# terminusdb-labs/parallel-hnsw

Measured on AMD Instinct MI355X. Metric: queries/sec at recall@10≥0.95 on 1M×768 f32, higher is better.
Workload: dtype f32

## Files before the change

### parallel_hnsw_amd/csrc/api.hip

```cpp
#include <hip/hip_runtime.h>

#include <algorithm>
#include <atomic>
#include <cmath>
#include <cstdarg>
#include <cstdio>
#include <cstring>
#include <new>
#include <stdexcept>
#include <vector>

#include "exact_slices.h"
#include "phnsw_internal.h"

static thread_local std::string g_err;

void ph_set_error(const char *fmt, ...) {
  char buf[1024];
  va_list ap;
  va_start(ap, fmt);
  vsnprintf(buf, sizeof(buf), fmt, ap);
  va_end(ap);
  g_err = buf;
}
// ... 359 lines not shown
    int rc = ph_order_by_keys_device(L.pos + first, count, L.ord, 0);
    if (rc) return rc;
    L.ord_first = first;
    L.ord_count = count;
  }
  *out = L.ord;
  return 0;
}

int ph_layer_upload(phnsw_index *ix, const uint32_t *nodes, const uint32_t *neighbors, uint32_t n, uint32_t W,
                    PhLayerHost *out) {
  if (ix) ix->nodes_epoch++;
  PhLayerHost l;
  l.n_nodes = n;
  l.W = W;
  hipError_t e = hipMalloc(&l.nodes, (size_t)n * 4);
  if (e == hipSuccess) e = hipMalloc(&l.neighbors, (size_t)n * W * 4);
  if (e == hipSuccess) e = hipMemcpy(l.nodes, nodes, (size_t)n * 4, hipMemcpyHostToDevice);
  if (e == hipSuccess && neighbors)
    e = hipMemcpy(l.neighbors, neighbors, (size_t)n * W * 4, hipMemcpyHostToDevice);
  if (e != hipSuccess) {
    ph_layer_free(l);
    return ph_hip_fail(e, "layer upload", __FILE__, __LINE__);
  }
  if (!neighbors) {
    int rc = ph_fill_u32(l.neighbors, PH_EMPTY32, (uint64_t)n * W, 0);
    if (rc) {
      ph_layer_free(l);
      return rc;
    }
  }
  bool identity = true;
  for (uint32_t i = 0; i < n; i++)
    if (nodes[i] != i) {
      identity = false;
      break;
    }
  l.identity = identity;
  if (!identity) {
    e = hipMalloc(&l.vec2node, (size_t)ix->store->n * 4);
    if (e != hipSuccess) {
      ph_layer_free(l);
      return ph_hip_fail(e, "vec2node alloc", __FILE__, __LINE__);
    }
    int rc = ph_fill_u32(l.vec2node, PH_EMPTY32, ix->store->n, 0);
    if (!rc) rc = ph_scatter_vec2node(l.nodes, n, l.vec2node, 0);
    if (!rc) {
      e = hipDeviceSynchronize();
      if (e != hipSuccess) rc = ph_hip_fail(e, "vec2node sync", __FILE__, __LINE__);
    }
    if (rc) {
      ph_layer_free(l);
      return rc;
    }
  }
  *out = l;
  return 0;
}

static std::atomic<uint64_t> g_import_dups{0};
extern "C" uint64_t phnsw_debug_import_duplicates(void) { return g_import_dups.load(); }

static int validate_layer(const phnsw_store *s, const uint64_t *nodes, const uint64_t *neighbors, uint64_t n,
                          uint64_t W, std::vector<uint32_t> &nodes32, std::vector<uint32_t> &nb32) {
  if (n == 0 || W == 0 || W > 64 || n >= 0x7FFFFFFFull) {
    ph_set_error("layer shape unsupported: node_count=%llu neighborhood_size=%llu (1..64)", (unsigned long long)n,
                 (unsigned long long)W);
    return PHNSW_E_UNSUPPORTED;
  }
  const bool strict = getenv("PHNSW_STRICT_IMPORT") != nullptr;
  nodes32.resize(n);
  nb32.resize(n * W);
  for (uint64_t i = 0; i < n; i++) {
    if (nodes[i] >= s->n || (i > 0 && nodes[i] <= nodes[i - 1])) {
      ph_set_error("layer nodes must be strictly increasing VectorIds below the store size (search.rs:150-157)");
      return PHNSW_E_INVALID;
    }
    nodes32[i] = (uint32_t)nodes[i];
  }
  for (uint64_t i = 0; i < n; i++) {
    bool ended = false;
    uint64_t o = 0;
    for (uint64_t k = 0; k < W; k++) {
      uint64_t v = neighbors[i * W + k];
      if (v == PHNSW_EMPTY) {
        ended = true;
        continue;
      }
      if (ended || v >= n) {
        ph_set_error("neighbor row %llu: ids must be < node_count and sentinels trailing only (lib.rs:108-125)",
                     (unsigned long long)i);
        return PHNSW_E_INVALID;
      }
      bool dup = false;
      for (uint64_t j = 0; j < o; j++)
        if (nb32[i * W + j] == (uint32_t)v) dup = true;
      if (dup) {
        if (strict) {
          ph_set_error("neighbor row %llu holds node %llu twice (PHNSW_STRICT_IMPORT)", (unsigned long long)i,
                       (unsigned long long)v);
          return PHNSW_E_INVALID;
        }
        g_import_dups++;
        continue;
      }
      nb32[i * W + o++] = (uint32_t)v;
    }
    for (; o < W; o++) nb32[i * W + o] = PH_EMPTY32;
  }
  return 0;
}

extern "C" int phnsw_index_from_layers(phnsw_store *s, uint32_t layer_count, const uint64_t *node_counts,
                                       const uint64_t *neighborhood_sizes, const uint64_t *const *nodes,
                                       const uint64_t *const *neighbors, phnsw_index **out) try {
  if (!s || !out || layer_count == 0 || layer_count > PH_MAX_LAYERS || !node_counts || !neighborhood_sizes ||
      !nodes || !neighbors) {
    ph_set_error("phnsw_index_from_layers: invalid argument");
    return PHNSW_E_INVALID;
  }
  PH_HIP(hipSetDevice(s->device));
  phnsw_index *ix = new phnsw_index();
  ix->store = s;
  s->refcount++;
  phnsw_default_build_params(&ix->bp);
  for (uint32_t l = 0; l < layer_count; l++) {
    std::vector<uint32_t> n32, nb32;
    int rc = validate_layer(s, nodes[l], neighbors[l], node_counts[l], neighborhood_sizes[l], n32, nb32);
    PhLayerHost lh;
    if (!rc) rc = ph_layer_upload(ix, n32.data(), nb32.data(), (uint32_t)node_counts[l], (uint32_t)neighborhood_sizes[l], &lh);
    if (rc) {
      phnsw_index_destroy(ix);
      return rc;
    }
    ix->layers.push_back(lh);
  }
  *out = ix;
  return 0;
} catch (...) { return ph_caught(); }

extern "C" void phnsw_index_destroy(phnsw_index *ix) {
  if (!ix) return;
  hipSetDevice(ix->store->device);
  for (auto &l : ix->layers) ph_layer_free(l);
  ph_pending_free(ix);
  ph_workspace_free(ix->ws[0]);
  ph_workspace_free(ix->ws[1]);
  ph_host_stages_free(ix);
  ph_exact_free(ix);
  ph_auto_free(ix);
  ph_build_table_free(ix);
  if (ix->totals) hipFree(ix->totals);
  phnsw_store_destroy(ix->store);
  delete ix;
  ph_pool_trim();
}

extern "C" uint32_t phnsw_index_layer_count(const phnsw_index *ix) { return ix ? (uint32_t)ix->layers.size() : 0; }

extern "C" int phnsw_index_layer_info(const phnsw_index *ix, uint32_t lft, uint64_t *node_count, uint64_t *W) try {
  if (!ix || lft >= ix->layers.size()) {
    ph_set_error("layer %u out of range", lft);
    return PHNSW_E_INVALID;
  }
  if (node_count) *node_count = ix->layers[lft].n_nodes;
  if (W) *W = ix->layers[lft].W;
  return 0;
} catch (...) { return ph_caught(); }

extern "C" int phnsw_index_layer_read(const phnsw_index *ix, uint32_t lft, uint64_t *nodes, uint64_t *neighbors) try {
  if (!ix || lft >= ix->layers.size()) {
    ph_set_error("layer %u out of range", lft);
    return PHNSW_E_INVALID;
  }
  PH_HIP(hipSetDevice(ix->store->device));
  const PhLayerHost &l = ix->layers[lft];
  if (nodes) {
    std::vector<uint32_t> t(l.n_nodes);
    PH_HIP(hipMemcpy(t.data(), l.nodes, (size_t)l.n_nodes * 4, hipMemcpyDeviceToHost));
    for (uint32_t i = 0; i < l.n_nodes; i++) nodes[i] = t[i];
  }
  if (neighbors) {
    std::vector<uint32_t> t((size_t)l.n_nodes * l.W);
    PH_HIP(hipMemcpy(t.data(), l.neighbors, t.size() * 4, hipMemcpyDeviceToHost));
    for (size_t i = 0; i < t.size(); i++) neighbors[i] = t[i] == PH_EMPTY32 ? PHNSW_EMPTY : t[i];
  }
  return 0;
} catch (...) { return ph_caught(); }


int ph_check_sp(const phnsw_index *ix, const phnsw_search_params *sp) {
  if (!ix || !sp || ix->layers.empty()) {
    ph_set_error("search: null index/params or index without layers");
    return PHNSW_E_INVALID;
  }
  if (sp->number_of_candidates == 0 || sp->number_of_candidates > 1024 || sp->probe_depth == 0 ||
      sp->probe_depth > 0xFFFFFFFFull) {
    ph_set_error("search: number_of_candidates must be 1..1024 and probe_depth >= 1 (got %llu, %llu)",
                 (unsigned long long)sp->number_of_candidates, (unsigned long long)sp->probe_depth);
    return PHNSW_E_INVALID;
  }
  return 0;
}

static void fill_args(const phnsw_index *ix, const PhSearchCall &c, PhSearchArgs &a) {
  memset(&a, 0, sizeof(a));
  const phnsw_store *s = ix->store;
  a.dist = ph_dist_args(s);
  uint32_t nl = (c.upto == 0 || c.upto > ix->layers.size()) ? (uint32_t)ix->layers.size() : c.upto;
  a.n_layers = nl;
  for (uint32_t l = 0; l < nl; l++) {
    const PhLayerHost &h = ix->layers[l];
    a.layers[l].n_nodes = h.n_nodes;
    a.layers[l].W = h.W;
    a.layers[l].nodes = h.nodes;
    a.layers[l].neighbors = h.neighbors;
    a.layers[l].vec2node = h.identity ? nullptr : h.vec2node;
  }
  a.ef = (uint32_t)c.sp->number_of_candidates;
  a.upper = (uint32_t)std::min<uint64_t>(c.sp->upper_layer_candidate_count, 0xFFFFFFFFull);
  a.probe_depth = (uint32_t)c.sp->probe_depth;
  a.queries = c.queries;
  a.ldq = c.ldq;
  a.qids = c.qids;
  a.exclude = c.exclude;
  if (c.filter.words) {
    a.filter = c.filter.words;
    a.filter_stride = c.filter.stride;
    a.filter_flags = c.filter.flags;
  }
  a.nq = (uint32_t)c.nq;
  a.out_ids = c.out_ids;
  a.out_d = c.out_d;
  a.out_len = c.out_len;
  a.out_stats = c.out_stats;
  a.status = c.status;
  a.knn_mode = c.knn_mode;
  a.out_stride = c.out_stride;
  a.out_hit = c.out_hit;
  a.threshold = c.threshold;
  a.first_node = c.first_node;
  a.hit_eps = c.hit_eps;
  a.cap_max = c.knn_mode == 2 ? c.out_stride : 0;
  a.out_index = c.out_index;
  a.order = c.order;
}

uint32_t ph_default_ovf_cap(uint32_t ef) {
  if (const char *e = getenv("PHNSW_OVF_CAP"))
    if (atoi(e) > 0) return (uint32_t)atoi(e);
  return std::max<uint32_t>(8192u, ef * 64u);
}
static uint32_t default_ovf_cap(uint32_t ef) { return ph_default_ovf_cap(ef); }

static uint64_t two_launch_min() {
  const char *e = getenv("PHNSW_TWO_LAUNCH_MIN");
  return (e && atoll(e) > 0) ? (uint64_t)atoll(e) : (uint64_t)PH_TWO_LAUNCH_MIN;
}
static std::atomic<uint64_t> g_two_launch_count{0};
extern "C" uint64_t phnsw_debug_two_launch_count(void) { return g_two_launch_count.load(); }
extern "C" uint32_t phnsw_debug_last_search_chunks(const phnsw_index *ix) { return ix ? ix->ws[ix->ws_last].n_chunks : 0; }

extern "C" int phnsw_stream_create_beside(int device, void *other_stream, void **out_stream) try {
  if (!out_stream) {
    ph_set_error("phnsw_stream_create_beside: out_stream is NULL");
    return PHNSW_E_INVALID;
  }
  PH_HIP(hipSetDevice(device));
  hipStream_t st = nullptr;
  int rc = ph_stream_beside((hipStream_t)other_stream, &st);
  if (rc) return rc;
  *out_stream = (void *)st;
  return 0;
} catch (...) { return ph_caught(); }

static int attach_probes(phnsw_index *mix, const PhSearchCall &c, PhSearchArgs &a) {
  (void)mix, (void)c, (void)a;
#ifdef PH_CELL_PROBE
  {
    static unsigned long long *probe_dev = nullptr;
    if (!probe_dev) {
      PH_HIP(hipMalloc(&probe_dev, 12 * sizeof(unsigned long long)));
      PH_HIP(hipMemset(probe_dev, 0, 12 * sizeof(unsigned long long)));
    } else {
      unsigned long long h[12];
      PH_HIP(hipDeviceSynchronize());
      PH_HIP(hipMemcpy(h, probe_dev, sizeof(h), hipMemcpyDeviceToHost));
      if (h[11]) {
        fprintf(stderr, "[cell probe] %llu queries, %llu bottom-layer evaluations; within r chain ranks of the landing cell:", h[11], h[10]);
        for (int k = 0; k < 10; k++) fprintf(stderr, " r<=%u: %.3f", k ? (1u << (k - 1)) : 0u, (double)h[k] / (double)h[10]);
        fprintf(stderr, "\n");
      }
      PH_HIP(hipMemset(probe_dev, 0, 12 * sizeof(unsigned long long)));
    }
    a.probe_out = probe_dev;
    a.probe_pos = nullptr;
    if (!c.knn_mode && ph_store_f32(mix->store) && c.nq >= 1000) {
      int rc = ph_layer_anchor_pos(mix->store, mix->layers[a.n_layers - 1]);
      if (rc) return rc;
      a.probe_pos = mix->layers[a.n_layers - 1].pos;
    }
  }
#endif
#ifdef PH_VISITED_PROBE
  {
    static unsigned long long *vprobe_dev = nullptr;
    if (!vprobe_dev) {
      PH_HIP(hipMalloc(&vprobe_dev, 130 * sizeof(unsigned long long)));
      PH_HIP(hipMemset(vprobe_dev, 0, 130 * sizeof(unsigned long long)));
    } else {
      unsigned long long h[130];
      PH_HIP(hipDeviceSynchronize());
      PH_HIP(hipMemcpy(h, vprobe_dev, sizeof(h), hipMemcpyDeviceToHost));
      for (int k = 0; k < 2; k++) {
        unsigned long long n = 0, sum = 0, run = 0;
        for (int b = 0; b < 64; b++) n += h[64 * k + b], sum += h[64 * k + b] * (64ull * b + 32ull);
        if (!n) continue;
        fprintf(stderr, "[visited probe] %s: %llu walks, mean ~%.0f ids, past the LDS load limit: %.4f; ids < 64*(b+1) for",
                k ? "bottom layer" : "upper gathered layers", n, (double)sum / (double)n, (double)h[128 + k] / (double)n);
        for (int b = 0; b < 64; b++) {
          run += h[64 * k + b];
          if (h[64 * k + b]) fprintf(stderr, " b%d:%.4f", b, (double)run / (double)n);
        }
        fprintf(stderr, "\n");
      }
      PH_HIP(hipMemset(vprobe_dev, 0, 130 * sizeof(unsigned long long)));
    }
    a.vprobe_out = vprobe_dev;
  }
#endif
  return 0;
}

int ph_search_device(const phnsw_index *ix, const PhSearchCall &c) {
  phnsw_index *mix = const_cast<phnsw_index *>(ix);
  const uint64_t nq = c.nq;
  const uint32_t knn_mode = c.knn_mode, out_stride = c.out_stride;
  uint32_t *const out_index = c.out_index;
  const hipStream_t stream = c.stream;
  if (ph_store_converted(ix->store) && (knn_mode || out_index || c.hint || c.out_hit)) {
    return ph_search_only_unsupported(ix->store, knn_mode ? "knn / threshold_nn" : (out_index ? "search_instrumented" : "build search"));
  }
  PhSearchArgs a;
  fill_args(ix, c, a);
  if (ix->dbg_order && ix->dbg_order_n == nq) a.order = ix->dbg_order;
  std::lock_guard<std::mutex> g(mix->ws_mutex);
  if (!mix->totals) {
    PH_HIP(hipMalloc(&mix->totals, 16));
    PH_HIP(hipMemset(mix->totals, 0, 16));
  }
  a.totals = mix->totals;
  PhWorkspace &ws = mix->ws[mix->ws_next & 1];
  mix->ws_last = mix->ws_next & 1;
  mix->ws_next++;
  int rc = ph_workspace_ensure(ix, ws, std::max(a.ef, a.cap_max), c.ovf_cap ? c.ovf_cap : default_ovf_cap(a.ef));
  if (rc) return rc;
  const uint32_t T = (knn_mode || out_index) ? 0u : ph_tiny_layer_count(ix, a.n_layers, a.ef);
  uint32_t first_big = a.n_layers;
  for (uint32_t l = std::max(1u, T); l < a.n_layers; l++)
    if (ph_layer_own_launch(ix->layers[l].n_nodes, ph_row_bytes(ix->store))) {
      first_big = l;
      break;
    }
  if (!a.order && knn_mode && nq >= PH_ORDER_MIN) {
    PhLayerHost &B = mix->layers[a.n_layers - 1];
    rc = ph_layer_anchor_pos(ix->store, B);
    if (!rc && c.first_node + nq <= B.n_nodes) rc = ph_layer_range_order(B, c.first_node, (uint32_t)nq, &a.order);
    if (rc) return rc;
  }
  const bool split = (ph_store_f32(ix->store) || ph_store_converted(ix->store)) && !a.order && !knn_mode && !out_stride && !out_index && first_big < a.n_layers &&
                     nq >= two_launch_min() &&
                     !getenv("PHNSW_NO_LOCALITY");
  if (split) {
    g_two_launch_count++;
    rc = ph_workspace_order_ensure(ws, a.nq);
    for (uint32_t l = first_big; l < a.n_layers && !rc; l++)
      rc = ph_layer_anchor_pos(ix->store, mix->layers[l - 1]);
    if (rc) return rc;
  }
  rc = attach_probes(mix, c, a);
  if (rc) return rc;
  rc = ph_search_begin(ws, stream);
  if (rc) return rc;
  bool kept_table = false;
  if (c.hint && T && !split) {
    rc = ph_build_table_prepare(mix, ws, a, *c.hint, T, stream, &kept_table);
    if (rc) return rc;
  }
  const uint64_t tmax = (T && !kept_table) ? ph_tiny_max_positions(ix, a.n_layers, a.ef) : 0;
  const uint64_t chunk = (tmax && nq > tmax) ? tmax : nq;
  for (uint64_t c0 = 0; c0 < nq; c0 += chunk) {
    PhSearchArgs b = a;
    const uint64_t cnt = std::min<uint64_t>(chunk, nq - c0);
    const bool last_chunk = c0 + cnt == nq;
    b.nq = (uint32_t)cnt;
    if (b.order) {
      b.order += c0;
    } else if (c0) {
      const uint32_t ostride = out_stride ? out_stride : b.ef;
      if (b.queries) b.queries += c0 * c.ldq;
      if (b.qids) b.qids += c0;
      if (b.exclude) b.exclude += c0;
      if (b.filter) b.filter += c0 * b.filter_stride;
      b.out_ids += c0 * ostride;
      b.out_d += c0 * ostride;
      b.out_len += c0;
      if (b.out_stats) b.out_stats += 2 * c0;
      b.status += c0;
      if (b.out_hit) b.out_hit += c0;
      b.first_node += (uint32_t)c0;
    }
    ws.n_chunks = (uint32_t)(c0 / chunk) + 1;
    PH_HIP(hipEventRecord(ws.evc, stream));
    if (c0) PH_HIP(hipMemsetAsync(ws.dtotals, 0, sizeof(unsigned long long) * 3 * PH_MAX_DISPATCH, stream));
    if (!kept_table) {
      rc = ph_tiny_prepare(ix, ws, b, T, stream);
      if (rc) return rc;
    }
    ws.d_tiny = b.tiny_layers != 0;
    PH_HIP(hipEventRecord(ws.evd[0], stream));
    if (!split) {
      b.launch_totals = ws.dtotals;
      b.launch_tab = ws.dtotals + 2 * PH_MAX_DISPATCH;
      rc = ph_search_launch(ix, ws, b, stream, last_chunk);
      if (rc) return rc;
      PH_HIP(hipEventRecord(ws.evd[1], stream));
      ws.n_dispatch = 1;
      ws.d_lo[0] = knn_mode ? b.n_layers - 1 : 0;
      ws.d_hi[0] = b.n_layers;
      continue;
    }
    const uint32_t Td = b.tiny_layers;
    const bool dense_first = Td && Td < b.n_layers && b.nq >= PH_DENSE_SPLIT_MIN && !getenv("PHNSW_NO_DENSE_SPLIT");
    if (dense_first) b.dense_flag = ws.tiny_member + b.tiny_n;
    uint32_t di = 0;
    uint32_t *const out_hit_final = b.out_hit;
    const uint32_t first_hi = dense_first ? Td : first_big;
    for (uint32_t lo = 0, hi = first_hi; lo < b.n_layers; lo = hi, hi = (lo == Td && dense_first && first_big > Td) ? first_big : hi + 1) {
      PhSearchArgs p = b;
      const bool last = hi == b.n_layers;
      p.layer_lo = lo;
      p.layer_hi = hi;
      if (lo) p.tiny_layers = 0;
      if (dense_first) {
        p.dense_only = lo == 0 ? 1u : 0u;
        p.after_dense = lo == Td ? Td : 0u;
      }
      p.order = lo ? ws.oorder : nullptr;
      p.out_hit = last ? out_hit_final : nullptr;
      p.out_key = last ? nullptr : ws.okey;
      p.key_pos = last ? nullptr : ix->layers[hi - 1].pos;
      p.launch_totals = ws.dtotals + 2 * di;
      p.launch_tab = ws.dtotals + 2 * PH_MAX_DISPATCH + di;
      rc = ph_search_launch(ix, ws, p, stream, last && last_chunk);
      if (!rc && !last) rc = ph_workspace_order_sort(ws, b.nq, stream);
      if (rc) return rc;
      PH_HIP(hipEventRecord(ws.evd[1 + di], stream));
      ws.d_lo[di] = lo;
      ws.d_hi[di] = hi;
      ws.n_dispatch = ++di;
    }
  }
  return 0;
}

static int check_device_call(const char *call, const phnsw_index *ix, const PhSearchCall &c) {
  int rc = ph_check_sp(ix, c.sp);
  if (rc) return rc;
  if ((!c.queries && !c.qids) || !c.out_ids || !c.out_d || !c.out_len || !c.status || c.nq > 0xFFFFFFFFull ||
      (c.queries && (c.ldq < ix->store->ld || (c.ldq % 4) || ((uintptr_t)c.queries % 16)))) {
    ph_set_error("%s: invalid argument (queries need ldq >= store ld, multiple of 4, 16-byte base)", call);
    return PHNSW_E_INVALID;
  }
  return 0;
}

static PhSearchCall device_call(const float *queries_dev, uint32_t ldq, const uint32_t *qids_dev, uint64_t nq,
                                const phnsw_search_params *sp, uint32_t upto_layers, const uint32_t *exclude_dev,
                                uint32_t *out_ids_dev, float *out_d_dev, uint32_t *out_len_dev, uint32_t *out_stats_dev,
                                uint32_t *status_dev, void *stream) {
  PhSearchCall c = {};
  c.queries = queries_dev, c.ldq = ldq, c.qids = qids_dev, c.exclude = exclude_dev, c.nq = nq;
  c.sp = sp, c.upto = upto_layers;
  c.out_ids = out_ids_dev, c.out_d = out_d_dev, c.out_len = out_len_dev, c.status = status_dev;
  c.out_stats = out_stats_dev;
  c.stream = (hipStream_t)stream;
  return c;
}

extern "C" int phnsw_search_batch_device(const phnsw_index *ix, const float *queries_dev, uint32_t ldq,
                                         const uint32_t *qids_dev, uint64_t nq, const phnsw_search_params *sp,
                                         uint32_t upto_layers, const uint32_t *exclude_dev, uint32_t *out_ids_dev,
                                         float *out_d_dev, uint32_t *out_len_dev, uint32_t *out_stats_dev,
                                         uint32_t *status_dev, void *stream) try {
  const PhSearchCall c = device_call(queries_dev, ldq, qids_dev, nq, sp, upto_layers, exclude_dev, out_ids_dev, out_d_dev,
                                     out_len_dev, out_stats_dev, status_dev, stream);
  int rc = check_device_call("phnsw_search_batch_device", ix, c);
  if (rc) return rc;
  if (nq == 0) return 0;
  PH_HIP(hipSetDevice(ix->store->device));
  return ph_search_device(ix, c);
} catch (...) { return ph_caught(); }


int ph_filter_check(const phnsw_index *ix, const uint32_t *filter, uint32_t stride, uint32_t flags, const char *call,
                    PhFilter *f) {
  const uint64_t words = (ix->store->n + 31u) / 32u;
  if (flags & ~(uint32_t)PHNSW_FILTER_STRICT) {
    ph_set_error("%s: unknown flag bits 0x%x", call, flags);
    return PHNSW_E_INVALID;
  }
  if (stride && stride < words) {
    ph_set_error("%s: filter_stride_words %u is below the %llu words of one bitmap (0 = one shared bitmap)", call, stride,
                 (unsigned long long)words);
    return PHNSW_E_INVALID;
  }
  f->words = filter;
  f->stride = filter ? stride : 0u;
  f->flags = flags;
  return 0;
}

extern "C" int phnsw_search_batch_filtered_device(const phnsw_index *ix, const float *queries_dev, uint32_t ldq,
                                                  const uint32_t *qids_dev, uint64_t nq, const phnsw_search_params *sp,
                                                  uint32_t upto_layers, const uint32_t *exclude_dev,
                                                  const uint32_t *filter_dev, uint32_t filter_stride_words, uint32_t flags,
                                                  uint32_t *out_ids_dev, float *out_d_dev, uint32_t *out_len_dev,
                                                  uint32_t *out_stats_dev, uint32_t *status_dev, void *stream) try {
  PhSearchCall c = device_call(queries_dev, ldq, qids_dev, nq, sp, upto_layers, exclude_dev, out_ids_dev, out_d_dev,
                               out_len_dev, out_stats_dev, status_dev, stream);
  int rc = check_device_call("phnsw_search_batch_filtered_device", ix, c);
  if (rc) return rc;
  rc = ph_filter_check(ix, filter_dev, filter_stride_words, flags, "phnsw_search_batch_filtered_device", &c.filter);
  if (rc) return rc;
  if (!c.filter.words) c.filter.words = ix->default_filter;
  if (nq == 0) return 0;
  PH_HIP(hipSetDevice(ix->store->device));
  return ph_search_device(ix, c);
} catch (...) { return ph_caught(); }

extern "C" int phnsw_index_set_filter_device(phnsw_index *ix, const uint32_t *filter_dev) try {
  if (!ix) {
    ph_set_error("phnsw_index_set_filter_device: null index");
    return PHNSW_E_INVALID;
  }
  ix->default_filter = filter_dev;
  return 0;
} catch (...) { return ph_caught(); }


int ph_exact_check(const phnsw_index *ix, uint64_t k, const char *call) {
  if (!ix || ix->layers.empty()) {
    ph_set_error("%s: null index or index without layers", call);
    return PHNSW_E_INVALID;
  }
  if (!ph_exact_k_valid(k)) {
    ph_set_error("%s: k must be 1..1024 (got %llu)", call, (unsigned long long)k);
    return PHNSW_E_INVALID;
  }
  if (ph_store_pq_shared(ix->store)) {
    ph_set_error("%s: not supported over a shared-codebook PQ store; use its reconstruction store", call);
    return PHNSW_E_UNSUPPORTED;
  }
  return 0;
}

extern "C" int phnsw_search_exact_filtered_device(const phnsw_index *ix, const float *queries_dev, uint32_t ldq,
                                                  const uint32_t *qids_dev, uint64_t nq, const uint32_t *exclude_dev,
                                                  const uint32_t *filter_dev, uint32_t filter_stride_words, uint64_t k,
                                                  uint32_t *out_ids_dev, float *out_d_dev, uint32_t *out_len_dev,
                                                  uint32_t *status_dev, void *stream) try {
  const char *const call = "phnsw_search_exact_filtered_device";
  int rc = ph_exact_check(ix, k, call);
  if (rc) return rc;
  if (nq == 0) return 0;
  if (((!queries_dev) == (!qids_dev)) || !out_ids_dev || !out_d_dev || !out_len_dev || !status_dev || nq > 0xFFFFFFFFull ||
      (queries_dev && (ldq < ix->store->ld || (ldq % 4) || ((uintptr_t)queries_dev % 16)))) {
    ph_set_error("%s: invalid argument (queries or qids, exactly one; outputs; queries need ldq >= store ld, multiple of 4, "
                 "16-byte base)", call);
    return PHNSW_E_INVALID;
  }
  PhExactCall c = {};
  rc = ph_filter_check(ix, filter_dev, filter_stride_words, 0u, call, &c.filter);
  if (rc) return rc;
  if (!c.filter.words) c.filter.words = ix->default_filter;
  c.queries = queries_dev, c.ldq = ldq, c.qids = qids_dev, c.exclude = exclude_dev, c.nq = nq, c.k = (uint32_t)k;
  c.out_ids = out_ids_dev, c.out_d = out_d_dev, c.out_len = out_len_dev, c.status = status_dev;
  c.stream = (hipStream_t)stream;
  PH_HIP(hipSetDevice(ix->store->device));
  return ph_exact_device(ix, c);
} catch (...) { return ph_caught(); }

extern "C" int phnsw_filter_count_device(const phnsw_index *ix, const uint32_t *filter_dev, uint32_t filter_stride_words,
                                         uint64_t nbitmaps, uint32_t *out_count_dev, void *stream) try {
  const char *const call = "phnsw_filter_count_device";
  if (!ix || ix->layers.empty() || (!out_count_dev && nbitmaps)) {
    ph_set_error("%s: null index, index without layers or null output", call);
    return PHNSW_E_INVALID;
  }
  PhFilter f;
  int rc = ph_filter_check(ix, filter_dev, filter_stride_words, 0u, call, &f);
  if (rc) return rc;
  if (!f.words) f.words = ix->default_filter;
  PH_HIP(hipSetDevice(ix->store->device));
  return ph_filter_count(ix, f, nbitmaps, out_count_dev, (hipStream_t)stream);
} catch (...) { return ph_caught(); }

extern "C" int phnsw_debug_last_tiny_table(const phnsw_index *ix, float *out_host, uint64_t cap_floats, uint32_t *npos,
                                           uint32_t *tn, uint32_t *stride, int *g) try {
  if (!ix) return PHNSW_E_INVALID;
  phnsw_index *mix = const_cast<phnsw_index *>(ix);
  std::lock_guard<std::mutex> lock(mix->ws_mutex);
  PhWorkspace &ws = mix->ws[mix->ws_last];
  if (!ws.timed || !ws.d_tiny || !ws.tiny_d) {
    ph_set_error("the last search on this index made no dense table");
    return PHNSW_E_INVALID;
  }
  const uint64_t need = (uint64_t)ws.tiny_last_npos * ws.tiny_last_stride;
  if (npos) *npos = ws.tiny_last_npos;
  if (tn) *tn = ws.tiny_last_tn;
  if (stride) *stride = ws.tiny_last_stride;
  if (g) *g = ws.tiny_table_g;
  if (out_host) {
    if (cap_floats < need) {
      ph_set_error("phnsw_debug_last_tiny_table: %llu floats needed", (unsigned long long)need);
      return PHNSW_E_INVALID;
    }
    PH_HIP(hipSetDevice(ix->store->device));
    PH_HIP(hipEventSynchronize(ws.ev1));
    PH_HIP(hipMemcpy(out_host, ws.tiny_d, need * 4u, hipMemcpyDeviceToHost));
  }
  return 0;
} catch (...) { return ph_caught(); }

extern "C" int phnsw_debug_layer_pos(phnsw_index *ix, uint32_t lft, uint32_t *out_host) try {
  if (lft >= ix->layers.size() || !ix->layers[lft].pos) return PHNSW_E_INVALID;
  PH_HIP(hipMemcpy(out_host, ix->layers[lft].pos, (size_t)ix->layers[lft].n_nodes * 4, hipMemcpyDeviceToHost));
  return 0;
} catch (...) { return ph_caught(); }

extern "C" int phnsw_debug_set_order(phnsw_index *ix, const uint32_t *order_dev, uint64_t n) try {
  ix->dbg_order = order_dev;
  ix->dbg_order_n = n;
  return 0;
} catch (...) { return ph_caught(); }

extern "C" int phnsw_index_counters(const phnsw_index *ix, uint64_t *n_dist, uint64_t *n_hops) try {
  if (!ix) return PHNSW_E_INVALID;
  unsigned long long h[2] = {0, 0};
  if (ix->totals) {
    PH_HIP(hipSetDevice(ix->store->device));
    PH_HIP(hipDeviceSynchronize());
    PH_HIP(hipMemcpy(h, ix->totals, 16, hipMemcpyDeviceToHost));
  }
  if (n_dist) *n_dist = h[0];
  if (n_hops) *n_hops = h[1];
  return 0;
} catch (...) { return ph_caught(); }

extern "C" int phnsw_last_search_kernel_ms(const phnsw_index *ix, float *ms) try {
  if (!ix || !ms) return PHNSW_E_INVALID;
  phnsw_index *mix = const_cast<phnsw_index *>(ix);
  std::lock_guard<std::mutex> g(mix->ws_mutex);
  PhWorkspace &ws = mix->ws[mix->ws_last];
  if (!ws.timed) {
    ph_set_error("no search has been launched on this index");
    return PHNSW_E_INVALID;
  }
  PH_HIP(hipEventSynchronize(ws.ev1));
  PH_HIP(hipEventElapsedTime(ms, ws.ev0, ws.ev1));
  return 0;
} catch (...) { return ph_caught(); }

extern "C" int phnsw_last_search_dispatches(const phnsw_index *ix, uint32_t cap, uint32_t *count, float *ms,
                                            uint64_t *n_dist, uint64_t *n_hops, uint32_t *layer_lo,
                                            uint32_t *layer_hi) try {
  if (!ix || !count) return PHNSW_E_INVALID;
  phnsw_index *mix = const_cast<phnsw_index *>(ix);
  std::lock_guard<std::mutex> g(mix->ws_mutex);
  PhWorkspace &ws = mix->ws[mix->ws_last];
  if (!ws.timed) {
    ph_set_error("no search has been launched on this index");
    return PHNSW_E_INVALID;
  }
  PH_HIP(hipSetDevice(ix->store->device));
  PH_HIP(hipEventSynchronize(ws.ev1));
  unsigned long long h[2 * PH_MAX_DISPATCH];
  PH_HIP(hipMemcpy(h, ws.dtotals, sizeof(h), hipMemcpyDeviceToHost));
  const uint32_t n = ws.n_dispatch + 1;
  *count = n;
  for (uint32_t i = 0; i < n && i < cap; i++) {
    float t = 0.f;
    PH_HIP(hipEventElapsedTime(&t, i == 0 ? ws.evc : ws.evd[i - 1], ws.evd[i]));
    if (ms) ms[i] = t;
    if (n_dist) n_dist[i] = i ? h[2 * (i - 1)] : 0;
    if (n_hops) n_hops[i] = i ? h[2 * (i - 1) + 1] : 0;
    if (layer_lo) layer_lo[i] = i ? ws.d_lo[i - 1] : 0;
    if (layer_hi) layer_hi[i] = i ? ws.d_hi[i - 1] : 0;
  }
  return 0;
} catch (...) { return ph_caught(); }

extern "C" int phnsw_last_search_table_evals(const phnsw_index *ix, uint32_t cap, uint32_t *count, uint64_t *n_table) try {
  if (!ix || !count) return PHNSW_E_INVALID;
  phnsw_index *mix = const_cast<phnsw_index *>(ix);
  std::lock_guard<std::mutex> g(mix->ws_mutex);
  PhWorkspace &ws = mix->ws[mix->ws_last];
  if (!ws.timed) {
    ph_set_error("no search has been launched on this index");
    return PHNSW_E_INVALID;
  }
  PH_HIP(hipSetDevice(ix->store->device));
  PH_HIP(hipEventSynchronize(ws.ev1));
  unsigned long long h[PH_MAX_DISPATCH];
  PH_HIP(hipMemcpy(h, ws.dtotals + 2 * PH_MAX_DISPATCH, sizeof(h), hipMemcpyDeviceToHost));
  const uint32_t n = ws.n_dispatch + 1;
  *count = n;
  for (uint32_t i = 0; i < n && i < cap; i++)
    if (n_table) n_table[i] = i ? h[i - 1] : 0;
  return 0;
} catch (...) { return ph_caught(); }

extern "C" int phnsw_dense_top_layers(const phnsw_index *ix, uint64_t number_of_candidates, uint32_t *layers, uint64_t *nodes,
                                      uint32_t *matrix_cores) try {
  if (!ix || !ix->store) {
    ph_set_error("phnsw_dense_top_layers: null index");
    return PHNSW_E_INVALID;
  }
  const uint32_t ef = (uint32_t)std::min<uint64_t>(number_of_candidates, 0xFFFFFFFFull);
  const uint32_t T = ph_tiny_layer_count(ix, (uint32_t)ix->layers.size(), ef);
  if (layers) *layers = T;
  if (nodes) *nodes = T ? ix->layers[T - 1].n_nodes : 0;
  if (matrix_cores) *matrix_cores = (T && ph_tiny_matrix_cores(ix)) ? 1u : 0u;
  return 0;
} catch (...) { return ph_caught(); }

extern "C" int phnsw_knn(const phnsw_index *ix, uint64_t k, uint64_t probe_depth, uint64_t *out_ids, float *out_d,
                         uint64_t *out_len) try {
  if (ix)
    if (int rc = ph_search_only_unsupported(ix->store, "phnsw_knn")) return rc;
  if (!ix || ix->layers.empty() || k == 0 || k * 3 > 1024) {
    ph_set_error("phnsw_knn: k must be 1..341");
    return PHNSW_E_INVALID;
  }
  const PhLayerHost &L = ix->layers.back();
  phnsw_search_params sp = {k * 3, k * 3, probe_depth};
  uint64_t n = L.n_nodes, cap = k * 3;
  std::vector<uint64_t> ids(n * cap), len(n);
  std::vector<float> d(n * cap);
  PhHostSearch h = {};
  h.nq = n, h.sp = &sp, h.knn_mode = 1;
  h.out_ids = ids.data(), h.out_d = d.data(), h.out_len = len.data();
  int rc = ph_search_host(ix, h);
  if (rc) return rc;
  std::vector<uint64_t> nodes(n);
  rc = phnsw_index_layer_read(ix, (uint32_t)ix->layers.size() - 1, nodes.data(), nullptr);
  if (rc) return rc;
  for (uint64_t i = 0; i < n; i++) {
    uint64_t o = 0;
    for (uint64_t j = 0; j < len[i] && o < k; j++) {
      if (ids[i * cap + j] == nodes[i]) continue;
      out_ids[i * k + o] = ids[i * cap + j];
      out_d[i * k + o] = d[i * cap + j];
      o++;
    }
    out_len[i] = o;
    for (; o < k; o++) {
      out_ids[i * k + o] = PHNSW_EMPTY;
      out_d[i * k + o] = PH_FMAX;
    }
  }
  return 0;
} catch (...) { return ph_caught(); }

namespace {
template <class T>
struct GrowBuf {
  T *p = nullptr;
  size_t have = 0;
  int alloc(size_t count) {
    count = std::max<size_t>(count, 1);
    if (have >= count) return 0;
    if (p) hipFree(p);
    p = nullptr;
    have = 0;
    hipError_t e = hipMalloc((void **)&p, count * sizeof(T));
    if (e != hipSuccess) return ph_hip_fail(e, "hipMalloc (threshold_nn)", __FILE__, __LINE__);
    have = count;
    return 0;
  }
  ~GrowBuf() {
    if (p) hipFree(p);
  }
  GrowBuf() = default;
  GrowBuf(const GrowBuf &) = delete;
  GrowBuf &operator=(const GrowBuf &) = delete;
};
}
#define PH_TRY_(x)         \
  do {                     \
    int rc__ = (x);        \
    if (rc__) return rc__; \
  } while (0)

static int threshold_nn_big(const phnsw_index *ix, const phnsw_search_params *sp, float threshold,
                            const std::vector<uint32_t> &all_nodes, const std::vector<uint32_t> &h_nodes, uint64_t max_out,
                            uint64_t *out_ids, float *out_d, uint64_t *out_len, uint32_t lds_cap) {
  const PhLayerHost &L = ix->layers.back();
  const uint32_t n = L.n_nodes;
  const uint64_t isd = sp->number_of_candidates;
  const uint32_t os = (uint32_t)std::min<uint64_t>(max_out + 2, (uint64_t)n + 1);
  const uint64_t words = ((uint64_t)n + 31) / 32 + 1;
  uint64_t cap0 = isd * 2;
  while (cap0 <= lds_cap) cap0 *= 2;
  GrowBuf<uint32_t> d_nodes, d_vis, d_q, d_oid, d_len, d_status, d_counter;
  GrowBuf<float> d_od;
  GrowBuf<uint2> d_ovf;
  std::vector<uint32_t> h_ids, h_len, h_status;
  std::vector<float> h_d;
  size_t piece = std::max<size_t>(1, std::min<size_t>(16384, (1ull << 30) / ((size_t)os * 8)));
  if (const char *e = getenv("PHNSW_THRESHOLD_BIG_PIECE"))
    if (atoll(e) > 0) piece = (size_t)atoll(e);
  for (size_t c0 = 0; c0 < all_nodes.size(); c0 += piece) {
  std::vector<uint32_t> nodes(all_nodes.begin() + c0, all_nodes.begin() + std::min(all_nodes.size(), c0 + piece));
  uint64_t cap = cap0;
  while (!nodes.empty()) {
    if (cap > 0x7FFFFFFFull) {
      ph_set_error("threshold_nn: queue capacity beyond 2^31");
      return PHNSW_E_UNSUPPORTED;
    }
    const bool final_cap = cap >= 2ull * n;
    const uint64_t per_slot = cap * 8 + (uint64_t)n * 8 + words * 4;
    uint64_t budget = 4ull << 30;
    if (const char *e = getenv("PHNSW_THRESHOLD_BIG_BYTES")) budget = strtoull(e, nullptr, 10);
    const uint32_t grid = (uint32_t)std::min<uint64_t>(std::min<uint64_t>(nodes.size(), 1024), std::max<uint64_t>(1, budget / per_slot));
    const size_t cnt = nodes.size();
    PH_TRY_(d_nodes.alloc(cnt));
    PH_TRY_(d_oid.alloc(cnt * os));
    PH_TRY_(d_od.alloc(cnt * os));
    PH_TRY_(d_len.alloc(cnt));
    PH_TRY_(d_status.alloc(cnt));
    PH_TRY_(d_counter.alloc(128));
    PH_TRY_(d_vis.alloc((size_t)grid * words));
    PH_TRY_(d_ovf.alloc((size_t)grid * n));
    PH_TRY_(d_q.alloc((size_t)grid * 2 * cap));
    PH_HIP(hipMemset(d_vis.p, 0, (size_t)grid * words * 4));
    PH_HIP(hipMemcpy(d_nodes.p, nodes.data(), cnt * 4, hipMemcpyHostToDevice));
    PhSearchCall c = {};
    c.nq = cnt, c.sp = sp;
    c.out_ids = d_oid.p, c.out_d = d_od.p, c.out_len = d_len.p, c.status = d_status.p;
    c.knn_mode = 2, c.threshold = threshold, c.out_stride = os;
    PhSearchArgs a;
    fill_args(ix, c, a);
    a.cap_max = (uint32_t)cap;
    a.knn_nodes = d_nodes.p;
    a.big_q = d_q.p;
    a.visited = d_vis.p;
    a.visited_words = words;
    a.ovf = d_ovf.p;
    a.ovf_cap = n;
    a.counter = d_counter.p;
    PH_TRY_(ph_search_launch_big(ix, a, grid, 0));
    PH_HIP(hipDeviceSynchronize());
    h_ids.resize(cnt * os);
    h_d.resize(cnt * os);
    h_len.resize(cnt);
    h_status.resize(cnt);
    PH_HIP(hipMemcpy(h_ids.data(), d_oid.p, cnt * os * 4, hipMemcpyDeviceToHost));
    PH_HIP(hipMemcpy(h_d.data(), d_od.p, cnt * os * 4, hipMemcpyDeviceToHost));
    PH_HIP(hipMemcpy(h_len.data(), d_len.p, cnt * 4, hipMemcpyDeviceToHost));
    PH_HIP(hipMemcpy(h_status.data(), d_status.p, cnt * 4, hipMemcpyDeviceToHost));
    std::vector<uint32_t> again;
    for (size_t x = 0; x < cnt; x++) {
      const uint64_t i = nodes[x];
      if (h_status[x] == 6 && !final_cap) {
        again.push_back(nodes[x]);
        continue;
      }
      if (h_status[x]) {
        ph_set_error("threshold_nn: node %llu failed with status %u at a queue capacity of %llu", (unsigned long long)i,
                     h_status[x], (unsigned long long)cap);
        return PHNSW_E_OVERFLOW;
      }
      uint64_t o = 0;
      for (uint32_t j = 0; j < h_len[x]; j++) {
        const uint32_t v = h_ids[x * os + j];
        const float d = h_d[x * os + j];
        if (v == h_nodes[i]) continue;
        if (!(d < threshold)) break;
        if (o == max_out) {
          ph_set_error("threshold_nn: node %llu has more than max_out=%llu results", (unsigned long long)i,
                       (unsigned long long)max_out);
          return PHNSW_E_OVERFLOW;
        }
        out_ids[i * max_out + o] = v;
        out_d[i * max_out + o] = d;
        o++;
      }
      out_len[i] = o;
      for (; o < max_out; o++) {
        out_ids[i * max_out + o] = PHNSW_EMPTY;
        out_d[i * max_out + o] = PH_FMAX;
      }
    }
    nodes.swap(again);
    cap *= 2;
  }
  }
  return 0;
}

extern "C" int phnsw_threshold_nn(const phnsw_index *ix, float threshold, uint64_t probe_depth,
                                  uint64_t initial_search_depth, uint64_t max_out, uint64_t *out_ids, float *out_d,
                                  uint64_t *out_len) try {
  if (ix)
    if (int rc = ph_search_only_unsupported(ix->store, "phnsw_threshold_nn")) return rc;
  if (!ix || ix->layers.empty() || !out_ids || !out_d || !out_len || initial_search_depth == 0 ||
      initial_search_depth > 0x40000000ull || probe_depth == 0 || max_out == 0) {
    ph_set_error("phnsw_threshold_nn: initial_search_depth and probe_depth must be >= 1");
    return PHNSW_E_INVALID;
  }
  const phnsw_store *s = ix->store;
  PH_HIP(hipSetDevice(s->device));
  const PhLayerHost &L = ix->layers.back();
  const uint32_t n = L.n_nodes, CAPMAX = 1024, CHUNK = 16384;
  phnsw_search_params sp = {initial_search_depth, initial_search_depth, probe_depth};
  std::vector<uint32_t> h_nodes(n);
  PH_HIP(hipMemcpy(h_nodes.data(), L.nodes, (size_t)n * 4, hipMemcpyDeviceToHost));
  std::vector<uint32_t> big;
  if (initial_search_depth > CAPMAX || getenv("PHNSW_THRESHOLD_ALL_BIG")) {
    big.resize(n);
    for (uint32_t i = 0; i < n; i++) big[i] = i;
    return threshold_nn_big(ix, &sp, threshold, big, h_nodes, max_out, out_ids, out_d, out_len, 0);
// ... 70 lines not shown
```

### parallel_hnsw_amd/csrc/phnsw_internal.h

```cpp
#pragma once
#include <hip/hip_runtime.h>
#include <stdint.h>
#include <stdlib.h>

#include <mutex>
#include <string>
#include <vector>

#include "../../include/phnsw.h"

#define PH_EMPTY32 0xFFFFFFFFu
#define PH_FMAX 3.4028234663852886e38f
#define PH_MAX_LAYERS 24
#define PH_WAVE 64
#define PH_MAX_DISPATCH 24
#define PH_DENSE_SPLIT_MIN 2048u
#define PH_TINY_MAX_NODES 8192u
#define PH_TINY_LDS_NODES 1024u
#define PH_TINY_MAX_LAYERS 8

void ph_set_error(const char *fmt, ...);
int ph_caught() noexcept;
int ph_hip_fail(hipError_t e, const char *what, const char *file, int line);
#define PH_HIP(x)                                                       \
  do {                                                                  \
    hipError_t e__ = (x);                                               \
    if (e__ != hipSuccess) return ph_hip_fail(e__, #x, __FILE__, __LINE__); \
  } while (0)

struct PhLayerDev {
  uint32_t n_nodes;
  uint32_t W;
  const uint32_t *nodes;
  const uint32_t *neighbors;
  const uint32_t *vec2node;
};

struct PhLayerHost {
  uint32_t n_nodes = 0, W = 0;
  uint32_t *nodes = nullptr;
  uint32_t *neighbors = nullptr;
  float *nbr_dist = nullptr;
  uint64_t links_epoch = 0;
  uint32_t *vec2node = nullptr;
  bool identity = false;
  uint32_t *recall_q = nullptr;
  uint32_t recall_n = 0;
  uint32_t *pos = nullptr;
  uint32_t *ord = nullptr;
  uint32_t ord_first = 0, ord_count = 0;
};

enum PhRowKind : int {
  PH_ROWS_F32 = 0,
  PH_ROWS_F16,
  PH_ROWS_I8,
  PH_ROWS_PQ,
  PH_ROWS_PQ_SHARED,
  PH_ROWS_I8Q,
};
static inline bool ph_rows_converted(int kind) { return kind == PH_ROWS_F16 || kind == PH_ROWS_I8 || kind == PH_ROWS_I8Q; }
static inline bool ph_rows_i8_layout(int kind) { return kind == PH_ROWS_I8 || kind == PH_ROWS_I8Q; }
static inline const char *ph_rows_name(int kind) {
  static const char *const names[] = {"f32", "f16", "i8", "product-quantised", "shared-codebook product-quantised", "i8q"};
  return names[kind];
}
static inline int ph_chunk_count(uint32_t nv4) { return nv4 <= 64 ? 1 : (nv4 <= 192 ? 3 : (nv4 <= 384 ? 6 : 0)); }
int ph_dim_unsupported(uint32_t dim);
struct PhRows {
  const void *base;
  uint32_t stride;
  int kind;
};

struct PhDistArgs {
  PhRows rows;
  uint32_t ld, nv4;
  int metric;
  const uint8_t *codes;
  const uint16_t *codes16;
  const float *codebook;
  uint32_t m, ksub, dsub;
  uint32_t table_f16;
};

struct phnsw_store {
  int device = 0;
  int kind = PH_ROWS_F32;
  float *rows = nullptr;
  uint8_t *codes = nullptr;
  uint16_t *codes16 = nullptr;
  phnsw_store *centroid_store = nullptr;
  phnsw_index *centroid_index = nullptr;
  phnsw_search_params quantized_search = {0, 0, 0};
  float *codebook = nullptr;
  uint32_t pq_m = 0, pq_ksub = 0, pq_dsub = 0;
  uint32_t pq_table_f16 = 0;
  void *packed = nullptr;
  uint32_t packed_stride = 0;
  float *anchors = nullptr;
  uint32_t *anchor_rank = nullptr;
  uint32_t n_anchors = 0;
  bool owns_rows = true;
  uint64_t n = 0;
  uint32_t dim = 0, ld = 0;
  int metric = 0;
  int refcount = 1;
};

struct PhTinyPrepKey {
  bool valid = false;
  uint64_t nodes_epoch = 0;
  uint32_t T = 0, tn = 0;
  const void *nodes[PH_TINY_MAX_LAYERS] = {}, *nbrs[PH_TINY_MAX_LAYERS] = {}, *vec2node = nullptr;
  uint32_t n[PH_TINY_MAX_LAYERS] = {}, W[PH_TINY_MAX_LAYERS] = {};
  uint64_t links[PH_TINY_MAX_LAYERS] = {};
};
struct PhTinyPackKey {
  bool valid = false;
  uint64_t nodes_epoch = 0;
  const void *vecs = nullptr, *tnodes = nullptr;
  uint32_t ld = 0, tn = 0, nv = 0;
};

struct PhWorkspace {
  uint32_t *visited = nullptr;
  uint64_t visited_words = 0;
  uint2 *ovf = nullptr;
  uint32_t ovf_cap = 0;
  uint32_t n_slots = 0;
  uint32_t *counter = nullptr;
  hipEvent_t ev0 = nullptr, ev1 = nullptr;
  hipEvent_t evc = nullptr;
  bool timed = false;
  void *pq_tables = nullptr;
  size_t pq_tables_bytes = 0;
  uint32_t *okey = nullptr, *okey_sorted = nullptr, *oiota = nullptr, *oorder = nullptr;
  void *sort_tmp = nullptr;
  size_t sort_tmp_bytes = 0;
  uint32_t order_cap = 0;
  float *tiny_d = nullptr;
  size_t tiny_d_bytes = 0;
  uint32_t *tiny_nbr = nullptr;
  size_t tiny_nbr_bytes = 0;
  uint32_t *tiny_member = nullptr;
  size_t tiny_member_bytes = 0;
  float4 *tiny_pq = nullptr, *tiny_pn = nullptr;
  size_t tiny_pq_bytes = 0, tiny_pn_bytes = 0;
  PhTinyPrepKey tiny_prep_key;
  PhTinyPackKey tiny_pack_key;
  int tiny_table_g = 0;
  uint32_t tiny_last_npos = 0, tiny_last_tn = 0, tiny_last_stride = 0;
  uint2 *dense_ovf = nullptr;
  size_t dense_ovf_bytes = 0;
  uint32_t *ovf_s = nullptr;
  size_t ovf_s_cap = 0;
  hipEvent_t evd[PH_MAX_DISPATCH + 1] = {};
  unsigned long long *dtotals = nullptr;
  uint32_t n_dispatch = 0;
  uint32_t n_chunks = 0;
  int cus = 0;
  uint32_t d_lo[PH_MAX_DISPATCH] = {}, d_hi[PH_MAX_DISPATCH] = {};
  bool d_tiny = false;
};

struct PhBuildTable {
  float *D = nullptr;
  size_t bytes = 0;
  size_t cap = 0;
  const uint32_t *qnodes = nullptr, *tnodes = nullptr;
  uint32_t qn = 0, tn = 0, T = 0, stride = 0;
  uint32_t lo_alloc = 0, hi_alloc = 0, lo = 0, hi = 0;
  uint64_t epoch = 0;
};
struct PhRowHint {
  const uint32_t *qnodes;
  uint32_t qn;
  const uint32_t *vec2node;
  uint32_t first, count;
  bool contiguous;
};

struct PhFilter {
  const uint32_t *words;
  uint32_t stride, flags;
};

struct PhExactScratch {
  uint64_t *keys = nullptr;
  size_t bytes = 0;
  hipEvent_t done = nullptr;
};

struct PhAutoSet;
struct PhPendingLayer;
struct PhHostStage;
struct phnsw_index {
  std::vector<PhHostStage *> stages;
  std::mutex stage_mutex;
  std::vector<PhBuildTable> bt;
  std::vector<std::pair<float *, size_t>> bt_spare;
  bool bt_enabled = false;
  uint64_t nodes_epoch = 0;
  PhPendingLayer *pending = nullptr;
  phnsw_store *store = nullptr;
  std::vector<PhLayerHost> layers;
  phnsw_build_params bp;
  std::mutex ws_mutex;
  PhWorkspace ws[2];
  uint32_t ws_next = 0, ws_last = 0;
  float last_kernel_ms = 0.f;
  unsigned long long *totals = nullptr;
  const uint32_t *dbg_order = nullptr;
  const uint32_t *default_filter = nullptr;
  uint64_t dbg_order_n = 0;
  std::mutex exact_mutex;
  PhExactScratch exact[2];
  uint32_t exact_next = 0;
  std::vector<PhAutoSet *> autos;
  std::mutex auto_mutex;
};

struct PhSearchArgs {
  PhDistArgs dist;
  const float *queries;
  uint32_t ldq;
  const uint32_t *qids;
  const uint32_t *exclude;
  const uint32_t *filter;
  uint32_t filter_stride, filter_flags;
  uint32_t nq;
  uint32_t n_layers;
  PhLayerDev layers[PH_MAX_LAYERS];
  uint32_t ef, upper, probe_depth;
  uint32_t *out_ids;
  float *out_d;
  uint32_t *out_len;
  uint32_t *out_stats;
  uint32_t *status;
  uint32_t *visited;
  uint64_t visited_words;
  uint2 *ovf;
  uint32_t ovf_cap;
  uint32_t *counter;
  uint32_t knn_mode;
  float threshold;
  uint32_t first_node;
  uint32_t cap_max;
  const uint32_t *knn_nodes;
  uint32_t *big_q;
  uint32_t tiny_lds_nodes;
  float hit_eps;
  uint32_t out_stride;
  unsigned long long *totals;
  unsigned long long *launch_totals;
  unsigned long long *launch_tab;
  void *pq_tables;
  uint32_t pq_table_bytes;
  uint32_t layer_lo, layer_hi;
  uint32_t *out_key;
  const uint32_t *key_pos;
  uint32_t dense_only, after_dense;
  const uint32_t *dense_flag;
  uint2 *dense_ovf;
  uint32_t dense_ovf_cap;
#ifdef PH_CELL_PROBE
  const uint32_t *probe_pos;
  unsigned long long *probe_out;
#endif
#ifdef PH_VISITED_PROBE
  unsigned long long *vprobe_out;
#endif
  uint32_t vis_slots, vis_limit, vis_off;
  const uint32_t *order;
  uint32_t seg;
  uint32_t *out_hit;
  uint32_t *out_index;
  uint32_t *ovf_s;
  uint32_t tiny_layers, tiny_n, tiny_stride;
  const float *tiny_d;
  const uint32_t *tiny_nbr;
  const uint32_t *tiny_member;
  uint32_t tiny_rows, tiny_row_first;
  const uint32_t *tiny_row_map;
  uint32_t tiny_off[PH_TINY_MAX_LAYERS];
};

uint32_t ph_default_ovf_cap(uint32_t ef);
hipError_t ph_timed_malloc(void **p, size_t bytes);
hipError_t ph_timed_free(void *p);
#ifndef PH_RAW_ALLOC
#define hipMalloc(p, n) ph_timed_malloc((void **)(p), (n))
#define hipFree(p) ph_timed_free((void *)(p))
#endif
int ph_stream_beside(hipStream_t other, hipStream_t *io);
hipError_t ph_pool_alloc(void **p, size_t bytes);
void ph_pool_free(void *p);
void ph_pool_trim(void);
void ph_layer_free(PhLayerHost &l);
void ph_pending_free(phnsw_index *ix);
void ph_host_stages_free(phnsw_index *ix);
int ph_layer_upload(phnsw_index *ix, const uint32_t *nodes, const uint32_t *neighbors, uint32_t n, uint32_t W,
                    PhLayerHost *out);
struct PhSearchCall {
  const float *queries;
  uint32_t ldq;
  const uint32_t *qids, *exclude;
  uint64_t nq;
  const phnsw_search_params *sp;
  uint32_t upto;
  PhFilter filter;
  uint32_t *out_ids;
  float *out_d;
  uint32_t *out_len, *status;
  uint32_t *out_stats;
  uint32_t ovf_cap;
  hipStream_t stream;
  uint32_t knn_mode, first_node, out_stride;
  float threshold, hit_eps;
  uint32_t *out_hit, *out_index;
  const uint32_t *order;
  const PhRowHint *hint;
};
int ph_search_device(const phnsw_index *ix, const PhSearchCall &c);
int ph_check_sp(const phnsw_index *ix, const phnsw_search_params *sp);
int ph_filter_check(const phnsw_index *ix, const uint32_t *filter, uint32_t stride, uint32_t flags, const char *call,
                    PhFilter *f);
struct PhHostSearch {
  const float *queries;
  const uint64_t *qids, *exclude;
  uint64_t nq;
  const phnsw_search_params *sp;
  uint32_t upto, knn_mode;
  uint64_t out_k;
  uint64_t *out_ids;
  float *out_d;
  uint64_t *out_len;
  uint64_t *out_stats, *out_index;
  PhFilter filter;
  bool filter_on_device;
  bool exact;
};
int ph_search_host(const phnsw_index *ix, const PhHostSearch &h);
struct PhExactCall {
  const float *queries;
  uint32_t ldq;
  const uint32_t *qids, *exclude;
  uint64_t nq;
  PhFilter filter;
  uint32_t k;
  uint32_t *out_ids;
  float *out_d;
  uint32_t *out_len, *status;
  hipStream_t stream;
  const uint32_t *list;
};
int ph_exact_device(const phnsw_index *ix, const PhExactCall &c);
int ph_exact_supported(const phnsw_index *ix, uint32_t k);
void ph_exact_bottom_layer(const phnsw_index *ix, uint32_t *n_nodes, const uint32_t **nodes, const uint32_t **vec2node);
int ph_filter_count(const phnsw_index *ix, const PhFilter &f, uint64_t nbitmaps, uint32_t *out_count_dev, hipStream_t stream);
void ph_exact_free(phnsw_index *ix);
struct PhAutoCall {
  const float *queries;
  uint32_t ldq;
  const uint32_t *qids, *exclude;
  uint64_t nq;
  const phnsw_search_params *sp;
  PhFilter filter;
  uint32_t k;
  uint64_t scan_below;
  uint32_t *out_ids;
  float *out_d;
  uint32_t *out_len, *status;
  uint32_t *out_route;
  hipStream_t stream;
};
int ph_auto_device(const phnsw_index *ix, const PhAutoCall &c);
void ph_auto_free(phnsw_index *ix);
int ph_exact_check(const phnsw_index *ix, uint64_t k, const char *call);
#define PH_ORDER_MIN 16384u
#define PH_POS_MIN 256u
#define PH_SPLIT_BYTES (4ull << 20)
static inline bool ph_layer_own_launch(uint64_t n_nodes, uint32_t row_bytes) {
  const char *e = getenv("PHNSW_SPLIT_BYTES");
  const uint64_t limit = (e && atoll(e) > 0) ? (uint64_t)atoll(e) : (uint64_t)PH_SPLIT_BYTES;
  return n_nodes * (uint64_t)row_bytes > limit;
}
int ph_layer_anchor_pos(const phnsw_store *s, PhLayerHost &L);
bool ph_layer_wants_cells(const phnsw_store *s, uint32_t n_nodes);
int ph_layer_cells_range(const phnsw_store *s, const PhLayerHost &L, uint32_t first, uint32_t count, uint32_t *out_pos);
void ph_store_anchors_free(phnsw_store *s);
int ph_order_by_keys_device(const uint32_t *keys, uint32_t n, uint32_t *order_out, hipStream_t st);
int ph_layer_range_order(PhLayerHost &L, uint32_t first, uint32_t count, const uint32_t **out);

static inline bool ph_store_converted(const phnsw_store *s) { return ph_rows_converted(s->kind); }
static inline bool ph_store_f32(const phnsw_store *s) { return s->kind == PH_ROWS_F32; }
static inline bool ph_store_pq(const phnsw_store *s) { return s->kind == PH_ROWS_PQ; }
static inline bool ph_store_pq_shared(const phnsw_store *s) { return s->kind == PH_ROWS_PQ_SHARED; }
int ph_converted_gather_rows(const phnsw_store *s, const uint32_t *ids_dev, uint32_t first, uint32_t cnt, float *out_dev);
int ph_converted_store_read(const phnsw_store *s, uint64_t first, uint64_t count, float *out);

int ph_tiny_prepare(const phnsw_index *ix, PhWorkspace &ws, PhSearchArgs &a, uint32_t max_layers, hipStream_t stream);
int ph_build_table_prepare(phnsw_index *ix, PhWorkspace &ws, PhSearchArgs &a, const PhRowHint &h, uint32_t T,
                           hipStream_t stream, bool *used);
void ph_build_table_free(phnsw_index *ix);
size_t ph_tiny_lds_bytes(const PhSearchArgs &a);
bool ph_tiny_matrix_cores(const phnsw_index *ix);
uint32_t ph_tiny_layer_count(const phnsw_index *ix, uint32_t n_layers, uint32_t ef);
uint64_t ph_tiny_max_positions(const phnsw_index *ix, uint32_t n_layers, uint32_t ef);
void ph_tiny_free(PhWorkspace &ws);

int ph_search_begin(PhWorkspace &ws, hipStream_t stream);
int ph_search_launch(const phnsw_index *ix, PhWorkspace &ws, PhSearchArgs &a, hipStream_t stream, bool mark_end = true);
int ph_search_launch_big(const phnsw_index *ix, PhSearchArgs &a, uint32_t grid, hipStream_t stream);
int ph_workspace_order_ensure(PhWorkspace &ws, uint32_t nq);
int ph_workspace_order_sort(PhWorkspace &ws, uint32_t nq, hipStream_t stream);
void ph_workspace_order_free(PhWorkspace &ws);
#define PH_TWO_LAUNCH_MIN 32768u
int ph_workspace_ensure(const phnsw_index *ix, PhWorkspace &ws, uint32_t ef, uint32_t ovf_cap);
void ph_workspace_free(PhWorkspace &ws);
size_t ph_tiny_beside_lds(const phnsw_index *ix, const PhSearchArgs &a);
static inline PhRows ph_store_rows(const phnsw_store *s) {
  PhRows r;
  r.base = ph_store_converted(s) ? (const void *)s->packed : (const void *)s->rows;
  r.stride = ph_store_converted(s) ? s->packed_stride : s->ld * 4u;
  r.kind = s->kind;
  return r;
}
static inline PhDistArgs ph_dist_args(const phnsw_store *s) {
  PhDistArgs d;
  d.rows = ph_store_rows(s);
  d.ld = s->ld;
  d.nv4 = s->ld / 4;
  d.metric = s->metric;
  d.codes = s->codes;
  d.codes16 = s->codes16;
  d.codebook = s->codebook;
  d.m = s->pq_m;
  d.ksub = s->pq_ksub;
  d.dsub = s->pq_dsub;
  d.table_f16 = s->pq_table_f16;
  return d;
}
static inline uint32_t ph_row_bytes(const phnsw_store *s) { return ph_store_rows(s).stride; }
static inline int ph_search_only_unsupported(const phnsw_store *s, const char *call) {
  if (!s || !ph_store_converted(s)) return 0;
  ph_set_error("%s: not supported on an %s store or an index over one (search-only; use the f32 store)", call,
               ph_rows_name(s->kind));
  return PHNSW_E_UNSUPPORTED;
}
static inline bool ph_pq_global_tables() {
  const char *e = getenv("PHNSW_PQ_TABLE");
  return !(e && e[0] == 'l');
}
static inline size_t ph_pq_lds_bytes(const phnsw_store *s) {
  return ph_store_pq(s) ? (size_t)s->pq_m * s->pq_ksub * (s->pq_table_f16 == 2 ? 1 : (s->pq_table_f16 ? 2 : 4)) : 0;
}

void ph_comm_range(const phnsw_comm *comm, uint32_t r, uint64_t n, uint64_t *chunk, uint64_t *first, uint64_t *count);
int ph_comm_all_gather_device(const phnsw_comm *comm, const void *send_dev, void *recv_dev, uint64_t bytes);

int ph_synth_rows(float *rows_dev, uint64_t first, uint64_t count, uint32_t dim, uint32_t ld,
                  uint64_t seed, int normalize, hipStream_t s);
int ph_synth_clustered_rows(float *rows_dev, uint64_t first, uint64_t count, uint32_t dim, uint32_t ld, uint64_t seed,
                            uint32_t n_clusters, float noise, hipStream_t s);
int ph_distance_batch(const phnsw_store *st, const float *q_dev, uint32_t query_id, const uint32_t *ids_dev,
                      uint32_t k, float *out_dev, hipStream_t s);
int ph_fill_u32(uint32_t *p, uint32_t v, uint64_t n, hipStream_t s);
int ph_take_launch(const uint32_t *ids, const float *d, uint32_t ef, uint32_t k, uint64_t n, uint64_t *ids64, float *dk,
                   hipStream_t s);
int ph_scatter_vec2node(const uint32_t *nodes, uint32_t n, uint32_t *vec2node, hipStream_t s);
int ph_count_nan(const float *rows, uint64_t n_floats, uint32_t *out_count_dev, hipStream_t s);

__host__ __device__ inline uint64_t ph_mix64(uint64_t x) {
  x ^= x >> 30;
  x *= 0xBF58476D1CE4E5B9ULL;
  x ^= x >> 27;
  x *= 0x94D049BB133111EBULL;
  x ^= x >> 31;
  return x;
}
__host__ __device__ inline uint64_t ph_mulhi64(uint64_t a, uint64_t b) {
#if defined(__HIP_DEVICE_COMPILE__)
  return __umul64hi(a, b);
#else
  return (uint64_t)(((__uint128_t)a * b) >> 64);
#endif
}
__host__ __device__ inline uint64_t ph_feistel_perm(uint64_t i, uint64_t domain, uint64_t key) {
  if (domain <= 1) return 0;
  uint32_t bits = 0;
  while (((uint64_t)1 << bits) < domain) bits++;
  uint32_t h = (bits + 1) / 2;
  if (h == 0) h = 1;
  uint64_t mask = ((uint64_t)1 << h) - 1;
  uint64_t x = i;
  do {
    uint64_t L = x >> h, R = x & mask;
    for (uint32_t r = 0; r < 4; r++) {
      uint64_t f = ph_mix64(R + key * 0x9E3779B97F4A7C15ULL + r * 0xC2B2AE3D27D4EB4FULL) & mask;
      uint64_t nl = R;
      R = L ^ f;
      L = nl;
    }
    x = (L << h) | R;
  } while (x >= domain);
  return x;
}
void ph_shuffle_u64(uint64_t *v, uint64_t n, uint64_t seed);
```

### parallel_hnsw_amd/csrc/search.hip

```cpp
#include "search_kernels.h"


static int pick_capc(uint32_t ef) { return ef <= 128 ? 2 : (ef <= 512 ? 8 : (ef <= 1024 ? 16 : 0)); }

static bool vis_lds_on() {
  const char *e = getenv("PHNSW_VISITED");
  return !(e && !strcmp(e, "global"));
}
static int pick_capc_f32(uint32_t ef, bool grows, int nv) {
  return (!grows && ef > 128 && ef <= 256 && vis_lds_on() && vis_lds_shape(4, nv)) ? 4 : pick_capc(ef);
}
static int pick_capc_dense(uint32_t ef) { return ef <= 128 ? 2 : (ef <= 256 ? 4 : (ef <= 512 ? 8 : (ef <= 1024 ? 16 : 0))); }

static int pick_pqr(const phnsw_store *s, int capc) {
  if (!ph_store_pq(s) || s->pq_table_f16 != 2 || (capc != 2 && capc != 8) || getenv("PHNSW_PQ_TABLE")) return 0;
  const uint32_t m = s->pq_m;
  return (s->pq_ksub == 256 && (m == 32 || m == 64 || m == 96 || m == 128)) ? (int)m : 0;
}
static ph_search_fn pick_kernel_instr(int capc, int nv) {
#define PH_KI(C, N) \
  if (capc == C && nv == N) return (ph_search_fn)ph_search_kernel_instr<C, N>;
  PH_KI(8, 1) PH_KI(8, 3) PH_KI(8, 6) PH_KI(16, 1) PH_KI(16, 3) PH_KI(16, 6)
#undef PH_KI
  return nullptr;
}

#define PH_LATENCY_MAX 1024u
static size_t lds_bytes(int capc, size_t pq_lds) { return (size_t)(5 * capc * 64 + 64) * 4 + pq_lds; }

#define PH_VIS_SLOTS_MIN 1024u
#define PH_VIS_SLOTS_MAX 4096u
#define PH_LDS_GRANULE 1280u

static uint32_t vis_table_slots(ph_search_fn fn, size_t lds, int per_cu, size_t lds_cu, uint32_t ef, size_t hole) {
  if (!vis_lds_on() || per_cu <= 0) return 0;
  if (const char *e = getenv("PHNSW_VISITED_LDS_SLOTS")) {
    const long n = atol(e);
    if (n > 0) return lds + (size_t)n * 4u <= 64u * 1024u ? (uint32_t)n : 0u;
  }
  const uint32_t least = std::max<uint32_t>(PH_VIS_SLOTS_MIN, 4u * ef);
  size_t share = lds_cu / (size_t)per_cu;
  if (hole) {
    const size_t G = PH_LDS_GRANULE, hole_blocks = (hole + G - 1u) / G;
    const size_t with_hole = lds_cu / G > hole_blocks ? (lds_cu / G - hole_blocks) / (size_t)per_cu * G : 0u;
    if (with_hole >= lds + (size_t)least * 4u) share = with_hole;
  }
  const size_t room = std::min<size_t>(share, 64u * 1024u);
  if (room <= lds) return 0;
  for (uint32_t n = std::min<uint32_t>(PH_VIS_SLOTS_MAX, (uint32_t)((room - lds) / 4u) & ~63u); n >= least; n -= 64u) {
    int got = 0;
    if (hipOccupancyMaxActiveBlocksPerMultiprocessor(&got, (const void *)fn, 64, lds + (size_t)n * 4u) == hipSuccess &&
        got >= per_cu)
      return n;
  }
  return 0;
}

struct PhKernelChoice {
  ph_search_fn fn = nullptr;
  PhKernelFamily family = PH_KF_ROWS_F32;
  int capc = 0;
  int nv = 0;
  int pqr_m = 0;
  size_t pq_lds = 0;
  bool lat_shape = false;
};
static bool kf_rows(PhKernelFamily f) {
  return f == PH_KF_ROWS_F32 || f == PH_KF_ROWS_F16 || f == PH_KF_ROWS_I8 || f == PH_KF_ROWS_I8Q;
}

static PhKernelChoice pick_unfiltered_kernel(const phnsw_store *s, uint32_t ef_max, uint32_t nv4, bool grows, uint64_t nq,
                                             bool instr) {
  PhKernelChoice k;
  const int capc = pick_capc(ef_max);
  k.capc = capc;
  if (!capc) return k;
  switch (s->kind) {
    case PH_ROWS_PQ:
      k.pqr_m = pick_pqr(s, capc);
      k.family = k.pqr_m ? PH_KF_PQ_REG : PH_KF_PQ_TABLE;
      if (k.pqr_m) {
        k.fn = pick_kernel_pqr<false>(capc, k.pqr_m);
      } else {
        k.fn = pick_kernel_pqt<false>(capc, ph_pq_global_tables());
        k.pq_lds = ph_pq_global_tables() ? 0 : ph_pq_lds_bytes(s);
      }
      return k;
    case PH_ROWS_PQ_SHARED:
      k.family = PH_KF_PQ_SHARED;
      k.nv = ph_chunk_count(nv4);
      k.fn = pick_kernel_pqs<false>(capc, k.nv);
      return k;
    default: break;
  }
  k.nv = ph_chunk_count(nv4);
  if (s->kind == PH_ROWS_F32 && !instr && nq <= PH_LATENCY_MAX && !getenv("PHNSW_NO_LAT") && pick_kernel_lat<false>(capc, k.nv)) {
    k.family = PH_KF_LATENCY;
    k.fn = pick_kernel_lat<false>(capc, k.nv);
    k.lat_shape = true;
    return k;
  }
  if (instr) {
    k.family = PH_KF_INSTR;
    k.capc = std::max(capc, 8);
    k.fn = pick_kernel_instr(k.capc, k.nv);
    k.lat_shape = nq <= PH_LATENCY_MAX && !getenv("PHNSW_NO_LAT") && pick_kernel_lat<false>(capc, k.nv);
    return k;
  }
  k.capc = pick_capc_f32(ef_max, grows, k.nv);
  switch (s->kind) {
    case PH_ROWS_F16: k.family = PH_KF_ROWS_F16; k.fn = pick_kernel_rows<DistF16, false>(k.capc, k.nv); break;
    case PH_ROWS_I8: k.family = PH_KF_ROWS_I8; k.fn = pick_kernel_rows<DistI8, false>(k.capc, k.nv); break;
    case PH_ROWS_I8Q: k.family = PH_KF_ROWS_I8Q; k.fn = pick_kernel_rows<DistI8Q, false>(k.capc, k.nv); break;
    default: k.family = PH_KF_ROWS_F32; k.fn = pick_kernel_rows<DistF32, false>(k.capc, k.nv); break;
  }
  return k;
}

static PhKernelChoice pick_search_kernel(const phnsw_store *s, uint32_t ef_max, uint32_t nv4, bool grows, uint64_t nq,
                                         bool instr, bool filt = false) {
  PhKernelChoice k = pick_unfiltered_kernel(s, ef_max, nv4, grows, nq, instr);
  if (filt && k.fn) k.fn = ph_pick_filtered_kernel(k.family, k.capc, k.nv, k.pqr_m, ph_pq_global_tables());
  return k;
}

static uint32_t ph_search_slots(const PhKernelChoice &k, uint32_t ef, uint32_t *vis_slots = nullptr, size_t hole = 0) {
  if (vis_slots) *vis_slots = 0;
  if (!k.fn) return 0;
  int dev = 0;
  hipGetDevice(&dev);
  hipDeviceProp_t prop;
  if (hipGetDeviceProperties(&prop, dev) != hipSuccess) return 0;
  size_t lds = lds_bytes(k.capc, k.pq_lds);
  if (lds > 64 * 1024) {
    if (lds > 160 * 1024) return 0;
    if (hipFuncSetAttribute((const void *)k.fn, hipFuncAttributeMaxDynamicSharedMemorySize, (int)lds) != hipSuccess) return 0;
  }
  int per_cu = 0;
  if (hipOccupancyMaxActiveBlocksPerMultiprocessor(&per_cu, (const void *)k.fn, 64, lds) != hipSuccess || per_cu <= 0)
    per_cu = 1;
  int cap = 16;
  per_cu = std::min(per_cu, cap);
  if (const char *e = getenv("PHNSW_WAVES_PER_CU")) {
    if (atoi(e) > 0) per_cu = atoi(e);
    if (getenv("PHNSW_VERBOSE")) fprintf(stderr, "[phnsw] search grid: %d waves per CU (forced), lds %zu\n", per_cu, lds);
  }
  if (vis_slots && kf_rows(k.family) && vis_lds_shape(k.capc, k.nv))
    *vis_slots = vis_table_slots(k.fn, lds, per_cu, prop.maxSharedMemoryPerMultiProcessor, ef, hole);
  if (vis_slots && getenv("PHNSW_VERBOSE"))
    fprintf(stderr, "[phnsw] search grid: %d waves per CU, lds %zu + visited table %u slots (of %zu per CU, %zu left to a table block)\n",
            per_cu, lds, *vis_slots, (size_t)prop.maxSharedMemoryPerMultiProcessor, hole);
  return (uint32_t)(per_cu * prop.multiProcessorCount);
}

void ph_workspace_free(PhWorkspace &ws) {
  if (ws.visited) hipFree(ws.visited);
  if (ws.ovf) hipFree(ws.ovf);
  if (ws.counter) hipFree(ws.counter);
  if (ws.pq_tables) hipFree(ws.pq_tables);
  if (ws.ev0) hipEventDestroy(ws.ev0);
  if (ws.ev1) hipEventDestroy(ws.ev1);
  if (ws.evc) hipEventDestroy(ws.evc);
  for (auto &e : ws.evd)
    if (e) hipEventDestroy(e);
  if (ws.dtotals) hipFree(ws.dtotals);
  if (ws.dense_ovf) hipFree(ws.dense_ovf);
  if (ws.ovf_s) hipFree(ws.ovf_s);
  ph_workspace_order_free(ws);
  ph_tiny_free(ws);
  ws = PhWorkspace();
}

int ph_workspace_ensure(const phnsw_index *ix, PhWorkspace &ws, uint32_t ef, uint32_t ovf_cap) {
  uint64_t max_nodes = 0;
  for (auto &l : ix->layers) max_nodes = std::max<uint64_t>(max_nodes, l.n_nodes);
  uint64_t words = (max_nodes + 31) / 32 + 1;
  const phnsw_store *st = ix->store;
  uint32_t slots = 0;
  PhKernelFamily family = PH_KF_ROWS_F32;
  for (bool grows : {false, true}) {
    const PhKernelChoice k = pick_search_kernel(st, ef, st->ld / 4, grows, UINT64_MAX, false);
    slots = std::max(slots, ph_search_slots(k, ef));
    family = k.family;
  }
  const bool pqg = family == PH_KF_PQ_REG || (family == PH_KF_PQ_TABLE && ph_pq_global_tables());
  if (slots == 0) {
    ph_set_error("unsupported search shape: ef=%u dim=%u (ef <= 1024, dim <= 1536; PQ table + queue <= 160 KB LDS)", ef,
                 ix->store->dim);
    return PHNSW_E_UNSUPPORTED;
  }
  if (!ws.counter) {
    PH_HIP(hipMalloc(&ws.counter, 512));
    PH_HIP(hipEventCreate(&ws.ev0));
    PH_HIP(hipEventCreate(&ws.ev1));
    PH_HIP(hipEventCreate(&ws.evc));
    for (auto &e : ws.evd) PH_HIP(hipEventCreate(&e));
    PH_HIP(hipMalloc(&ws.dtotals, sizeof(unsigned long long) * 3 * PH_MAX_DISPATCH));
  }
  if (ws.n_slots < slots || ws.visited_words < words) {
    if (ws.visited) PH_HIP(hipFree(ws.visited));
    ws.visited = nullptr;
    uint32_t ns = std::max(ws.n_slots, slots);
    uint64_t nw = std::max(ws.visited_words, words);
    PH_HIP(hipMalloc(&ws.visited, (size_t)ns * nw * 4));
    PH_HIP(hipMemset(ws.visited, 0, (size_t)ns * nw * 4));
    if (ws.ovf && ws.n_slots < ns) {
      PH_HIP(hipFree(ws.ovf));
      ws.ovf = nullptr;
    }
    ws.n_slots = ns;
    ws.visited_words = nw;
  }
  if (pqg && ws.pq_tables_bytes < (size_t)ws.n_slots * ph_pq_lds_bytes(ix->store)) {
    if (ws.pq_tables) PH_HIP(hipFree(ws.pq_tables));
    ws.pq_tables = nullptr;
    ws.pq_tables_bytes = (size_t)ws.n_slots * ph_pq_lds_bytes(ix->store);
    PH_HIP(hipMalloc(&ws.pq_tables, ws.pq_tables_bytes));
  }
  if (!ws.ovf || ws.ovf_cap < ovf_cap) {
    if (ws.ovf) PH_HIP(hipFree(ws.ovf));
    ws.ovf = nullptr;
    ws.ovf_cap = std::max(ws.ovf_cap, ovf_cap);
    PH_HIP(hipMalloc(&ws.ovf, (size_t)ws.n_slots * ws.ovf_cap * sizeof(uint2)));
  }
  return 0;
}

int ph_search_begin(PhWorkspace &ws, hipStream_t stream) {
  if (ws.timed) PH_HIP(hipStreamWaitEvent(stream, ws.ev1, 0));
  PH_HIP(hipEventRecord(ws.ev0, stream));
  PH_HIP(hipMemsetAsync(ws.dtotals, 0, sizeof(unsigned long long) * 3 * PH_MAX_DISPATCH, stream));
  ws.n_dispatch = 0;
  ws.d_tiny = false;
  return 0;
}

template <class T>
static hipError_t grow_buf(T **p, size_t *have, size_t need) {
  if (*have >= need) return hipSuccess;
  if (*p) hipFree(*p);
  *p = nullptr;
  *have = 0;
  hipError_t e = hipMalloc((void **)p, need);
  if (e == hipSuccess) *have = need;
  return e;
}

static int search_launch_dense(PhWorkspace &ws, PhSearchArgs &a, hipStream_t stream) {
  const int capc = pick_capc_dense(a.ef);
  ph_search_fn fn = a.filter ? ph_pick_filtered_dense(capc) : pick_kernel_dense<false>(capc);
  if (!fn) {
    ph_set_error("unsupported search shape: ef=%u", a.ef);
    return PHNSW_E_UNSUPPORTED;
  }
  const size_t lds = lds_bytes(capc, ph_tiny_lds_bytes(a));
  if (!ws.cus) {
    int dev = 0;
    PH_HIP(hipGetDevice(&dev));
    PH_HIP(hipDeviceGetAttribute(&ws.cus, hipDeviceAttributeMultiprocessorCount, dev));
  }
  const int cus = ws.cus;
  int per_cu = 0;
  if (hipOccupancyMaxActiveBlocksPerMultiprocessor(&per_cu, (const void *)fn, 64, lds) != hipSuccess || per_cu <= 0) per_cu = 8;
  per_cu = std::min(per_cu, 32);
  if (const char *e = getenv("PHNSW_DENSE_WAVES_PER_CU"))
    if (atoi(e) > 0) per_cu = atoi(e);
  const uint32_t grid = (uint32_t)std::min<uint64_t>((uint64_t)per_cu * cus, a.nq);
  if (grid == 0) return 0;
  a.dense_ovf_cap = a.tiny_stride;
  PH_HIP(grow_buf(&ws.dense_ovf, &ws.dense_ovf_bytes, (size_t)grid * a.dense_ovf_cap * sizeof(uint2)));
  a.dense_ovf = ws.dense_ovf;
  a.visited = ws.visited;
  a.visited_words = 0;
  a.vis_slots = a.vis_limit = a.vis_off = 0;
  a.ovf = ws.ovf;
  a.ovf_cap = ws.ovf_cap;
  a.counter = ws.counter;
  PH_HIP(hipMemsetAsync(ws.counter, 0, 512, stream));
  a.seg = a.order ? (a.nq + 7u) / 8u : 0u;
  hipLaunchKernelGGL(fn, dim3(grid), dim3(64), lds, stream, a);
  PH_HIP(hipGetLastError());
  return 0;
}

int ph_search_launch_big(const phnsw_index *ix, PhSearchArgs &a, uint32_t grid, hipStream_t stream) {
  const phnsw_store *s = ix->store;
  const int nv = s->kind == PH_ROWS_PQ ? 0 : ph_chunk_count(a.dist.nv4);
  ph_search_fn fn = nullptr;
  size_t pq_lds = 0;
  if (s->kind == PH_ROWS_PQ_SHARED) {
    fn = nv == 1 ? (ph_search_fn)ph_search_kernel_big<DistPQS<1>>
                 : (nv == 3 ? (ph_search_fn)ph_search_kernel_big<DistPQS<3>> : (nv == 6 ? (ph_search_fn)ph_search_kernel_big<DistPQS<6>> : nullptr));
  } else if (s->kind == PH_ROWS_PQ) {
    fn = (ph_search_fn)ph_search_kernel_big<DistPQ>;
    pq_lds = ph_pq_lds_bytes(s);
  } else if (s->kind == PH_ROWS_F32) {
    fn = nv == 1 ? (ph_search_fn)ph_search_kernel_big<DistF32<1>>
                 : (nv == 3 ? (ph_search_fn)ph_search_kernel_big<DistF32<3>> : (nv == 6 ? (ph_search_fn)ph_search_kernel_big<DistF32<6>> : nullptr));
  }
  const size_t lds = lds_bytes(2, pq_lds);
  if (!fn || lds > 160 * 1024 || a.knn_mode != 2 || !a.big_q || a.cap_max < 2 * a.ef || grid == 0) {
    ph_set_error("unsupported search shape: threshold_nn with a queue of %u entries, dim %u", a.cap_max, s->dim);
    return PHNSW_E_UNSUPPORTED;
  }
  if (lds > 64 * 1024)
    PH_HIP(hipFuncSetAttribute((const void *)fn, hipFuncAttributeMaxDynamicSharedMemorySize, (int)lds));
  a.pq_tables = nullptr;
  a.pq_table_bytes = 0;
  a.seg = 0;
  a.order = nullptr;
  a.vis_slots = a.vis_limit = a.vis_off = 0;
  PH_HIP(hipMemsetAsync(a.counter, 0, 512, stream));
  hipLaunchKernelGGL(fn, dim3(grid), dim3(64), lds, stream, a);
  PH_HIP(hipGetLastError());
  return 0;
}

int ph_search_launch(const phnsw_index *ix, PhWorkspace &ws, PhSearchArgs &a, hipStream_t stream, bool mark_end) {
  if (a.dense_only) return search_launch_dense(ws, a, stream);
  const phnsw_store *st = ix->store;
  const uint32_t ef_max = std::max(a.ef, a.cap_max);
  if (ph_store_converted(st) && (a.knn_mode || a.out_index))
    return ph_search_only_unsupported(st, "knn / threshold_nn / search_instrumented");
  if (a.out_index && st->kind != PH_ROWS_F32) {
    ph_set_error("search_instrumented: f32 stores only");
    return PHNSW_E_UNSUPPORTED;
  }
  if (a.filter && (a.knn_mode || a.out_index)) {
    ph_set_error("knn / threshold_nn / search_instrumented take no filter");
    return PHNSW_E_UNSUPPORTED;
  }
  PhKernelChoice k = pick_search_kernel(st, ef_max, a.dist.nv4, a.knn_mode == 2, a.nq, a.out_index != nullptr, a.filter != nullptr);
  a.pq_tables = ws.pq_tables;
  a.pq_table_bytes = (uint32_t)ph_pq_lds_bytes(st);
  if (k.lat_shape && a.tiny_layers && a.tiny_n > a.tiny_lds_nodes && !getenv("PHNSW_NO_LAT_LDS_ROW") &&
      lds_bytes(pick_capc(ef_max), (size_t)a.tiny_stride * 4u + (size_t)((a.tiny_n + 31u) / 32u + 1u) * 4u) <= (160u * 1024u) / 3u)
    a.tiny_lds_nodes = a.tiny_n;
  if (st->kind != PH_ROWS_PQ) k.pq_lds = ph_tiny_lds_bytes(a);
  if (k.family == PH_KF_INSTR && k.fn) {
    if (ws.ovf_s_cap < (size_t)ws.n_slots * ws.ovf_cap) {
      if (ws.ovf_s) PH_HIP(hipFree(ws.ovf_s));
      ws.ovf_s = nullptr;
      ws.ovf_s_cap = 0;
      PH_HIP(hipMalloc(&ws.ovf_s, (size_t)ws.n_slots * ws.ovf_cap * 4));
      ws.ovf_s_cap = (size_t)ws.n_slots * ws.ovf_cap;
    }
    a.ovf_s = ws.ovf_s;
  }
  const ph_search_fn fn = k.fn;
  if (!fn) {
    ph_set_error("unsupported search shape: ef=%u nv4=%u", a.ef, a.dist.nv4);
    return PHNSW_E_UNSUPPORTED;
  }
  a.visited = ws.visited;
  a.visited_words = ws.visited_words;
  a.ovf = ws.ovf;
  a.ovf_cap = ws.ovf_cap;
  a.counter = ws.counter;
  uint32_t vis_slots = 0;
  const bool lat = k.family == PH_KF_LATENCY || k.family == PH_KF_INSTR;
  uint32_t slots = std::min<uint32_t>(ph_search_slots(k, ef_max, &vis_slots, lat ? 0 : ph_tiny_beside_lds(ix, a)), ws.n_slots);
  uint32_t grid = (uint32_t)std::min<uint64_t>(slots, a.nq);
  if (grid == 0) return 0;
  a.vis_slots = vis_slots;
  a.vis_limit = vis_slots - vis_slots / 4u;
  a.vis_off = (uint32_t)(lds_bytes(k.capc, k.pq_lds) / 4u);
  PH_HIP(hipMemsetAsync(ws.counter, 0, 512, stream));
  a.seg = a.order ? (a.nq + 7u) / 8u : 0u;
  hipLaunchKernelGGL(fn, dim3(grid), dim3(64), lds_bytes(k.capc, k.pq_lds) + (size_t)vis_slots * 4u, stream, a);
  PH_HIP(hipGetLastError());
  if (mark_end) {
    PH_HIP(hipEventRecord(ws.ev1, stream));
    ws.timed = true;
  }
  return 0;
}
```

### parallel_hnsw_amd/csrc/search_kernels.h

```cpp
#pragma once
#include <hip/hip_runtime.h>

#include <algorithm>
#include <cstdio>
#include <cstdlib>
#include <cstring>

#include "phnsw_internal.h"

#include "phnsw_device.h"

#ifdef PH_HOP_PROFILE
#define PH_TICK(k)                                   \
  {                                                  \
    asm volatile("s_waitcnt vmcnt(0) lgkmcnt(0)");   \
    const uint64_t t_now = wall_clock64();           \
    tprof[k] += t_now - t_last;                      \
    t_last = t_now;                                  \
  }
#else
#define PH_TICK(k)
#endif

template <bool BIG>
__device__ __forceinline__ void queue_sync() {
  if constexpr (BIG) __threadfence();
  __syncthreads();
}

__host__ __device__ constexpr bool vis_lds_shape(int capc, int nv) {
  return capc == 2 || (capc == 4 && nv != 1) || (capc == 8 && nv == 6);
}
template <int CAPC, class D, class = void>
struct vis_lds_policy : std::false_type {};
template <int CAPC, class D>
struct vis_lds_policy<CAPC, D, std::enable_if_t<D::ROW_STORE>>
    : std::integral_constant<bool, D::ROWS_IN_FLIGHT != 0 && vis_lds_shape(CAPC, D::CHUNKS)> {};

__device__ __forceinline__ uint32_t vis_slot(uint32_t id, uint32_t slots) {
  return (uint32_t)(((uint64_t)(id * 0x9E3779B1u) * slots) >> 32);
}

__device__ __forceinline__ bool vis_insert(uint32_t *H, uint32_t slots, uint32_t id, bool valid) {
  bool fresh = false, pending = valid;
  uint32_t s = valid ? vis_slot(id, slots) : 0u;
  while (__ballot(pending)) {
    if (pending) {
      const uint32_t old = atomicCAS(&H[s], PH_EMPTY32, id);
      if (old == PH_EMPTY32 || old == id) {
        fresh = old == PH_EMPTY32;
        pending = false;
      } else {
        s = s + 1u == slots ? 0u : s + 1u;
      }
    }
  }
  return fresh;
}

template <int CAPC, class Dist, bool INSTR = false, bool BIG = false, bool FILT = false>
__device__ __forceinline__ void ph_search_body(const PhSearchArgs &a) {
  extern __shared__ uint32_t smem[];
  constexpr int CAP = CAPC * 64;
  uint32_t *Cid = smem;
  float *Cd = (float *)(smem + CAP);
  uint32_t *Qid = smem + 2 * CAP;
  float *Qd = (float *)(smem + 3 * CAP);
  if constexpr (BIG) {
    Qid = a.big_q + (uint64_t)blockIdx.x * 2u * a.cap_max;
    Qd = (float *)(Qid + a.cap_max);
  }
  uint32_t *S = smem + 4 * CAP;
  float *dist_lds = (float *)(smem + 5 * CAP + 64);
  if (Dist::GLOBAL_TABLE) dist_lds = (float *)((char *)a.pq_tables + (size_t)blockIdx.x * a.pq_table_bytes);
  const uint32_t T = (a.tiny_layers && a.tiny_member[a.tiny_n] == 0u) ? a.tiny_layers : 0u;
  const bool tiny_lds_row = a.tiny_n <= a.tiny_lds_nodes;
  float *Dl = (float *)(smem + 5 * CAP + 64);
  uint32_t *Vl = smem + 5 * CAP + 64 + (tiny_lds_row ? a.tiny_stride : 0u);
  const uint32_t tiny_words = (a.tiny_n + 31u) / 32u;

  const uint32_t lane = threadIdx.x;
  const uint64_t lt = lanemask_lt(lane);
  constexpr bool DENSE_ONLY = dist_is_none<Dist>::value;
  const bool table_ok = (a.dense_only || a.after_dense) ? a.dense_flag[0] == 0u : true;
  if (DENSE_ONLY && !table_ok) return;
  const uint32_t layer_lo = a.after_dense ? (table_ok ? a.after_dense : 0u) : a.layer_lo;
  uint32_t *vis = a.visited + (uint64_t)blockIdx.x * a.visited_words;
  uint2 *ovf = DENSE_ONLY ? a.dense_ovf + (uint64_t)blockIdx.x * a.dense_ovf_cap : a.ovf + (uint64_t)blockIdx.x * a.ovf_cap;
  const uint32_t ovf_cap = DENSE_ONLY ? a.dense_ovf_cap : a.ovf_cap;
  uint32_t *const Qs = S;
  uint32_t *const ovf_s = INSTR ? a.ovf_s + (uint64_t)blockIdx.x * a.ovf_cap : nullptr;
  uint32_t *const H = smem + a.vis_off;
  const uint32_t hslots = (BIG || INSTR || !vis_lds_policy<CAPC, Dist>::value) ? 0u : a.vis_slots;
  for (uint32_t i = lane; i < hslots; i += 64) H[i] = PH_EMPTY32;

  uint32_t seg_cur = 0, seg_done = 0;
  if (a.order) {
    uint32_t xcc;
    asm volatile("s_getreg_b32 %0, hwreg(HW_REG_XCC_ID)" : "=s"(xcc));
    seg_cur = (xcc & 15u) & 7u;
  }

  for (;;) {
    uint32_t q = 0, qpos = 0;
    if (!a.order) {
      if (lane == 0) q = atomicAdd(a.counter, 1u);
      q = rfl32(q);
      if (q >= a.nq) break;
      qpos = q;
    } else {
      for (;;) {
        uint32_t p = 0;
        if (lane == 0) p = atomicAdd(a.counter + seg_cur * 16u, 1u);
        p = rfl32(p);
        const uint32_t base = seg_cur * a.seg;
        const uint32_t len = base >= a.nq ? 0u : min(a.seg, a.nq - base);
        if (p < len) {
          qpos = base + p;
          q = a.order[qpos];
          break;
        }
        seg_cur = (seg_cur + 1u) & 7u;
        if (++seg_done == 8u) {
          q = PH_EMPTY32;
          break;
        }
      }
      if (q == PH_EMPTY32) break;
    }

    const uint32_t last_layer = a.n_layers - 1;
    const uint32_t layer_hi = a.layer_hi ? a.layer_hi : a.n_layers;
    if (layer_lo && a.status[q] != ST_OK) continue;
    const uint32_t qnode = (BIG && a.knn_nodes) ? a.knn_nodes[q] : a.first_node + q;
    uint32_t qvec = a.knn_mode ? a.layers[last_layer].nodes[qnode] : (a.qids ? a.qids[q] : 0u);
    uint64_t trow = qpos;
    if (a.tiny_rows) trow = (uint64_t)((a.tiny_row_map ? a.tiny_row_map[qvec] : qvec) - a.tiny_row_first);
    Dist dist;
    if (a.queries && !a.knn_mode)
      dist.prepare_raw(a.dist, a.queries + (uint64_t)q * a.ldq, dist_lds, lane);
    else
      dist.prepare_stored(a.dist, qvec, dist_lds, lane);
    const uint32_t excl = a.exclude ? a.exclude[q] : PH_EMPTY32;
    const uint32_t *const allow = FILT ? a.filter + (uint64_t)q * a.filter_stride : nullptr;
    uint32_t n_dist = 0, n_hops = 0, err = ST_OK;
    uint32_t index_distance = 0xFFFFFFFFu;
    uint32_t n_tab = 0;
    uint32_t n_dist0 = 0, n_hops0 = 0;
    uint32_t clen = 0;
    uint32_t ef = a.ef;
    bool big_written = false;

    if (layer_lo) {
      clen = a.out_len[q];
#pragma unroll
      for (int c = 0; c < CAPC; c++) {
        uint32_t i = lane + 64u * c;
        if (i < clen) {
          Cid[i] = a.out_ids[(uint64_t)q * a.ef + i];
          Cd[i] = a.out_d[(uint64_t)q * a.ef + i];
        }
      }
      if (a.out_stats) {
        n_dist = a.out_stats[2 * (uint64_t)q];
        n_hops = a.out_stats[2 * (uint64_t)q + 1];
      }
      n_dist0 = n_dist;
      n_hops0 = n_hops;
    } else if (!a.knn_mode) {
      uint32_t entry = a.layers[0].nodes[0];
      float d0;
      if constexpr (DENSE_ONLY) {
        const PhLayerDev TLy = a.layers[a.tiny_layers - 1];
        const uint32_t tid = TLy.vec2node ? TLy.vec2node[entry] : entry;
        d0 = (a.tiny_d + trow * a.tiny_stride)[tid < a.tiny_n ? tid : 0u];
      } else {
        d0 = dist.batch(a.dist, 1ull, entry, lane);
      }
      d0 = __uint_as_float(rl32(__float_as_uint(d0), 0));
      n_dist = 1;
      if (lane == 0) {
        Cid[0] = entry;
        Cd[0] = d0;
      }
      clen = 1;
    }
    const float *Dg = a.tiny_d + trow * a.tiny_stride;
    if (T) {
      if (tiny_lds_row)
        for (uint32_t i = lane; i < a.tiny_n; i += 64) Dl[i] = Dg[i];
      for (uint32_t i = lane; i < tiny_words; i += 64) Vl[i] = 0u;
    }
    queue_sync<BIG>();

    for (uint32_t li = a.knn_mode ? last_layer : layer_lo; li < layer_hi && err == ST_OK; li++) {
      PhLayerDev L = a.layers[li];
      const bool tl = li < T;
      if (tl) {
        const PhLayerDev TLy = a.layers[T - 1];
        L.n_nodes = a.tiny_n;
        L.nodes = TLy.nodes;
        L.vec2node = TLy.vec2node;
        L.neighbors = a.tiny_nbr + a.tiny_off[li];
      }
      const bool identity = L.vec2node == nullptr;
      bool hv = hslots && !tl;
      uint32_t hn = 0;
      auto visit = [&](uint32_t id, bool valid) -> bool {
        if (hv && hn + (uint32_t)__popcll(__ballot(valid)) > a.vis_limit) {
          for (uint32_t i = lane; i < hslots; i += 64) {
            const uint32_t o = H[i];
            if (o != PH_EMPTY32) {
              atomicOr(&vis[o >> 5], 1u << (o & 31));
              H[i] = PH_EMPTY32;
            }
          }
          wait_vm0();
          hv = false;
        }
        if (hv) {
          const bool f = vis_insert(H, hslots, id, valid);
          hn += (uint32_t)__popcll(__ballot(f));
          return f;
        }
        if (!valid) return false;
        const uint32_t bit = 1u << (id & 31);
        return !(atomicOr(&vis[id >> 5], bit) & bit);
      };
      uint32_t qlen;
      if (a.knn_mode) {
        if (lane == 0) {
          Qid[0] = qnode;
          Qd[0] = 0.0f;
        }
        visit(qnode, lane == 0);
        qlen = 1;
      } else {
        bool miss = false;
#pragma unroll
        for (int c = 0; c < CAPC; c++) {
          uint32_t i = lane + 64u * c;
          if (i < clen) {
            uint32_t vid = Cid[i];
            uint32_t nid = identity ? vid : L.vec2node[vid];
            if (nid >= L.n_nodes || (tl && !((a.tiny_member[nid] >> li) & 1u))) {
              miss = true;
              nid = 0;
            }
            Qid[i] = nid;
            Qd[i] = Cd[i];
          }
        }
        if (__ballot(miss)) {
          err = ST_MISSING;
          break;
        }
#pragma unroll
        for (int c = 0; c < CAPC; c++) {
          uint32_t i = lane + 64u * c;
          if (tl) {
            if (i < clen) atomicOr(&Vl[Qid[i] >> 5], 1u << (Qid[i] & 31));
          } else if (64u * c < clen) {
            visit(i < clen ? Qid[i] : 0u, i < clen);
          }
        }
        qlen = clen;
      }
      queue_sync<BIG>();

      float thr_last = 0.0f;
      uint32_t thr_last_size = 0;
      for (;;) {
      if (a.knn_mode == 2) {
        if (!(thr_last < a.threshold && qlen > thr_last_size)) break;
        thr_last_size = qlen;
        if (thr_last_size > 1 || n_hops > 0) {
#pragma unroll
          for (int c = 0; c < (BIG ? (int)((qlen + 63u) >> 6) : CAPC); c++) {
            uint32_t i = lane + 64u * c;
            uint32_t nid = 0;
            if (i < qlen) {
              nid = Qid[i] & IDM;
              Qid[i] = nid;
            }
            if (64u * c < qlen) visit(nid, i < qlen);
          }
          queue_sync<BIG>();
        }
      }
      uint32_t ovf_n = 0;
      uint32_t pd = a.probe_depth;
      uint32_t highest = 0;
      if constexpr (INSTR) {
#pragma unroll
        for (int c = 0; c < CAPC; c++)
          if (lane + 64u * c < qlen) Qs[lane + 64u * c] = 0u;
        queue_sync<BIG>();
      }
      uint32_t scan_from = 0;
#ifdef PH_CELL_PROBE
      const bool probing = a.probe_pos && li == last_layer && !tl;
      uint32_t probe_p0 = 0, probe_cnt[11] = {0, 0, 0, 0, 0, 0, 0, 0, 0, 0, 0};
      if (probing) probe_p0 = a.probe_pos[Qid[0] & IDM];
#endif
#ifdef PH_HOP_PROFILE
      uint64_t tprof[8] = {0, 0, 0, 0, 0, 0, 0, 0};
      uint64_t t_last = wall_clock64();
      const uint32_t hops_before = n_hops, dist_before = n_dist;
#endif
      for (;;) {
        int pop = -1;
        uint32_t cur = 0;
        for (uint32_t c = scan_from >> 6; 64u * c < qlen; c++) {
          const uint32_t i = lane + 64u * c;
          const uint32_t e = i < qlen ? Qid[i] : EXPF;
          const uint64_t b = __ballot(!(e & EXPF));
          if (b) {
            const int pl = __builtin_ctzll(b);
            pop = (int)(64u * c) + pl;
            cur = rl32(e, pl);
            break;
          }
        }
        if (pop >= 0) {
          if (lane == 0) Qid[pop] = cur | EXPF;
          if constexpr (BIG) __threadfence();
        } else {
          if (ovf_n == 0) break;
          wait_vm0();
          uint64_t best = KEY_NONE;
          uint32_t bi = 0;
          for (uint32_t i = lane; i < ovf_n; i += 64) {
            uint32_t id = __hip_atomic_load(&ovf[i].x, __ATOMIC_RELAXED, __HIP_MEMORY_SCOPE_AGENT);
            if (!(id & EXPF)) {
              uint32_t db = __hip_atomic_load(&ovf[i].y, __ATOMIC_RELAXED, __HIP_MEMORY_SCOPE_AGENT);
              uint64_t k = mkkey(__uint_as_float(db), id);
              if (k < best) {
                best = k;
                bi = i;
              }
            }
          }
#pragma unroll
          for (int s = 32; s >= 1; s >>= 1) {
            uint64_t o = ((uint64_t)__shfl_xor((uint32_t)(best >> 32), s) << 32) | __shfl_xor((uint32_t)best, s);
            uint32_t oi = __shfl_xor(bi, s);
            if (o < best) {
              best = o;
              bi = oi;
            }
          }
          if (best == KEY_NONE) break;
          cur = (uint32_t)best & IDM;
          if (lane == 0)
            __hip_atomic_store(&ovf[bi].x, cur | EXPF, __ATOMIC_RELAXED, __HIP_MEMORY_SCOPE_AGENT);
          pop = -1 - (int)bi;
        }
        uint32_t cur_s = 0;
        if constexpr (INSTR) cur_s = pop >= 0 ? Qs[pop] : ovf_s[(uint32_t)(-1 - pop)];
        cur &= IDM;
        n_hops++;
        PH_TICK(0)

        uint32_t nb = PH_EMPTY32;
        if (lane < L.W) nb = L.neighbors[(uint64_t)cur * L.W + lane];
        if constexpr (Dist::EARLY) {
          const bool valid = nb < L.n_nodes;
          uint32_t v = 0;
          if (valid) v = identity ? nb : L.nodes[nb];
          dist.prefetch(a.dist, valid, v, lane);
        }
        PH_TICK(1)
        bool fresh = false;
        if (tl) {
          if (nb < L.n_nodes) {
            uint32_t bit = 1u << (nb & 31);
            fresh = !(atomicOr(&Vl[nb >> 5], bit) & bit);
          }
        } else {
          fresh = visit(nb, nb < L.n_nodes);
        }
        const uint64_t fm = __ballot(fresh);
        const uint32_t m = __popcll(fm);
        n_dist += m;
        if (tl) n_tab += m;
#ifdef PH_CELL_PROBE
        if (probing) {
          uint32_t dd = 0xFFFFFFFFu;
          if (fresh) {
            const int d0 = (int)a.probe_pos[nb] - (int)probe_p0;
            dd = (uint32_t)(d0 < 0 ? -d0 : d0);
          }
#pragma unroll
          for (int k = 0; k < 10; k++) probe_cnt[k] += __popcll(__ballot(fresh && dd <= (k ? (1u << (k - 1)) : 0u)));
          probe_cnt[10] += m;
        }
#endif
        PH_TICK(2)

        float myd;
        if (tl) {
          myd = 0.f;
          if (fresh) myd = tiny_lds_row ? Dl[nb] : Dg[nb];
        } else if constexpr (Dist::EARLY) {
          myd = dist.finish(a.dist, fm, lane);
        } else {
          uint32_t vid = 0;
          if (fresh) vid = identity ? nb : L.nodes[nb];
          myd = dist.batch(a.dist, fm, vid, lane);
        }

        PH_TICK(3)
        const uint64_t key = fresh ? mkkey(myd, nb) : KEY_NONE;
        uint32_t my_s = 0;
        if constexpr (INSTR) {
          uint32_t rank_all = 0;
          uint64_t remf = fm;
          while (remf) {
            const int j = __builtin_ctzll(remf);
            remf &= remf - 1;
            rank_all += (rl64(key, j) < key) ? 1u : 0u;
          }
          my_s = cur_s + rank_all + 1u;
        }
        const bool full = qlen == ef;
        const float dtail = full ? Qd[ef - 1] : PH_FMAX;
        const uint64_t tailkey = full ? mkkey(dtail, Qid[ef - 1]) : KEY_NONE;
        const bool ins = fresh && key < tailkey && myd <= PH_FMAX;
        const uint64_t im = __ballot(ins);
        uint32_t pos = 0, pos_min = 0xFFFFFFFFu, newpos = 0xFFFFFFFFu;
        bool did = im != 0;
        if (!im && m >= 2) did = __ballot(fresh && myd == dtail) != 0;
        if (im) {
          uint32_t rank = 0, greater = 0;
          bool first_pass = true;
          const int c_top = (int)((qlen - 1u) >> 6);
          int c = c_top, c_low;
          for (;;) {
            const bool two = c > 0;
            const uint32_t i1 = lane + 64u * (uint32_t)c, i0 = i1 - 64u;
            const bool has1 = i1 < qlen;
            const uint32_t qi1 = has1 ? Qid[i1] : PH_EMPTY32;
            const float qd1 = has1 ? Qd[i1] : PH_FMAX;
            const uint64_t qk1 = has1 ? mkkey(qd1, qi1) : KEY_NONE;
            uint32_t qi0 = PH_EMPTY32;
            float qd0 = PH_FMAX;
            if (two) {
              qi0 = Qid[i0];
              qd0 = Qd[i0];
            }
            const uint64_t qk0 = two ? mkkey(qd0, qi0) : KEY_NONE;
            uint32_t qs1 = 0, qs0 = 0;
            if constexpr (INSTR) {
              qs1 = has1 ? Qs[i1] : 0u;
              qs0 = two ? Qs[i0] : 0u;
            }
            uint32_t sh1 = 0, sh0 = 0;
            uint64_t rem = im;
            if (first_pass) {
              while (rem) {
                const int j = __builtin_ctzll(rem);
                rem &= rem - 1;
                const uint64_t kj = rl64(key, j);
                rank += (kj < key) ? 1u : 0u;
                const bool g1 = kj < qk1, g0 = two && kj < qk0;
                sh1 += g1 ? 1u : 0u;
                sh0 += g0 ? 1u : 0u;
                const uint32_t g = (uint32_t)__popcll(__ballot(g1)) + (uint32_t)__popcll(__ballot(g0));
                greater += lane == (uint32_t)j ? g : 0u;
              }
              first_pass = false;
            } else {
              while (rem) {
                const int j = __builtin_ctzll(rem);
                rem &= rem - 1;
                const uint64_t kj = rl64(key, j);
                const bool g1 = kj < qk1, g0 = two && kj < qk0;
                sh1 += g1 ? 1u : 0u;
                sh0 += g0 ? 1u : 0u;
                const uint32_t g = (uint32_t)__popcll(__ballot(g1)) + (uint32_t)__popcll(__ballot(g0));
                greater += lane == (uint32_t)j ? g : 0u;
              }
            }
            __builtin_amdgcn_fence(__ATOMIC_ACQ_REL, "wavefront");
            if constexpr (BIG) wait_vm0();
            const uint32_t np1 = i1 + sh1, np0 = i0 + sh0;
            if (has1 && np1 < ef) {
              Qid[np1] = qi1;
              Qd[np1] = qd1;
              if constexpr (INSTR) Qs[np1] = qs1;
            }
            if (two && np0 < ef) {
              Qid[np0] = qi0;
              Qd[np0] = qd0;
              if constexpr (INSTR) Qs[np0] = qs0;
            }
            if (qlen + 64u > ef) {
              const bool spill1 = has1 && np1 >= ef;
              const uint64_t sm1 = __ballot(spill1);
              if (sm1) {
                const uint32_t at = ovf_n + __popcll(sm1 & lt);
                if (spill1 && at < ovf_cap) ovf[at] = make_uint2(qi1, __float_as_uint(qd1));
                if constexpr (INSTR)
                  if (spill1 && at < ovf_cap) ovf_s[at] = qs1;
                ovf_n += __popcll(sm1);
              }
              const bool spill0 = two && np0 >= ef;
              const uint64_t sm0 = __ballot(spill0);
              if (sm0) {
                const uint32_t at = ovf_n + __popcll(sm0 & lt);
                if (spill0 && at < ovf_cap) ovf[at] = make_uint2(qi0, __float_as_uint(qd0));
                if constexpr (INSTR)
                  if (spill0 && at < ovf_cap) ovf_s[at] = qs0;
                ovf_n += __popcll(sm0);
              }
            }
            c_low = two ? c - 1 : c;
            if (c_low == 0 || rl32(two ? sh0 : sh1, 0) == 0u) break;
            c -= 2;
          }
          pos = 64u * (uint32_t)(c_top + 1) - greater;
          if (ins) newpos = pos + rank;
          pos_min = rl32(pos, __builtin_ctzll(__ballot(ins && rank == 0u)));
          PH_TICK(5)
          queue_sync<BIG>();
          PH_TICK(6)
        }
        {
          if (fresh && newpos < ef) {
            Qid[newpos] = nb;
            Qd[newpos] = myd;
            if constexpr (INSTR) Qs[newpos] = my_s;
          }
          bool spill = fresh && newpos >= ef;
          uint64_t sm = __ballot(spill);
          if (sm) {
            uint32_t at = ovf_n + __popcll(sm & lt);
            if (spill && at < ovf_cap) ovf[at] = make_uint2(nb, __float_as_uint(myd));
            if constexpr (INSTR)
              if (spill && at < ovf_cap) ovf_s[at] = my_s;
            ovf_n += __popcll(sm);
          }
          if constexpr (INSTR)
            if (__ballot(fresh && newpos == 0u)) highest = cur_s;
        }
        qlen = min(ef, qlen + (uint32_t)__popcll(im));
        scan_from = min(pop >= 0 ? (uint32_t)pop + 1u : scan_from, pos_min);
        queue_sync<BIG>();
        PH_TICK(4)
        if (ovf_n > ovf_cap) {
          err = ST_OVERFLOW;
          break;
        }
        if (!did) {
          pd -= 1;
          if (pd == 0) break;
        }
      }
      if (err != ST_OK) break;
      if constexpr (INSTR) index_distance = highest;
#ifdef PH_CELL_PROBE
      if (probing && lane == 0) {
        for (int k = 0; k < 11; k++) atomicAdd(&a.probe_out[k], (unsigned long long)probe_cnt[k]);
        atomicAdd(&a.probe_out[11], 1ull);
      }
#endif
#ifdef PH_HOP_PROFILE
      if (lane == 0 && q == 0)
        printf("hop profile q0 layer %u%s: hops %u evals %u | us: pop %.1f nbr %.1f visited %.1f dist %.1f merge %.1f (+ search/rank %.1f, shift %.1f)\n", li,
               tl ? " (dense)" : "", n_hops - hops_before, n_dist - dist_before, tprof[0] * 0.01, tprof[1] * 0.01, tprof[2] * 0.01,
               tprof[3] * 0.01, tprof[4] * 0.01, tprof[5] * 0.01, tprof[6] * 0.01);
#endif

#ifdef PH_VISITED_PROBE
      if (!tl && lane == 0) {
        const uint32_t k = li == last_layer ? 1u : 0u;
        atomicAdd(&a.vprobe_out[k * 64u + min((qlen + ovf_n) >> 6, 63u)], 1ull);
        if (!hv && hslots) atomicAdd(&a.vprobe_out[128u + k], 1ull);
      }
#endif
      if (tl) {
        for (uint32_t i = lane; i < tiny_words; i += 64) Vl[i] = 0u;
      } else if (hv) {
        for (uint32_t i = lane; i < hslots; i += 64) H[i] = PH_EMPTY32;
      } else {
#pragma unroll
        for (int c = 0; c < (BIG ? (int)((qlen + 63u) >> 6) : CAPC); c++) {
          uint32_t i = lane + 64u * c;
          if (i < qlen) vis[(Qid[i] & IDM) >> 5] = 0u;
        }
        if (ovf_n) {
          wait_vm0();
          for (uint32_t i = lane; i < ovf_n; i += 64) {
            uint32_t id = __hip_atomic_load(&ovf[i].x, __ATOMIC_RELAXED, __HIP_MEMORY_SCOPE_AGENT) & IDM;
            vis[id >> 5] = 0u;
          }
        }
      }
      wait_vm0();
      hv = hslots && !tl;
      hn = 0;
      if (a.knn_mode != 2) break;
      thr_last = Qd[qlen - 1];
      if (thr_last < a.threshold && qlen == ef) {
        if (ef * 2 > (BIG ? a.cap_max : (uint32_t)CAP)) {
          err = ST_CAPACITY;
          break;
        }
        ef *= 2;
      }
      }
      if (err != ST_OK) break;

      if constexpr (BIG) {
        const uint32_t os = a.out_stride ? a.out_stride : a.ef;
        uint32_t kept = 0;
        for (uint32_t base = 0; base < qlen && kept < os; base += 64) {
          const uint32_t i = base + lane;
          const bool has = i < qlen;
          const uint32_t nid = has ? (Qid[i] & IDM) : 0u;
          const uint32_t v = has ? (identity ? nid : L.nodes[nid]) : PH_EMPTY32;
          const bool keep = has && v != excl;
          const uint64_t km = __ballot(keep);
          const uint32_t at = kept + __popcll(km & lt);
          if (keep && at < os) {
            a.out_ids[(uint64_t)q * os + at] = v;
            a.out_d[(uint64_t)q * os + at] = Qd[i];
          }
          kept += __popcll(km);
        }
        clen = min(kept, os);
        for (uint32_t i = clen + lane; i < os; i += 64) {
          a.out_ids[(uint64_t)q * os + i] = PH_EMPTY32;
          a.out_d[(uint64_t)q * os + i] = PH_FMAX;
        }
        big_written = true;
        continue;
      }
      const uint32_t candidate_count = (a.n_layers == 1 || li == last_layer) ? ef : a.upper;
      uint32_t bv[CAPC];
      float bd[CAPC];
      uint32_t bpos[CAPC];
      uint32_t kept = 0;
#pragma unroll
      for (int c = 0; c < CAPC; c++) {
        uint32_t i = lane + 64u * c;
        bool has = i < qlen;
        uint32_t nid = has ? (Qid[i] & IDM) : 0u;
        bd[c] = has ? Qd[i] : PH_FMAX;
        bv[c] = has ? (identity ? nid : L.nodes[nid]) : PH_EMPTY32;
        bool keep = has && bv[c] != excl;
        if constexpr (FILT)
          if (keep) keep = (allow[bv[c] >> 5] >> (bv[c] & 31)) & 1u;
        uint64_t km = __ballot(keep);
        uint32_t at = kept + __popcll(km & lt);
        bpos[c] = (keep && at < candidate_count) ? at : PH_EMPTY32;
        kept += __popcll(km);
      }
      const uint32_t blen = min(kept, candidate_count);
      queue_sync<BIG>();
#pragma unroll
      for (int c = 0; c < CAPC; c++) {
        if (bpos[c] != PH_EMPTY32) {
          Qid[bpos[c]] = bv[c];
          Qd[bpos[c]] = bd[c];
        }
      }
      queue_sync<BIG>();

      uint32_t ci[CAPC];
      float cd[CAPC];
      uint32_t cpos[CAPC];
      uint32_t dups = 0;
#pragma unroll
      for (int c = 0; c < CAPC; c++) {
        uint32_t i = lane + 64u * c;
        bool has = i < clen;
        ci[c] = has ? Cid[i] : PH_EMPTY32;
        cd[c] = has ? Cd[i] : PH_FMAX;
        bool dup = false;
        uint32_t lb = 0;
        if (has) {
          uint64_t k = mkkey(cd[c], ci[c]);
          lb = lds_lower_bound(Qid, Qd, blen, k);
          dup = lb < blen && mkkey(Qd[lb], Qid[lb]) == k;
        }
        uint64_t dm = __ballot(dup);
        uint32_t pre = dups + __popcll(dm & lt);
        S[i] = pre;
        cpos[c] = (has && !dup) ? (i - pre) + lb : PH_EMPTY32;
        dups += __popcll(dm);
      }
      if (lane == 0) S[CAP] = dups;
      queue_sync<BIG>();
#pragma unroll
      for (int c = 0; c < CAPC; c++) {
        uint32_t j = lane + 64u * c;
        bool has = j < blen;
        bv[c] = has ? Qid[j] : PH_EMPTY32;
        bd[c] = has ? Qd[j] : PH_FMAX;
        bpos[c] = PH_EMPTY32;
        if (has) {
          uint32_t la = lds_lower_bound(Cid, Cd, clen, mkkey(bd[c], bv[c]));
          uint32_t dupb = la < clen ? S[la] : S[CAP];
          if (la == clen) dupb = dups;
          bpos[c] = j + (la - dupb);
        }
      }
      queue_sync<BIG>();
#pragma unroll
      for (int c = 0; c < CAPC; c++) {
        if (cpos[c] < ef) {
          Cid[cpos[c]] = ci[c];
          Cd[cpos[c]] = cd[c];
        }
        if (bpos[c] < ef) {
          Cid[bpos[c]] = bv[c];
          Cd[bpos[c]] = bd[c];
        }
      }
      clen = min(ef, clen - dups + blen);
      queue_sync<BIG>();
    }

    if (err != ST_OK) {
      if (!DENSE_ONLY)
        for (uint64_t w = lane; w < a.visited_words; w += 64) vis[w] = 0u;
      for (uint32_t i = lane; i < hslots; i += 64) H[i] = PH_EMPTY32;
      wait_vm0();
      clen = 0;
    }
    if (FILT && (a.filter_flags & PHNSW_FILTER_STRICT) && layer_hi == a.n_layers && !big_written) {
      uint32_t sv[CAPC];
      float sd[CAPC];
      uint32_t spos[CAPC];
      uint32_t kept = 0;
#pragma unroll
      for (int c = 0; c < CAPC; c++) {
        const uint32_t i = lane + 64u * c;
        const bool has = i < clen;
        sv[c] = has ? Cid[i] : 0u;
        sd[c] = has ? Cd[i] : PH_FMAX;
        bool keep = false;
        if (has) keep = (allow[sv[c] >> 5] >> (sv[c] & 31)) & 1u;
        const uint64_t km = __ballot(keep);
        spos[c] = keep ? kept + __popcll(km & lt) : PH_EMPTY32;
        kept += __popcll(km);
      }
      queue_sync<BIG>();
#pragma unroll
      for (int c = 0; c < CAPC; c++) {
        if (spos[c] != PH_EMPTY32) {
          Cid[spos[c]] = sv[c];
          Cd[spos[c]] = sd[c];
        }
      }
      clen = kept;
      queue_sync<BIG>();
    }
    const uint32_t ostride = a.out_stride ? a.out_stride : a.ef;
    for (uint32_t i = lane; i < ostride && !big_written; i += 64) {
      a.out_ids[(uint64_t)q * ostride + i] = i < clen ? Cid[i] : PH_EMPTY32;
      a.out_d[(uint64_t)q * ostride + i] = i < clen ? Cd[i] : PH_FMAX;
    }
    if (a.out_hit) {
      uint32_t cut = clen;
      if (a.hit_eps > 0.f) {
#pragma unroll
        for (int c = 0; c < CAPC; c++) {
          uint32_t i = lane + 64u * c;
          bool far = i < clen && !(fabsf(Cd[i]) < a.hit_eps);
          uint64_t fmk = __ballot(far);
          if (fmk && cut == clen) cut = 64u * c + __builtin_ctzll(fmk);
        }
      }
      bool hit = false;
#pragma unroll
      for (int c = 0; c < CAPC; c++) {
        uint32_t i = lane + 64u * c;
        hit |= (i < cut && Cid[i] == qvec);
      }
      uint64_t hm = __ballot(hit);
      if (lane == 0) a.out_hit[q] = hm ? 1u : 0u;
    }
    if (a.out_key && lane == 0) {
      uint32_t key = PH_EMPTY32;
      if (clen) {
        const PhLayerDev KL = a.layers[layer_hi - 1];
        uint32_t nid = KL.vec2node ? KL.vec2node[Cid[0]] : Cid[0];
        if (nid < KL.n_nodes) key = a.key_pos ? a.key_pos[nid] : nid;
      }
      a.out_key[q] = key;
    }
    if (lane == 0 && a.totals) {
      atomicAdd(&a.totals[0], (unsigned long long)(n_dist - n_dist0));
      atomicAdd(&a.totals[1], (unsigned long long)(n_hops - n_hops0));
    }
    if (lane == 0 && a.launch_totals) {
      atomicAdd(&a.launch_totals[0], (unsigned long long)(n_dist - n_dist0));
      atomicAdd(&a.launch_totals[1], (unsigned long long)(n_hops - n_hops0));
      if (a.launch_tab && n_tab) atomicAdd(a.launch_tab, (unsigned long long)n_tab);
    }
    if constexpr (INSTR)
      if (lane == 0) a.out_index[q] = index_distance;
    if (lane == 0) {
      a.out_len[q] = clen;
      a.status[q] = err;
      if (a.out_stats) {
        a.out_stats[2 * (uint64_t)q] = n_dist;
        a.out_stats[2 * (uint64_t)q + 1] = n_hops;
      }
    }
    queue_sync<BIG>();
  }
}

template <int CAPC, class Dist, bool FILT = false>
__global__ __launch_bounds__(64) void ph_search_kernel(PhSearchArgs a) {
  ph_search_body<CAPC, Dist, false, false, FILT>(a);
}

template <int CAPC, bool FILT = false>
__global__ __launch_bounds__(64) void ph_search_kernel_dense(PhSearchArgs a) {
  ph_search_body<CAPC, DistNone, false, false, FILT>(a);
}

template <int CAPC, int NV, bool FILT = false>
__global__ __launch_bounds__(64, 1) void ph_search_kernel_lat(PhSearchArgs a) {
  ph_search_body<CAPC, DistF32<NV, 0>, false, false, FILT>(a);
}

template <int CAPC, int NV>
__global__ __launch_bounds__(64) void ph_search_kernel_instr(PhSearchArgs a) {
  ph_search_body<CAPC, DistF32<NV>, true>(a);
}

template <class Dist>
__global__ __launch_bounds__(64) void ph_search_kernel_big(PhSearchArgs a) {
  ph_search_body<2, Dist, false, true>(a);
}

template <int CAPC, int M, bool FILT = false>
__global__ __launch_bounds__(64, 2) void ph_search_kernel_pqr(PhSearchArgs a) {
  ph_search_body<CAPC, DistPQR<M>, false, false, FILT>(a);
}


typedef void (*ph_search_fn)(PhSearchArgs);

enum PhKernelFamily {
  PH_KF_ROWS_F32,
  PH_KF_ROWS_F16,
  PH_KF_ROWS_I8,
  PH_KF_ROWS_I8Q,
  PH_KF_PQ_TABLE,
  PH_KF_PQ_REG,
  PH_KF_PQ_SHARED,
  PH_KF_LATENCY,
  PH_KF_INSTR,
};

template <bool FILT>
static ph_search_fn pick_kernel_pqr(int capc, int m) {
#define PH_KR(C, M) \
  if (capc == C && m == M) return (ph_search_fn)ph_search_kernel_pqr<C, M, FILT>;
  PH_KR(2, 32) PH_KR(2, 64) PH_KR(2, 96) PH_KR(2, 128)
  PH_KR(8, 32) PH_KR(8, 64) PH_KR(8, 96) PH_KR(8, 128)
#undef PH_KR
  return nullptr;
}

template <bool FILT>
static ph_search_fn pick_kernel_pqs(int capc, int nv) {
#define PH_KS(C, N) \
  if (capc == C && nv == N) return (ph_search_fn)ph_search_kernel<C, DistPQS<N>, FILT>;
  PH_KS(2, 1) PH_KS(2, 3) PH_KS(2, 6) PH_KS(8, 1) PH_KS(8, 3) PH_KS(8, 6) PH_KS(16, 1) PH_KS(16, 3) PH_KS(16, 6)
#undef PH_KS
  return nullptr;
}

template <bool FILT>
static ph_search_fn pick_kernel_dense(int capc) {
  switch (capc) {
    case 2: return (ph_search_fn)ph_search_kernel_dense<2, FILT>;
    case 4: return (ph_search_fn)ph_search_kernel_dense<4, FILT>;
    case 8: return (ph_search_fn)ph_search_kernel_dense<8, FILT>;
    case 16: return (ph_search_fn)ph_search_kernel_dense<16, FILT>;
  }
  return nullptr;
}

template <bool FILT>
static ph_search_fn pick_kernel_lat(int capc, int nv) {
#define PH_KL(C, N) \
  if (capc == C && nv == N) return (ph_search_fn)ph_search_kernel_lat<C, N, FILT>;
  PH_KL(2, 1) PH_KL(2, 3) PH_KL(8, 1) PH_KL(8, 3)
#undef PH_KL
  return nullptr;
}

template <template <int, int> class D, bool FILT>
static ph_search_fn pick_kernel_rows(int capc, int nv) {
#define PH_K(C, N) \
  if (capc == C && nv == N) return (ph_search_fn)ph_search_kernel<C, D<N, 4>, FILT>;
  PH_K(2, 1) PH_K(2, 3) PH_K(2, 6)
  if (capc == 4 && nv == 3) return (ph_search_fn)ph_search_kernel<4, D<3, 8>, FILT>;
  PH_K(4, 6)
  PH_K(8, 1) PH_K(8, 3) PH_K(8, 6)
  PH_K(16, 1) PH_K(16, 3) PH_K(16, 6)
#undef PH_K
  return nullptr;
}

template <bool FILT>
static ph_search_fn pick_kernel_pqt(int capc, bool global) {
#define PH_KQ(C) \
  if (capc == C) return global ? (ph_search_fn)ph_search_kernel<C, DistPQG, FILT> : (ph_search_fn)ph_search_kernel<C, DistPQ, FILT>;
  PH_KQ(2) PH_KQ(8) PH_KQ(16)
#undef PH_KQ
  return nullptr;
}

template <bool FILT>
static ph_search_fn pick_kernel_family(int family, int capc, int nv, int pqr_m, bool pq_global) {
  switch (family) {
    case PH_KF_ROWS_F32: return pick_kernel_rows<DistF32, FILT>(capc, nv);
    case PH_KF_ROWS_F16: return pick_kernel_rows<DistF16, FILT>(capc, nv);
    case PH_KF_ROWS_I8: return pick_kernel_rows<DistI8, FILT>(capc, nv);
    case PH_KF_ROWS_I8Q: return pick_kernel_rows<DistI8Q, FILT>(capc, nv);
    case PH_KF_PQ_TABLE: return pick_kernel_pqt<FILT>(capc, pq_global);
    case PH_KF_PQ_REG: return pick_kernel_pqr<FILT>(capc, pqr_m);
    case PH_KF_PQ_SHARED: return pick_kernel_pqs<FILT>(capc, nv);
    case PH_KF_LATENCY: return pick_kernel_lat<FILT>(capc, nv);
    default: return nullptr;
  }
}

ph_search_fn ph_pick_filtered_kernel(int family, int capc, int nv, int pqr_m, bool pq_global);
ph_search_fn ph_pick_filtered_dense(int capc);
```

### parallel_hnsw_amd/csrc/tiny.hip

```cpp
#include <hip/hip_runtime.h>

#include <algorithm>
#include <cstdlib>
#include <cstring>

#include "phnsw_device.h"

struct PhTinyPrepArgs {
  PhLayerDev layers[PH_TINY_MAX_LAYERS];
  uint32_t T, tiny_n;
  uint32_t off[PH_TINY_MAX_LAYERS];
  uint32_t *nbr;
  uint32_t *member;
};

__global__ void ph_tiny_prep_kernel(PhTinyPrepArgs p) {
  const uint32_t l = blockIdx.y;
  const PhLayerDev L = p.layers[l], TL = p.layers[p.T - 1];
  for (uint32_t i = blockIdx.x * blockDim.x + threadIdx.x; i < L.n_nodes; i += gridDim.x * blockDim.x) {
    const uint32_t vid = L.nodes[i];
    const uint32_t t = TL.vec2node ? TL.vec2node[vid] : vid;
    if (t >= p.tiny_n) {
      p.member[p.tiny_n] = 1u;
      continue;
    }
    atomicOr(&p.member[t], 1u << l);
    for (uint32_t k = 0; k < L.W; k++) {
      const uint32_t nb = L.neighbors[(uint64_t)i * L.W + k];
      uint32_t tn = PH_EMPTY32;
      if (nb < L.n_nodes) {
        const uint32_t v2 = L.nodes[nb];
        tn = TL.vec2node ? TL.vec2node[v2] : v2;
        if (tn >= p.tiny_n) {
          p.member[p.tiny_n] = 1u;
          tn = PH_EMPTY32;
        }
      }
      p.nbr[p.off[l] + (uint64_t)t * L.W + k] = tn;
    }
  }
}

struct PhTinyTableArgs {
  PhDistArgs dist;
  const float *queries;
  uint32_t ldq;
  const uint32_t *qids;
  const uint32_t *order;
  uint32_t npos;
  const uint32_t *tnodes;
  uint32_t tiny_n, stride;
  float *D;
  uint32_t rows_per_slice;
  uint32_t dbg;
};

template <int M>
__device__ __forceinline__ float fold2(float A, float B, uint32_t lane) {
#ifdef PH_FOLD_GENERIC
  const bool hi = (lane & M) != 0;
  const float own = hi ? B : A, other = hi ? A : B;
  return own + __shfl_xor(other, M);
#else
  if constexpr (M == 32) {
    auto r = __builtin_amdgcn_permlane32_swap(__float_as_uint(A), __float_as_uint(B), false, false);
    return __uint_as_float(r[0]) + __uint_as_float(r[1]);
  } else if constexpr (M == 16) {
    auto r = __builtin_amdgcn_permlane16_swap(__float_as_uint(A), __float_as_uint(B), false, false);
    return __uint_as_float(r[0]) + __uint_as_float(r[1]);
  } else {
    const bool hi = (lane & M) != 0;
    const float own = hi ? B : A, other = hi ? A : B;
    const int o = (int)__float_as_uint(other);
    int t;
    if constexpr (M == 8) {
      t = __builtin_amdgcn_update_dpp(0, o, 0x128, 0xF, 0xF, true);
    } else if constexpr (M == 4) {
      t = __builtin_amdgcn_update_dpp(o, o, 0x114, 0xF, 0xA, false);
      t = __builtin_amdgcn_update_dpp(t, o, 0x104, 0xF, 0x5, false);
    } else if constexpr (M == 2) {
      t = __builtin_amdgcn_update_dpp(0, o, 0x4E, 0xF, 0xF, true);
    } else {
      t = __builtin_amdgcn_update_dpp(0, o, 0xB1, 0xF, 0xF, true);
    }
    return own + __uint_as_float((uint32_t)t);
  }
#endif
}

template <int NV, int QT, bool EXACT, bool L2>
__device__ __forceinline__ void tiny_tile(const float4 *lds, const ph_f2 (&qv)[QT / 2][NV][4], uint32_t nv4, uint32_t lane,
                                          float &V) {
  float R[8];
#pragma unroll
  for (int i = 0; i < 8; i++) {
    float4 x[NV];
#pragma unroll
    for (int k = 0; k < NV; k++) x[k] = lds[(i * NV + k) * 64 + lane];
    float p[QT];
    ph_f2 pp[QT / 2];
    chain_partial2<NV, QT / 2, EXACT, L2>(x, qv, nv4, lane, pp);
#pragma unroll
    for (int j = 0; j < QT / 2; j++) {
      p[2 * j] = pp[j].x;
      p[2 * j + 1] = pp[j].y;
    }
    if constexpr (QT == 8) {
      float f0 = fold2<32>(p[0], p[1], lane), f1 = fold2<32>(p[2], p[3], lane);
      float f2 = fold2<32>(p[4], p[5], lane), f3 = fold2<32>(p[6], p[7], lane);
      float g0 = fold2<16>(f0, f1, lane), g1 = fold2<16>(f2, f3, lane);
      R[i] = fold2<8>(g0, g1, lane);
    } else {
      float f0 = fold2<32>(p[0], p[1], lane), f1 = fold2<32>(p[2], p[3], lane);
      R[i] = fold2<16>(f0, f1, lane);
    }
  }
  constexpr int M0 = QT == 8 ? 4 : 8;
  float h0 = fold2<M0>(R[0], R[1], lane), h1 = fold2<M0>(R[2], R[3], lane);
  float h2 = fold2<M0>(R[4], R[5], lane), h3 = fold2<M0>(R[6], R[7], lane);
  float e0 = fold2<M0 / 2>(h0, h1, lane), e1 = fold2<M0 / 2>(h2, h3, lane);
  V = fold2<M0 / 4>(e0, e1, lane);
  if constexpr (QT == 4) V += __shfl_xor(V, 1);
}

template <int NV, int QT, class R = RowF32>
__global__ __launch_bounds__(256) void ph_tiny_table_kernel(PhTinyTableArgs a) {
  __shared__ float4 rows_lds[8 * NV * 64];
  const uint32_t lane = threadIdx.x & 63u, w = threadIdx.x >> 6;
  const uint32_t nv4 = a.dist.nv4;
  const uint32_t p0 = (blockIdx.x * 4u + w) * QT;
  ph_f2 qv[QT / 2][NV][4];
#pragma unroll
  for (int j = 0; j < QT; j++) {
    const uint32_t p = p0 + j;
    const bool valid = p < a.npos;
    const uint32_t q = valid ? (a.order ? a.order[p] : p) : 0u;
    const float4 *src = nullptr;
    const typename R::chunk *srcs = nullptr;
    typename R::aux sax = typename R::aux();
    if (valid) {
      if (a.queries)
        src = (const float4 *)(a.queries + (uint64_t)q * a.ldq);
      else {
        srcs = R::row(a.dist.rows, a.qids[q]);
        sax = R::row_aux(srcs);
      }
    }
#pragma unroll
    for (int k = 0; k < NV; k++) {
      const uint32_t c = lane + 64u * k;
      const float4 v = (valid && c < nv4) ? (src ? src[c] : R::widen(R::load(srcs, c), sax)) : make_float4(0.f, 0.f, 0.f, 0.f);
      qv[j / 2][k][0][j & 1] = v.x;
      qv[j / 2][k][1][j & 1] = v.y;
      qv[j / 2][k][2][j & 1] = v.z;
      qv[j / 2][k][3][j & 1] = v.w;
    }
  }
  const bool exact = nv4 == 64u * NV, l2 = a.dist.metric == PHNSW_METRIC_L2;
  const uint32_t r_begin = blockIdx.y * a.rows_per_slice;
  const uint32_t r_end = min(a.tiny_n, r_begin + a.rows_per_slice);
  for (uint32_t r0 = r_begin; r0 < r_end; r0 += 8) {
    __syncthreads();
    if (!(a.dbg & 2u) || r0 == r_begin)
#pragma unroll
    for (int u = 0; u < 2; u++) {
      const uint32_t slot = 2u * w + u;
      const uint32_t rr = min(r0 + slot, a.tiny_n - 1u);
      const typename R::chunk *src = R::row(a.dist.rows, a.tnodes[rr]);
      const typename R::aux ax = R::row_aux(src);
#pragma unroll
      for (int k = 0; k < NV; k++) {
        uint32_t c = lane + 64u * k;
        c = c < nv4 ? c : nv4 - 1u;
        rows_lds[(slot * NV + k) * 64 + lane] = R::widen(R::load(src, c), ax);
      }
    }
    __syncthreads();
    float V;
    if (exact) {
      if (l2)
        tiny_tile<NV, QT, true, true>(rows_lds, qv, nv4, lane, V);
      else
        tiny_tile<NV, QT, true, false>(rows_lds, qv, nv4, lane, V);
    } else {
      if (l2)
        tiny_tile<NV, QT, false, true>(rows_lds, qv, nv4, lane, V);
      else
        tiny_tile<NV, QT, false, false>(rows_lds, qv, nv4, lane, V);
    }
    uint32_t j, i;
    bool writer = true;
    if (QT == 8) {
      j = ((lane >> 5) & 1u) | (((lane >> 4) & 1u) << 1) | (((lane >> 3) & 1u) << 2);
      i = ((lane >> 2) & 1u) | (((lane >> 1) & 1u) << 1) | ((lane & 1u) << 2);
    } else {
      j = ((lane >> 5) & 1u) | (((lane >> 4) & 1u) << 1);
      i = ((lane >> 3) & 1u) | (((lane >> 2) & 1u) << 1) | (((lane >> 1) & 1u) << 2);
      writer = (lane & 1u) == 0u;
    }
    const uint32_t p = p0 + j, r = r0 + i;
    if (writer && p < a.npos && r < r_end && !(a.dbg & 1u)) a.D[(uint64_t)p * a.stride + r] = finalize_metric(V, a.dist.metric);
  }
}

typedef float ph_f32x32 __attribute__((ext_vector_type(32)));

__host__ __device__ constexpr uint32_t ph_rev5(uint32_t t) {
  return ((t & 1u) << 4) | ((t & 2u) << 2) | (t & 4u) | ((t & 8u) >> 2) | ((t & 16u) >> 4);
}

struct PhTinyPackArgs {
  PhRows rows;
  const float *queries;
  uint32_t ldq;
  const uint32_t *ids;
  const uint32_t *order;
  uint32_t n, n_pad;
  uint32_t nv;
  float4 *out;
};

template <class R>
__device__ __forceinline__ float4 tiny_pack_stored(const PhRows &rows, uint32_t vid, uint32_t c) {
  const typename R::chunk *src = R::row(rows, vid);
  return R::widen(R::load(src, c), R::row_aux(src));
}
__global__ void ph_tiny_pack_kernel(PhTinyPackArgs p) {
  const uint32_t r = blockIdx.x * 32u + threadIdx.x;
  const uint32_t c = blockIdx.y * 8u + threadIdx.y;
  float4 v = make_float4(0.f, 0.f, 0.f, 0.f);
  if (r < p.n) {
    const uint32_t e = p.order ? p.order[r] : r;
    if (p.queries) {
      v = ((const float4 *)(p.queries + (uint64_t)e * p.ldq))[c];
    } else {
      switch (p.rows.kind) {
        case PH_ROWS_F16: v = tiny_pack_stored<RowF16>(p.rows, p.ids[e], c); break;
        case PH_ROWS_I8: v = tiny_pack_stored<RowI8>(p.rows, p.ids[e], c); break;
        default: v = tiny_pack_stored<RowF32>(p.rows, p.ids[e], c); break;
      }
    }
  }
  const uint32_t t = ph_rev5(c & 31u), b = (c >> 5) & 1u, k = c >> 6;
  p.out[(((((uint64_t)(r >> 5) * 32u + t) * p.nv + k) * 2u + b) << 5) + (r & 31u)] = v;
}

struct PhTinyMfmaArgs {
  const float4 *pq, *pn;
  uint32_t npos, tiny_n, stride;
  uint32_t qtiles, ntiles;
  int metric;
  float *D;
};

template <int NV, int G>
struct PhMfmaTile {
  static constexpr int TILE4 = G * NV * 64;
  static constexpr int BUF4 = 4 * TILE4;
  static constexpr int NG = 32 / G;
  float4 *sm4;
  const float4 *mysrc;
  const float4 *A0, *B0;
  float4 *mydst;
  float4 stage[G * NV];

  __device__ __forceinline__ void fetch(int g) {
#pragma unroll
    for (int i = 0; i < G * NV; i++) stage[i] = mysrc[g * TILE4 + i * 64];
  }
  __device__ __forceinline__ void park(int buf) {
#pragma unroll
    for (int i = 0; i < G * NV; i++) mydst[buf * BUF4 + i * 64] = stage[i];
  }
  template <int T>
  __device__ __forceinline__ void leaf(float (&out)[16]) {
    constexpr int g = T / G, tt = T % G;
    if (tt == 0 && g + 1 < NG) fetch(g + 1);
    ph_f32x32 acc;
#pragma unroll
    for (int v = 0; v < 32; v++) acc[v] = 0.f;
#pragma unroll
    for (int k = 0; k < NV; k++) {
      const float4 qa = A0[(g & 1) * BUF4 + (tt * NV + k) * 64];
      const float4 xb = B0[(g & 1) * BUF4 + (tt * NV + k) * 64];
      acc = __builtin_amdgcn_mfma_f32_32x32x1f32(qa.x, xb.x, acc, 0, 0, 0);
      acc = __builtin_amdgcn_mfma_f32_32x32x1f32(qa.y, xb.y, acc, 0, 0, 0);
      acc = __builtin_amdgcn_mfma_f32_32x32x1f32(qa.z, xb.z, acc, 0, 0, 0);
      acc = __builtin_amdgcn_mfma_f32_32x32x1f32(qa.w, xb.w, acc, 0, 0, 0);
    }
#pragma unroll
    for (int v = 0; v < 16; v++) {
      out[v] = acc[v] + acc[v + 16];
      asm volatile("" : "+v"(out[v]));
    }
    if (tt == G - 1) {
      if (g + 1 < NG) park((g + 1) & 1);
      __syncthreads();
    }
  }
  template <int L, int T0>
  __device__ __forceinline__ void subtree(float (&out)[16]) {
    if constexpr (L == 0) {
      leaf<T0>(out);
    } else {
      float lo[16], hi[16];
      subtree<L - 1, T0>(lo);
      subtree<L - 1, T0 + (1 << (L - 1))>(hi);
#pragma unroll
      for (int v = 0; v < 16; v++) {
        out[v] = lo[v] + hi[v];
        asm volatile("" : "+v"(out[v]));
      }
    }
  }
};

template <int NV, int G>
__global__ __launch_bounds__(256, G == 1 ? 4 : 1) void ph_tiny_table_mfma_kernel(PhTinyMfmaArgs a) {
  extern __shared__ float4 sm4[];
  using Tile = PhMfmaTile<NV, G>;
  const uint32_t tid = threadIdx.x, lane = tid & 63u, w = tid >> 6;
  const uint32_t B = blockIdx.x, xcd = B & 7u, slot = B >> 3;
  const uint32_t sq = (a.qtiles + 7u) / 8u;
  const uint32_t super = (slot >> 6) * 8u + xcd, within = slot & 63u;
  const uint32_t qt = (super % sq) * 8u + (within & 7u), nt = (super / sq) * 8u + (within >> 3);
  if (qt >= a.qtiles || nt >= a.ntiles) return;
  Tile t;
  t.sm4 = sm4;
  t.mysrc = (w < 2u ? a.pq + (uint64_t)(2u * qt + w) * (32u * NV * 64u)
                    : a.pn + (uint64_t)(2u * nt + (w - 2u)) * (32u * NV * 64u)) + lane;
  t.mydst = sm4 + w * Tile::TILE4 + lane;
  t.A0 = sm4 + (w & 1u) * Tile::TILE4 + lane;
  t.B0 = sm4 + (2u + (w >> 1)) * Tile::TILE4 + lane;
  t.fetch(0);
  t.park(0);
  __syncthreads();
  float V[16];
  t.template subtree<5, 0>(V);
  const uint32_t r = (2u * nt + (w >> 1)) * 32u + (lane & 31u);
#pragma unroll
  for (int v = 0; v < 16; v++) {
    const uint32_t p = (2u * qt + (w & 1u)) * 32u + 8u * (v / 4) + 4u * (lane >> 5) + (v & 3);
    if (p < a.npos && r < a.tiny_n) a.D[(uint64_t)p * a.stride + r] = finalize_metric(V[v], a.metric);
  }
}

#define PH_I8T_KS 128u
#define PH_I8T_ROW (PH_I8T_KS + 16u)
#define PH_I8T_LDS (2u * 64u * PH_I8T_ROW)

struct PhTinyQuantArgs {
  PhRows rows;
  const float *queries;
  uint32_t ldq, nv4;
  const uint32_t *ids;
  const uint32_t *order;
  uint32_t n, n_pad;
  uint32_t kw;
  uint32_t *codes;
  float *scales;
};

__global__ __launch_bounds__(256) void ph_tiny_quant_kernel(PhTinyQuantArgs p) {
  const uint32_t lane = threadIdx.x & 63u, r = blockIdx.x * 4u + (threadIdx.x >> 6);
  if (r >= p.n_pad) return;
  uint32_t *dst = p.codes + (uint64_t)r * p.kw;
  float scale = 0.f;
  if (r >= p.n) {
    for (uint32_t c = lane; c < p.kw; c += 64u) dst[c] = 0u;
  } else {
    const uint32_t e = p.order ? p.order[r] : r;
    if (p.queries) {
      const float4 *q = (const float4 *)(p.queries + (uint64_t)e * p.ldq);
      float m = 0.f;
      for (uint32_t c = lane; c < p.nv4; c += 64u) m = ph_maxabs4(m, q[c]);
      scale = ph_i8_scale(wave_max(m));
      for (uint32_t c = lane; c < p.kw; c += 64u) dst[c] = c < p.nv4 ? ph_i8_quant4(q[c], scale) : 0u;
    } else {
      const uint32_t *row = RowI8::row(p.rows, p.ids[e]);
      scale = RowI8::row_aux(row);
      for (uint32_t c = lane; c < p.kw; c += 64u) dst[c] = c < p.nv4 ? RowI8::load(row, c) : 0u;
    }
  }
  if (lane == 0) p.scales[r] = scale;
}

typedef int ph_i32x4 __attribute__((ext_vector_type(4)));
typedef int ph_i32x16 __attribute__((ext_vector_type(16)));

struct PhTinyI8Args {
  const ph_i32x4 *cq, *cn;
  const float *sq, *sn;
  uint32_t npos, tiny_n, stride;
  uint32_t k16;
  int metric;
  float *D;
};

__global__ __launch_bounds__(256, 4) void ph_tiny_table_i8_kernel(PhTinyI8Args a) {
  __shared__ ph_i32x4 sm[PH_I8T_LDS / 16u];
  constexpr uint32_t ROW16 = PH_I8T_ROW / 16u, KS16 = PH_I8T_KS / 16u;
  const uint32_t tid = threadIdx.x, lane = tid & 63u, w = tid >> 6;
  const uint32_t qt = blockIdx.x, nt = blockIdx.y;
  const uint32_t srow = tid / KS16, scol = tid % KS16;
  const ph_i32x4 *gq = a.cq + ((uint64_t)qt * 64u + srow) * a.k16 + scol;
  const ph_i32x4 *gn = a.cn + ((uint64_t)nt * 64u + srow) * a.k16 + scol;
  ph_i32x4 *lq = sm + srow * ROW16 + scol, *ln = sm + (64u + srow) * ROW16 + scol;
  const ph_i32x4 *A = sm + ((w & 1u) * 32u + (lane & 31u)) * ROW16 + (lane >> 5);
  const ph_i32x4 *B = sm + (64u + (w >> 1) * 32u + (lane & 31u)) * ROW16 + (lane >> 5);
  ph_i32x16 acc;
#pragma unroll
  for (int v = 0; v < 16; v++) acc[v] = 0;
  const uint64_t half = (uint64_t)32u * a.k16;
  ph_i32x4 q0 = gq[0], q1 = gq[half], n0 = gn[0], n1 = gn[half];
  const uint32_t steps = a.k16 / KS16;
  for (uint32_t s = 0; s < steps; s++) {
    __syncthreads();
    lq[0] = q0;
    lq[32u * ROW16] = q1;
    ln[0] = n0;
    ln[32u * ROW16] = n1;
    __syncthreads();
    if (s + 1u < steps) {
      const uint32_t o = (s + 1u) * KS16;
      q0 = gq[o];
      q1 = gq[half + o];
      n0 = gn[o];
      n1 = gn[half + o];
    }
#pragma unroll
    for (uint32_t j = 0; j < KS16 / 2u; j++) acc = __builtin_amdgcn_mfma_i32_32x32x32_i8(A[2u * j], B[2u * j], acc, 0, 0, 0);
  }
  const uint32_t r = (2u * nt + (w >> 1)) * 32u + (lane & 31u);
  const float sr = a.sn[r];
#pragma unroll
  for (int v = 0; v < 16; v++) {
    const uint32_t p = (2u * qt + (w & 1u)) * 32u + 8u * (v / 4) + 4u * (lane >> 5) + (v & 3);
    if (p < a.npos && r < a.tiny_n) a.D[(uint64_t)p * a.stride + r] = ph_i8q_distance(a.sq[p], sr, acc[v], a.metric);
  }
}


void ph_tiny_free(PhWorkspace &ws) {
  ws.tiny_prep_key = PhTinyPrepKey();
  ws.tiny_pack_key = PhTinyPackKey();
  if (ws.tiny_d) hipFree(ws.tiny_d);
  if (ws.tiny_nbr) hipFree(ws.tiny_nbr);
  if (ws.tiny_member) hipFree(ws.tiny_member);
  if (ws.tiny_pq) hipFree(ws.tiny_pq);
  if (ws.tiny_pn) hipFree(ws.tiny_pn);
  ws.tiny_pq = ws.tiny_pn = nullptr;
  ws.tiny_pq_bytes = ws.tiny_pn_bytes = 0;
  ws.tiny_d = nullptr;
  ws.tiny_nbr = ws.tiny_member = nullptr;
  ws.tiny_d_bytes = ws.tiny_nbr_bytes = ws.tiny_member_bytes = 0;
}

static bool tiny_mfma_shape(int metric, uint32_t ld) {
  return metric != PHNSW_METRIC_L2 && (ld == 256u || ld == 768u || ld == 1536u) && !getenv("PHNSW_TINY_VALU");
}

static int table_beside_mode() {
  const char *e = getenv("PHNSW_TABLE_BESIDE");
  if (!e || !strcmp(e, "auto")) return 2;
  return atoi(e) > 0 ? 1 : 0;
}
static bool tiny_keep_off() { return getenv("PHNSW_NO_TINY_KEEP") != nullptr; }
static size_t tiny_mfma_lds(int nv, int g) { return (size_t)2 * 4 * g * nv * 64 * sizeof(float4); }

bool ph_tiny_matrix_cores(const phnsw_index *ix) {
  return ix->store->kind == PH_ROWS_I8Q || tiny_mfma_shape(ix->store->metric, ix->store->ld);
}

uint32_t ph_tiny_layer_count(const phnsw_index *ix, uint32_t n_layers, uint32_t ef) {
  const bool off = getenv("PHNSW_NO_TINY") != nullptr;
  if (off || (!ph_store_f32(ix->store) && !ph_store_converted(ix->store)) || !ph_chunk_count(ix->store->ld / 4)) return 0;
  const uint64_t per_ef = ph_tiny_matrix_cores(ix) ? 80ull : 48ull;
  uint64_t cap = std::min<uint64_t>(PH_TINY_MAX_NODES, per_ef * ef);
  if (const char *e = getenv("PHNSW_TINY_MAX"))
    if (atoi(e) > 0) cap = std::min<uint64_t>(PH_TINY_MAX_NODES, (uint64_t)atoi(e));
  uint32_t T = 0;
  while (T < n_layers && T < PH_TINY_MAX_LAYERS && ix->layers[T].n_nodes <= cap) T++;
  return T;
}

static uint32_t tiny_stride_of(uint32_t n) { return (n + 63u) / 64u * 64u; }

uint64_t ph_tiny_max_positions(const phnsw_index *ix, uint32_t n_layers, uint32_t ef) {
  uint32_t T = ph_tiny_layer_count(ix, n_layers, ef);
  if (!T) return 0;
  uint64_t budget = 4ull << 30;
  if (const char *e = getenv("PHNSW_TINY_TABLE_BYTES"))
    if (atoll(e) > 0) budget = (uint64_t)atoll(e);
  return std::max<uint64_t>(64, budget / ((uint64_t)tiny_stride_of(ix->layers[T - 1].n_nodes) * 4u));
}

size_t ph_tiny_beside_lds(const phnsw_index *ix, const PhSearchArgs &a) {
  if (!a.tiny_layers || a.tiny_rows || !table_beside_mode()) return 0;
  if (ix->store->kind == PH_ROWS_I8Q) return PH_I8T_LDS;
  const uint32_t nv4 = a.dist.nv4;
  if (!tiny_mfma_shape(ix->store->metric, nv4 * 4u)) return 0;
  return tiny_mfma_lds((int)(nv4 / 64u), 1);
}

size_t ph_tiny_lds_bytes(const PhSearchArgs &a) {
  if (!a.tiny_layers) return 0;
  return (a.tiny_n <= a.tiny_lds_nodes ? (size_t)a.tiny_stride * 4u : 0u) + (size_t)((a.tiny_n + 31u) / 32u + 1u) * 4u;
}

template <class T>
static hipError_t grow(T **p, size_t *have, size_t need) {
  if (*have >= need) return hipSuccess;
  if (*p) ph_timed_free(*p);
  *p = nullptr;
  *have = 0;
  hipError_t e = ph_timed_malloc((void **)p, need);
  if (e == hipSuccess) *have = need;
  return e;
}

static bool same_key(const PhTinyPrepKey &a, const PhTinyPrepKey &b) {
  if (!a.valid || !b.valid || a.nodes_epoch != b.nodes_epoch || a.T != b.T || a.tn != b.tn || a.vec2node != b.vec2node) return false;
  for (uint32_t l = 0; l < a.T; l++)
    if (a.nodes[l] != b.nodes[l] || a.nbrs[l] != b.nbrs[l] || a.n[l] != b.n[l] || a.W[l] != b.W[l] || a.links[l] != b.links[l])
      return false;
  return true;
}

static int tiny_prep_graph(const phnsw_index *ix, PhWorkspace &ws, PhSearchArgs &a, uint32_t T, uint32_t tn, hipStream_t stream,
                           bool *kept = nullptr) {
  if (kept) *kept = false;
  PhTinyPrepArgs p;
  memset(&p, 0, sizeof(p));
  p.T = T;
  p.tiny_n = tn;
  PhTinyPrepKey key;
  key.valid = !tiny_keep_off();
  key.nodes_epoch = ix->nodes_epoch;
  key.T = T;
  key.tn = tn;
  key.vec2node = a.layers[T - 1].vec2node;
  size_t nbr_words = 0;
  for (uint32_t l = 0; l < T; l++) {
    p.layers[l] = a.layers[l];
    p.off[l] = (uint32_t)nbr_words;
    a.tiny_off[l] = (uint32_t)nbr_words;
    nbr_words += (size_t)tn * a.layers[l].W;
    key.nodes[l] = a.layers[l].nodes;
    key.nbrs[l] = a.layers[l].neighbors;
    key.n[l] = a.layers[l].n_nodes;
    key.W[l] = a.layers[l].W;
    key.links[l] = ix->layers[l].links_epoch;
  }
  const uint32_t *nbr_was = ws.tiny_nbr, *member_was = ws.tiny_member;
  if (grow(&ws.tiny_nbr, &ws.tiny_nbr_bytes, nbr_words * 4u) != hipSuccess ||
      grow(&ws.tiny_member, &ws.tiny_member_bytes, (size_t)(PH_TINY_MAX_NODES + 1u) * 4u) != hipSuccess) {
    (void)hipGetLastError();
    ws.tiny_prep_key.valid = false;
    return 1;
  }
  if (ws.tiny_nbr == nbr_was && ws.tiny_member == member_was && same_key(key, ws.tiny_prep_key)) {
    if (kept) *kept = true;
    return 0;
  }
  ws.tiny_prep_key = key;
  p.nbr = ws.tiny_nbr;
  p.member = ws.tiny_member;
  PH_HIP(hipMemsetAsync(ws.tiny_nbr, 0xFF, nbr_words * 4u, stream));
  PH_HIP(hipMemsetAsync(ws.tiny_member, 0, (size_t)(tn + 1u) * 4u, stream));
  hipLaunchKernelGGL(ph_tiny_prep_kernel, dim3((tn + 255u) / 256u, T), dim3(256), 0, stream, p);
  PH_HIP(hipGetLastError());
  return 0;
}

template <class R>
static void tiny_table_valu(int nv, dim3 grid, hipStream_t stream, const PhTinyTableArgs &t) {
  switch (nv) {
    case 1: hipLaunchKernelGGL((ph_tiny_table_kernel<1, 8, R>), grid, dim3(256), 0, stream, t); break;
    case 3: hipLaunchKernelGGL((ph_tiny_table_kernel<3, 8, R>), grid, dim3(256), 0, stream, t); break;
    default: hipLaunchKernelGGL((ph_tiny_table_kernel<6, 4, R>), grid, dim3(256), 0, stream, t); break;
  }
}

static int tiny_table_i8q(const phnsw_index *ix, PhWorkspace &ws, const PhDistArgs &dist, const float *queries, uint32_t ldq,
                          const uint32_t *qids, const uint32_t *order, uint32_t npos, const uint32_t *tnodes, uint32_t tn,
                          uint32_t stride, float *D, hipStream_t stream, bool *kept) {
  const uint32_t qtiles = (npos + 63u) / 64u, ntiles = (tn + 63u) / 64u;
  const uint32_t kpad = (dist.ld + PH_I8T_KS - 1u) / PH_I8T_KS * PH_I8T_KS;
  const size_t row_bytes = (size_t)kpad + 4u;
  const float4 *pn_was = ws.tiny_pn;
  if (grow(&ws.tiny_pq, &ws.tiny_pq_bytes, (size_t)qtiles * 64u * row_bytes) != hipSuccess ||
      grow(&ws.tiny_pn, &ws.tiny_pn_bytes, (size_t)ntiles * 64u * row_bytes) != hipSuccess) {
    (void)hipGetLastError();
    ws.tiny_pack_key.valid = false;
    return 1;
  }
  PhTinyPackKey key;
  key.valid = !tiny_keep_off();
  key.nodes_epoch = ix->nodes_epoch;
  key.vecs = dist.rows.base;
  key.tnodes = tnodes;
  key.ld = dist.ld;
  key.tn = tn;
  key.nv = kpad;
  const PhTinyPackKey &have = ws.tiny_pack_key;
  const bool pn_kept = ws.tiny_pn == pn_was && key.valid && have.valid && have.nodes_epoch == key.nodes_epoch &&
                       have.vecs == key.vecs && have.tnodes == key.tnodes && have.ld == key.ld && have.tn == key.tn &&
                       have.nv == key.nv;
  ws.tiny_pack_key = key;
  if (kept) *kept = pn_kept;
  PhTinyQuantArgs k;
  memset(&k, 0, sizeof(k));
  k.rows = dist.rows;
  k.nv4 = dist.nv4;
  k.kw = kpad / 4u;
  k.queries = queries;
  k.ldq = ldq;
  k.ids = qids;
  k.order = order;
  k.n = npos;
  k.n_pad = qtiles * 64u;
  k.codes = (uint32_t *)ws.tiny_pq;
  k.scales = (float *)((char *)ws.tiny_pq + (size_t)k.n_pad * kpad);
  hipLaunchKernelGGL(ph_tiny_quant_kernel, dim3(k.n_pad / 4u), dim3(256), 0, stream, k);
  PhTinyI8Args m;
  memset(&m, 0, sizeof(m));
  m.cq = (const ph_i32x4 *)k.codes;
  m.sq = k.scales;
  k.queries = nullptr;
  k.ids = tnodes;
  k.order = nullptr;
  k.n = tn;
  k.n_pad = ntiles * 64u;
  k.codes = (uint32_t *)ws.tiny_pn;
  k.scales = (float *)((char *)ws.tiny_pn + (size_t)k.n_pad * kpad);
  if (!pn_kept) hipLaunchKernelGGL(ph_tiny_quant_kernel, dim3(k.n_pad / 4u), dim3(256), 0, stream, k);
  PH_HIP(hipGetLastError());
  m.cn = (const ph_i32x4 *)k.codes;
  m.sn = k.scales;
  m.npos = npos;
  m.tiny_n = tn;
  m.stride = stride;
  m.k16 = kpad / 16u;
  m.metric = dist.metric;
  m.D = D;
  ws.tiny_table_g = 1;
  hipLaunchKernelGGL(ph_tiny_table_i8_kernel, dim3(qtiles, ntiles), dim3(256), 0, stream, m);
  PH_HIP(hipGetLastError());
  return 0;
}

static int tiny_table(const phnsw_index *ix, PhWorkspace &ws, const PhDistArgs &dist, const float *queries, uint32_t ldq,
                      const uint32_t *qids, const uint32_t *order, uint32_t npos, const uint32_t *tnodes, uint32_t tn,
                      uint32_t stride, float *D, hipStream_t stream, int g = 2, bool *kept = nullptr) {
  if (kept) *kept = false;
  ws.tiny_table_g = 0;
  PhTinyTableArgs t;
  memset(&t, 0, sizeof(t));
  t.dist = dist;
  t.queries = queries;
  t.ldq = ldq;
  t.qids = qids;
  t.order = order;
  t.npos = npos;
  t.tnodes = tnodes;
  t.tiny_n = tn;
  t.stride = stride;
  t.D = D;
  if (const char *e = getenv("PHNSW_TINY_DBG")) t.dbg = (uint32_t)atoi(e);
  const uint32_t nv4 = dist.nv4;
  const int nv = ph_chunk_count(nv4);
  if (dist.rows.kind == PH_ROWS_I8Q) return tiny_table_i8q(ix, ws, dist, queries, ldq, qids, order, npos, tnodes, tn, stride, D, stream, kept);
  const bool mfma = tiny_mfma_shape(dist.metric, nv4 * 4u) && nv4 == 64u * (uint32_t)nv && npos >= 32u;
  if (mfma) {
    const uint32_t qtiles = (npos + 63u) / 64u, ntiles = (tn + 63u) / 64u;
    const size_t row_bytes = (size_t)nv * 64u * sizeof(float4);
    const float4 *pn_was = ws.tiny_pn;
    if (grow(&ws.tiny_pq, &ws.tiny_pq_bytes, (size_t)qtiles * 64u * row_bytes) != hipSuccess ||
        grow(&ws.tiny_pn, &ws.tiny_pn_bytes, (size_t)ntiles * 64u * row_bytes) != hipSuccess) {
      (void)hipGetLastError();
      ws.tiny_pack_key.valid = false;
      return 1;
    }
    PhTinyPackKey key;
    key.valid = !tiny_keep_off();
    key.nodes_epoch = ix->nodes_epoch;
    key.vecs = dist.rows.base;
    key.tnodes = tnodes;
    key.ld = dist.ld;
    key.tn = tn;
    key.nv = (uint32_t)nv;
    const PhTinyPackKey &have = ws.tiny_pack_key;
    const bool pn_kept = ws.tiny_pn == pn_was && key.valid && have.valid && have.nodes_epoch == key.nodes_epoch &&
                         have.vecs == key.vecs && have.tnodes == key.tnodes && have.ld == key.ld && have.tn == key.tn &&
                         have.nv == key.nv;
    ws.tiny_pack_key = key;
    if (kept) *kept = pn_kept;
    PhTinyPackArgs k;
    memset(&k, 0, sizeof(k));
    k.rows = dist.rows;
    k.nv = (uint32_t)nv;
    k.queries = queries;
    k.ldq = ldq;
    k.ids = qids;
    k.order = order;
    k.n = npos;
    k.n_pad = qtiles * 64u;
    k.out = ws.tiny_pq;
    hipLaunchKernelGGL(ph_tiny_pack_kernel, dim3(k.n_pad / 32u, 8u * (uint32_t)nv), dim3(32, 8), 0, stream, k);
    k.queries = nullptr;
    k.ids = tnodes;
    k.order = nullptr;
    k.n = tn;
    k.n_pad = ntiles * 64u;
    k.out = ws.tiny_pn;
    if (!pn_kept) hipLaunchKernelGGL(ph_tiny_pack_kernel, dim3(k.n_pad / 32u, 8u * (uint32_t)nv), dim3(32, 8), 0, stream, k);
    PH_HIP(hipGetLastError());
    PhTinyMfmaArgs m;
    memset(&m, 0, sizeof(m));
    m.pq = ws.tiny_pq;
    m.pn = ws.tiny_pn;
    m.npos = npos;
    m.tiny_n = tn;
    m.stride = stride;
    m.qtiles = qtiles;
    m.ntiles = ntiles;
    m.metric = dist.metric;
    m.D = D;
    const uint32_t supers = ((qtiles + 7u) / 8u) * ((ntiles + 7u) / 8u);
    const uint32_t blocks = (supers + 7u) / 8u * 8u * 64u;
    const size_t lds = tiny_mfma_lds(nv, g == 1 ? 1 : 2);
    ws.tiny_table_g = g == 1 ? 1 : 2;
    if (g != 1 && nv == 6)
      PH_HIP(hipFuncSetAttribute((const void *)ph_tiny_table_mfma_kernel<6, 2>, hipFuncAttributeMaxDynamicSharedMemorySize, (int)lds));
#define PH_MFMA(NV, G) hipLaunchKernelGGL((ph_tiny_table_mfma_kernel<NV, G>), dim3(blocks), dim3(256), lds, stream, m)
    if (g == 1) {
      switch (nv) {
        case 1: PH_MFMA(1, 1); break;
        case 3: PH_MFMA(3, 1); break;
        default: PH_MFMA(6, 1); break;
      }
    } else {
      switch (nv) {
        case 1: PH_MFMA(1, 2); break;
        case 3: PH_MFMA(3, 2); break;
        default: PH_MFMA(6, 2); break;
      }
    }
#undef PH_MFMA
  } else {
    const uint32_t qt = nv == 6 ? 4u : 8u;
    const uint32_t gx = (npos + 4u * qt - 1u) / (4u * qt);
    const uint32_t tiles = (tn + 7u) / 8u;
    uint32_t slices = std::min<uint32_t>(tiles, std::max<uint32_t>(1u, (2048u + gx - 1u) / gx));
    t.rows_per_slice = (tiles + slices - 1u) / slices * 8u;
    slices = (tn + t.rows_per_slice - 1u) / t.rows_per_slice;
    dim3 grid(gx, slices);
    switch (dist.rows.kind) {
      case PH_ROWS_F16: tiny_table_valu<RowF16>(nv, grid, stream, t); break;
      case PH_ROWS_I8: tiny_table_valu<RowI8>(nv, grid, stream, t); break;
      default: tiny_table_valu<RowF32>(nv, grid, stream, t); break;
    }
  }
  PH_HIP(hipGetLastError());
  return 0;
}

int ph_tiny_prepare(const phnsw_index *ix, PhWorkspace &ws, PhSearchArgs &a, uint32_t max_layers, hipStream_t stream) {
  a.tiny_layers = 0;
  a.tiny_rows = 0;
  if (a.knn_mode || a.layer_lo) return 0;
  uint32_t T = std::min(ph_tiny_layer_count(ix, a.n_layers, a.ef), max_layers);
  if (!T) return 0;
  const uint32_t tn = ix->layers[T - 1].n_nodes, stride = tiny_stride_of(tn), npos = a.nq;
  if ((uint64_t)npos > ph_tiny_max_positions(ix, a.n_layers, a.ef)) return 0;
  if (grow(&ws.tiny_d, &ws.tiny_d_bytes, std::max<size_t>((size_t)npos * stride * 4u, 1u << 20)) != hipSuccess) {
    (void)hipGetLastError();
    return 0;
  }
  const int mode = table_beside_mode();
  bool beside = mode == 1;
  if (mode == 2) {
    const PhWorkspace &other = &ws == &ix->ws[0] ? ix->ws[1] : ix->ws[0];
    if ((&ws == &ix->ws[0] || &ws == &ix->ws[1]) && other.timed && other.ev1) {
      beside = hipEventQuery(other.ev1) == hipErrorNotReady;
      (void)hipGetLastError();
    }
  }
  bool prep_kept = false, pack_kept = false;
  int rc = tiny_prep_graph(ix, ws, a, T, tn, stream, &prep_kept);
  if (rc) return rc < 0 ? rc : 0;
  rc = tiny_table(ix, ws, a.dist, a.queries, a.ldq, a.qids, a.order, npos, a.layers[T - 1].nodes, tn, stride, ws.tiny_d, stream,
                  beside ? 1 : 2, &pack_kept);
  if (rc) return rc < 0 ? rc : 0;
  if (getenv("PHNSW_VERBOSE")) {
    if (ws.tiny_table_g)
      fprintf(stderr, "[phnsw] dense table: %u positions x %u nodes on the matrix cores, G = %d (%s), graph %s, node operand %s\n",
              npos, tn, ws.tiny_table_g, beside ? "beside the other workspace's launch" : "alone",
              prep_kept ? "kept" : "prepared", pack_kept ? "kept" : "packed");
    else
      fprintf(stderr, "[phnsw] dense table: %u positions x %u nodes on the vector units, graph %s\n", npos, tn,
              prep_kept ? "kept" : "prepared");
  }
  ws.tiny_last_npos = npos;
  ws.tiny_last_tn = tn;
  ws.tiny_last_stride = stride;
  a.tiny_layers = T;
  a.tiny_n = tn;
  a.tiny_lds_nodes = PH_TINY_LDS_NODES;
  a.tiny_stride = stride;
  a.tiny_d = ws.tiny_d;
  a.tiny_nbr = ws.tiny_nbr;
  a.tiny_member = ws.tiny_member;
  return 0;
}


void ph_build_table_free(phnsw_index *ix) {
  for (PhBuildTable &b : ix->bt)
    if (b.D) ph_timed_free(b.D);
  ix->bt.clear();
  for (auto &sp : ix->bt_spare) ph_timed_free(sp.first);
  ix->bt_spare.clear();
}
static void build_table_drop(phnsw_index *ix, PhBuildTable &b) {
  if (b.D) ix->bt_spare.emplace_back(b.D, b.cap);
  b.D = nullptr;
  b.bytes = b.cap = 0;
  b.lo = b.hi = b.lo_alloc = b.hi_alloc = 0;
}
static void build_table_recycle(phnsw_index *ix) {
  for (PhBuildTable &b : ix->bt) build_table_drop(ix, b);
  ix->bt.clear();
}
static float *build_table_buffer(phnsw_index *ix, size_t bytes, size_t *cap) {
  int best = -1;
  for (size_t i = 0; i < ix->bt_spare.size(); i++)
    if (ix->bt_spare[i].second >= bytes && ix->bt_spare[i].second <= 2 * bytes &&
        (best < 0 || ix->bt_spare[i].second < ix->bt_spare[(size_t)best].second))
      best = (int)i;
  if (best >= 0) {
    float *p = ix->bt_spare[(size_t)best].first;
    *cap = ix->bt_spare[(size_t)best].second;
    ix->bt_spare.erase(ix->bt_spare.begin() + best);
    return p;
  }
  size_t mfree = 0, mtotal = 0;
  if (hipMemGetInfo(&mfree, &mtotal) != hipSuccess) return nullptr;
  size_t want = bytes + bytes / 16;
  if (want + (8ull << 30) > mfree) {
    for (auto &sp : ix->bt_spare) ph_timed_free(sp.first);
    ix->bt_spare.clear();
    if (hipMemGetInfo(&mfree, &mtotal) != hipSuccess) return nullptr;
    want = bytes;
  }
  if (want + (8ull << 30) > mfree || bytes > mtotal / 2) return nullptr;
  float *p = nullptr;
  if (ph_timed_malloc((void **)&p, want) != hipSuccess) {
    (void)hipGetLastError();
    return nullptr;
  }
  *cap = want;
  return p;
}

static uint32_t build_table_min() {
  if (const char *e = getenv("PHNSW_BUILD_TABLE_MIN"))
    if (atoi(e) > 0) return (uint32_t)atoi(e);
  return 1024u;
}

int ph_build_table_prepare(phnsw_index *ix, PhWorkspace &ws, PhSearchArgs &a, const PhRowHint &h, uint32_t T,
                           hipStream_t stream, bool *used) {
  *used = false;
  a.tiny_rows = 0;
  if (!ix->bt_enabled || !T || !a.qids || a.queries || a.knn_mode || a.layer_lo || getenv("PHNSW_NO_BUILD_TABLE")) return 0;
  const uint32_t tn = ix->layers[T - 1].n_nodes, stride = tiny_stride_of(tn);
  const uint32_t *tnodes = a.layers[T - 1].nodes;
  if (tn < build_table_min() || h.qn == 0) return 0;
  if (!ix->bt.empty() && ix->bt[0].epoch != ix->nodes_epoch) build_table_recycle(ix);
  PhBuildTable *found = nullptr;
  for (PhBuildTable &b : ix->bt)
    if (b.qnodes == h.qnodes && b.qn == h.qn) found = &b;
  if (!found) {
    if (ix->bt.size() >= PH_MAX_LAYERS) return 0;
    ix->bt.emplace_back();
    found = &ix->bt.back();
    found->epoch = ix->nodes_epoch;
    found->qnodes = h.qnodes;
    found->qn = h.qn;
  }
  PhBuildTable &B = *found;
  const uint32_t need_lo = h.contiguous ? h.first : 0u, need_hi = h.contiguous ? h.first + h.count : h.qn;
  if (need_hi > h.qn || need_lo >= need_hi) return 0;
  const bool same = B.D && B.tnodes == tnodes && B.tn == tn && B.T == T;
  if (B.D && !same) build_table_drop(ix, B);
  if (!h.contiguous && !(B.D && B.lo <= need_lo && B.hi >= need_hi)) return 0;
  if (!B.D || need_lo < B.lo_alloc || need_hi > B.hi_alloc) {
    if (B.D && (need_lo > B.lo_alloc || need_hi < B.hi_alloc)) return 0;
    build_table_drop(ix, B);
    const size_t bytes = (size_t)(need_hi - need_lo) * stride * 4u;
    B.D = build_table_buffer(ix, bytes, &B.cap);
    if (!B.D) return 0;
    B.bytes = bytes;
    B.qnodes = h.qnodes;
    B.qn = h.qn;
    B.tnodes = tnodes;
    B.tn = tn;
    B.T = T;
    B.stride = stride;
    B.lo_alloc = need_lo;
    B.hi_alloc = need_hi;
    B.lo = B.hi = need_lo;
    B.epoch = ix->nodes_epoch;
  }
  auto fill = [&](uint32_t lo, uint32_t hi) -> int {
    const uint32_t PIECE = 131072u;
    for (uint32_t at = lo; at < hi; at += PIECE) {
      const uint32_t cnt = std::min(PIECE, hi - at);
      int rc = tiny_table(ix, ws, a.dist, nullptr, 0, h.qnodes + at, nullptr, cnt, tnodes, tn, stride,
                          B.D + (size_t)(at - B.lo_alloc) * stride, stream);
      if (rc) return rc;
    }
    return 0;
  };
  int rc = 0;
  if (B.lo == B.hi) {
    rc = fill(need_lo, need_hi);
    if (!rc) B.lo = need_lo, B.hi = need_hi;
  } else {
    if (need_lo < B.lo) {
      rc = fill(need_lo, B.lo);
      if (!rc) B.lo = need_lo;
    }
    if (!rc && need_hi > B.hi) {
      rc = fill(B.hi, need_hi);
      if (!rc) B.hi = need_hi;
    }
  }
  if (rc) return rc < 0 ? rc : 0;
  rc = tiny_prep_graph(ix, ws, a, T, tn, stream);
  if (rc) return rc < 0 ? rc : 0;
  a.tiny_layers = T;
  a.tiny_n = tn;
  a.tiny_lds_nodes = PH_TINY_LDS_NODES;
  a.tiny_stride = stride;
  a.tiny_d = B.D;
  a.tiny_rows = 1;
  a.tiny_row_first = B.lo_alloc;
  a.tiny_row_map = h.vec2node;
  a.tiny_nbr = ws.tiny_nbr;
  a.tiny_member = ws.tiny_member;
  *used = true;
  return 0;
}
```

Measured before the change: 1.049 million.

## Reorder dense table columns so upper-layer nodes come first and stage a window in LDS

After: 974,600. 7.1% lower.

```diff
diff --git a/parallel_hnsw_amd/csrc/api.hip b/parallel_hnsw_amd/csrc/api.hip
--- a/parallel_hnsw_amd/csrc/api.hip
+++ b/parallel_hnsw_amd/csrc/api.hip
@@ -685,6 +685,30 @@
     }
   }
 #endif
+#ifdef PH_TABLE_PROBE
+  {
+    constexpr int NP = 2 * PH_TINY_MAX_LAYERS + 2;
+    static unsigned long long *tprobe_dev = nullptr;
+    if (!tprobe_dev) {
+      PH_HIP(hipMalloc(&tprobe_dev, NP * sizeof(unsigned long long)));
+      PH_HIP(hipMemset(tprobe_dev, 0, NP * sizeof(unsigned long long)));
+    } else {
+      unsigned long long h[NP];
+      PH_HIP(hipDeviceSynchronize());
+      PH_HIP(hipMemcpy(h, tprobe_dev, sizeof(h), hipMemcpyDeviceToHost));
+      if (h[NP - 2]) {
+        fprintf(stderr, "[table probe] %llu queries, %.1f columns staged per query; look-ups per query (LDS / global):", h[NP - 2],
+                (double)h[NP - 1] / (double)h[NP - 2]);
+        for (int l = 0; l < (int)PH_TINY_MAX_LAYERS; l++)
+          if (h[2 * l] || h[2 * l + 1])
+            fprintf(stderr, " layer %d: %.1f / %.1f", l, (double)h[2 * l] / (double)h[NP - 2], (double)h[2 * l + 1] / (double)h[NP - 2]);
+        fprintf(stderr, "\n");
+      }
+      PH_HIP(hipMemset(tprobe_dev, 0, NP * sizeof(unsigned long long)));
+    }
+    a.tprobe_out = tprobe_dev;
+  }
+#endif
 #ifdef PH_VISITED_PROBE
   {
     static unsigned long long *vprobe_dev = nullptr;
@@ -797,7 +821,8 @@
     PH_HIP(hipEventRecord(ws.evc, stream));
     if (c0) PH_HIP(hipMemsetAsync(ws.dtotals, 0, sizeof(unsigned long long) * 3 * PH_MAX_DISPATCH, stream));
     if (!kept_table) {
-      rc = ph_tiny_prepare(ix, ws, b, T, stream);
+      const bool own_dense = split && T && T < b.n_layers && b.nq >= PH_DENSE_SPLIT_MIN && !getenv("PHNSW_NO_DENSE_SPLIT");
+      rc = ph_tiny_prepare(ix, ws, b, T, stream, !own_dense && ph_search_reads_columns(ix, b));
       if (rc) return rc;
     }
     ws.d_tiny = b.tiny_layers != 0;
@@ -1012,6 +1037,15 @@
     PH_HIP(hipSetDevice(ix->store->device));
     PH_HIP(hipEventSynchronize(ws.ev1));
     PH_HIP(hipMemcpy(out_host, ws.tiny_d, need * 4u, hipMemcpyDeviceToHost));
+    if (!ws.tiny_col) return PHNSW_E_INVALID;
+    std::vector<uint32_t> col(ws.tiny_last_tn);
+    PH_HIP(hipMemcpy(col.data(), ws.tiny_col, col.size() * 4u, hipMemcpyDeviceToHost));
+    std::vector<float> row(ws.tiny_last_tn);
+    for (uint64_t p = 0; p < ws.tiny_last_npos; p++) {
+      float *r = out_host + p * ws.tiny_last_stride;
+      for (uint32_t t = 0; t < ws.tiny_last_tn; t++) row[t] = r[col[t] < ws.tiny_last_tn ? col[t] : t];
+      memcpy(r, row.data(), row.size() * 4u);
+    }
   }
   return 0;
 } catch (...) { return ph_caught(); }
diff --git a/parallel_hnsw_amd/csrc/phnsw_internal.h b/parallel_hnsw_amd/csrc/phnsw_internal.h
--- a/parallel_hnsw_amd/csrc/phnsw_internal.h
+++ b/parallel_hnsw_amd/csrc/phnsw_internal.h
@@ -112,6 +112,7 @@
   bool valid = false;
   uint64_t nodes_epoch = 0;
   uint32_t T = 0, tn = 0;
+  bool node_order = false;
   const void *nodes[PH_TINY_MAX_LAYERS] = {}, *nbrs[PH_TINY_MAX_LAYERS] = {}, *vec2node = nullptr;
   uint32_t n[PH_TINY_MAX_LAYERS] = {}, W[PH_TINY_MAX_LAYERS] = {};
   uint64_t links[PH_TINY_MAX_LAYERS] = {};
@@ -121,6 +122,7 @@
   uint64_t nodes_epoch = 0;
   const void *vecs = nullptr, *tnodes = nullptr;
   uint32_t ld = 0, tn = 0, nv = 0;
+  uint64_t cols = 0;
 };
 
 struct PhWorkspace {
@@ -145,6 +147,9 @@
   size_t tiny_nbr_bytes = 0;
   uint32_t *tiny_member = nullptr;
   size_t tiny_member_bytes = 0;
+  uint32_t *tiny_col = nullptr;
+  size_t tiny_col_bytes = 0;
+  uint64_t tiny_col_serial = 0;
   float4 *tiny_pq = nullptr, *tiny_pn = nullptr;
   size_t tiny_pq_bytes = 0, tiny_pn_bytes = 0;
   PhTinyPrepKey tiny_prep_key;
@@ -271,6 +276,9 @@
 #ifdef PH_VISITED_PROBE
   unsigned long long *vprobe_out;
 #endif
+#ifdef PH_TABLE_PROBE
+  unsigned long long *tprobe_out;
+#endif
   uint32_t vis_slots, vis_limit, vis_off;
   const uint32_t *order;
   uint32_t seg;
@@ -280,6 +288,9 @@
   uint32_t tiny_layers, tiny_n, tiny_stride;
   const float *tiny_d;
   const uint32_t *tiny_nbr;
+  const uint32_t *tiny_nbrc;
+  uint32_t tiny_cols;
+  uint32_t tiny_lds_cols, tiny_win, tiny_win_off;
   const uint32_t *tiny_member;
   uint32_t tiny_rows, tiny_row_first;
   const uint32_t *tiny_row_map;
@@ -400,7 +411,8 @@
 int ph_converted_gather_rows(const phnsw_store *s, const uint32_t *ids_dev, uint32_t first, uint32_t cnt, float *out_dev);
 int ph_converted_store_read(const phnsw_store *s, uint64_t first, uint64_t count, float *out);
 
-int ph_tiny_prepare(const phnsw_index *ix, PhWorkspace &ws, PhSearchArgs &a, uint32_t max_layers, hipStream_t stream);
+int ph_tiny_prepare(const phnsw_index *ix, PhWorkspace &ws, PhSearchArgs &a, uint32_t max_layers, hipStream_t stream, bool cols);
+bool ph_search_reads_columns(const phnsw_index *ix, const PhSearchArgs &a);
 int ph_build_table_prepare(phnsw_index *ix, PhWorkspace &ws, PhSearchArgs &a, const PhRowHint &h, uint32_t T,
                            hipStream_t stream, bool *used);
 void ph_build_table_free(phnsw_index *ix);
diff --git a/parallel_hnsw_amd/csrc/search.hip b/parallel_hnsw_amd/csrc/search.hip
--- a/parallel_hnsw_amd/csrc/search.hip
+++ b/parallel_hnsw_amd/csrc/search.hip
@@ -153,6 +153,27 @@
   return (uint32_t)(per_cu * prop.multiProcessorCount);
 }
 
+static bool kernel_reads_columns(const PhKernelChoice &k) {
+  return k.fn && tcol_shape(kf_rows(k.family) && vis_lds_shape(k.capc, k.nv), k.capc, k.nv, k.family == PH_KF_ROWS_F32,
+                            k.family == PH_KF_ROWS_I8Q);
+}
+bool ph_search_reads_columns(const phnsw_index *ix, const PhSearchArgs &a) {
+  if (a.dense_only || a.knn_mode || a.out_index) return false;
+  return kernel_reads_columns(pick_search_kernel(ix->store, std::max(a.ef, a.cap_max), a.dist.nv4, false, a.nq, false, a.filter != nullptr));
+}
+
+static void ph_tiny_window(PhSearchArgs &a, int capc, bool reads_columns) {
+  a.tiny_win = a.tiny_win_off = 0;
+  if (!a.tiny_layers || !reads_columns) return;
+  if (a.tiny_n <= a.tiny_lds_nodes) {
+    a.tiny_win = a.tiny_n;
+    a.tiny_win_off = (uint32_t)(lds_bytes(capc, 0) / 4u);
+  } else {
+    a.tiny_win = ph_tcol_window(a.tiny_lds_cols, a.vis_slots, a.tiny_n);
+    a.tiny_win_off = a.vis_off;
+  }
+}
+
 void ph_workspace_free(PhWorkspace &ws) {
   if (ws.visited) hipFree(ws.visited);
   if (ws.ovf) hipFree(ws.ovf);
@@ -273,6 +294,11 @@
   a.visited = ws.visited;
   a.visited_words = 0;
   a.vis_slots = a.vis_limit = a.vis_off = 0;
+  ph_tiny_window(a, capc, false);
+  if (a.tiny_cols) {
+    ph_set_error("internal: a dense-only launch over a table in column order");
+    return PHNSW_E_UNSUPPORTED;
+  }
   a.ovf = ws.ovf;
   a.ovf_cap = ws.ovf_cap;
   a.counter = ws.counter;
@@ -310,6 +336,7 @@
   a.seg = 0;
   a.order = nullptr;
   a.vis_slots = a.vis_limit = a.vis_off = 0;
+  ph_tiny_window(a, 2, false);
   PH_HIP(hipMemsetAsync(a.counter, 0, 512, stream));
   hipLaunchKernelGGL(fn, dim3(grid), dim3(64), lds, stream, a);
   PH_HIP(hipGetLastError());
@@ -347,6 +374,10 @@
     }
     a.ovf_s = ws.ovf_s;
   }
+  if (a.tiny_layers && a.tiny_cols && !kernel_reads_columns(k)) {
+    ph_set_error("internal: a table in column order for a kernel that reads it by table id");
+    return PHNSW_E_UNSUPPORTED;
+  }
   const ph_search_fn fn = k.fn;
   if (!fn) {
     ph_set_error("unsupported search shape: ef=%u nv4=%u", a.ef, a.dist.nv4);
@@ -365,6 +396,7 @@
   a.vis_slots = vis_slots;
   a.vis_limit = vis_slots - vis_slots / 4u;
   a.vis_off = (uint32_t)(lds_bytes(k.capc, k.pq_lds) / 4u);
+  ph_tiny_window(a, k.capc, kernel_reads_columns(k));
   PH_HIP(hipMemsetAsync(ws.counter, 0, 512, stream));
   a.seg = a.order ? (a.nq + 7u) / 8u : 0u;
   hipLaunchKernelGGL(fn, dim3(grid), dim3(64), lds_bytes(k.capc, k.pq_lds) + (size_t)vis_slots * 4u, stream, a);
diff --git a/parallel_hnsw_amd/csrc/search_kernels.h b/parallel_hnsw_amd/csrc/search_kernels.h
--- a/parallel_hnsw_amd/csrc/search_kernels.h
+++ b/parallel_hnsw_amd/csrc/search_kernels.h
@@ -9,6 +9,7 @@
 #include "phnsw_internal.h"
 
 #include "phnsw_device.h"
+#include "table_columns.h"
 
 #ifdef PH_HOP_PROFILE
 #define PH_TICK(k)                                   \
@@ -36,6 +37,16 @@
 template <int CAPC, class D>
 struct vis_lds_policy<CAPC, D, std::enable_if_t<D::ROW_STORE>>
     : std::integral_constant<bool, D::ROWS_IN_FLIGHT != 0 && vis_lds_shape(CAPC, D::CHUNKS)> {};
+
+__host__ __device__ constexpr bool tcol_shape(bool vis_table, int capc, int nv, bool f32, bool i8q) {
+  return vis_table && !(capc == 2 && ((f32 && nv == 1) || (i8q && nv == 6)));
+}
+template <int CAPC, class D, class = void>
+struct tcol_policy : std::false_type {};
+template <int CAPC, class D>
+struct tcol_policy<CAPC, D, std::enable_if_t<D::ROW_STORE>>
+    : std::integral_constant<bool, tcol_shape(vis_lds_policy<CAPC, D>::value, CAPC, D::CHUNKS, std::is_same<D, DistF32<D::CHUNKS, D::ROWS_IN_FLIGHT>>::value,
+                                              std::is_same<D, DistI8Q<D::CHUNKS, D::ROWS_IN_FLIGHT>>::value)> {};
 
 __device__ __forceinline__ uint32_t vis_slot(uint32_t id, uint32_t slots) {
   return (uint32_t)(((uint64_t)(id * 0x9E3779B1u) * slots) >> 32);
@@ -93,6 +104,7 @@
   uint32_t *const H = smem + a.vis_off;
   const uint32_t hslots = (BIG || INSTR || !vis_lds_policy<CAPC, Dist>::value) ? 0u : a.vis_slots;
   for (uint32_t i = lane; i < hslots; i += 64) H[i] = PH_EMPTY32;
+  constexpr bool TCOL = !BIG && !INSTR && tcol_policy<CAPC, Dist>::value;
 
   uint32_t seg_cur = 0, seg_done = 0;
   if (a.order) {
@@ -187,8 +199,21 @@
     }
     const float *Dg = a.tiny_d + trow * a.tiny_stride;
     if (T) {
-      if (tiny_lds_row)
-        for (uint32_t i = lane; i < a.tiny_n; i += 64) Dl[i] = Dg[i];
+      if constexpr (TCOL) {
+        if (layer_lo < T) {
+          float *const Wl = (float *)(smem + a.tiny_win_off);
+          for (uint32_t i = lane; i < a.tiny_win; i += 64) Wl[i] = Dg[i];
+#ifdef PH_TABLE_PROBE
+          if (lane == 0) {
+            atomicAdd(&a.tprobe_out[2u * PH_TINY_MAX_LAYERS], 1ull);
+            atomicAdd(&a.tprobe_out[2u * PH_TINY_MAX_LAYERS + 1u], (unsigned long long)a.tiny_win);
+          }
+#endif
+        }
+      } else {
+        if (tiny_lds_row)
+          for (uint32_t i = lane; i < a.tiny_n; i += 64) Dl[i] = Dg[i];
+      }
       for (uint32_t i = lane; i < tiny_words; i += 64) Vl[i] = 0u;
     }
     queue_sync<BIG>();
@@ -196,12 +221,16 @@
     for (uint32_t li = a.knn_mode ? last_layer : layer_lo; li < layer_hi && err == ST_OK; li++) {
       PhLayerDev L = a.layers[li];
       const bool tl = li < T;
+      if constexpr (TCOL) {
+        if (li == T && T && layer_lo < T && !tiny_lds_row)
+          for (uint32_t i = lane; i < a.tiny_win; i += 64) H[i] = PH_EMPTY32;
+      }
       if (tl) {
         const PhLayerDev TLy = a.layers[T - 1];
         L.n_nodes = a.tiny_n;
         L.nodes = TLy.nodes;
         L.vec2node = TLy.vec2node;
-        L.neighbors = a.tiny_nbr + a.tiny_off[li];
+        L.neighbors = (TCOL ? a.tiny_nbrc : a.tiny_nbr) + a.tiny_off[li];
       }
       const bool identity = L.vec2node == nullptr;
       bool hv = hslots && !tl;
@@ -302,6 +331,9 @@
       const bool probing = a.probe_pos && li == last_layer && !tl;
       uint32_t probe_p0 = 0, probe_cnt[11] = {0, 0, 0, 0, 0, 0, 0, 0, 0, 0, 0};
       if (probing) probe_p0 = a.probe_pos[Qid[0] & IDM];
+#endif
+#ifdef PH_TABLE_PROBE
+      uint32_t tp_lds = 0, tp_glb = 0;
 #endif
 #ifdef PH_HOP_PROFILE
       uint64_t tprof[8] = {0, 0, 0, 0, 0, 0, 0, 0};
@@ -373,9 +405,10 @@
         PH_TICK(1)
         bool fresh = false;
         if (tl) {
-          if (nb < L.n_nodes) {
-            uint32_t bit = 1u << (nb & 31);
-            fresh = !(atomicOr(&Vl[nb >> 5], bit) & bit);
+          const uint32_t t = TCOL ? ph_tcol_tid(nb) : nb;
+          if (t < L.n_nodes) {
+            uint32_t bit = 1u << (t & 31);
+            fresh = !(atomicOr(&Vl[t >> 5], bit) & bit);
           }
         } else {
           fresh = visit(nb, nb < L.n_nodes);
@@ -401,7 +434,17 @@
         float myd;
         if (tl) {
           myd = 0.f;
-          if (fresh) myd = tiny_lds_row ? Dl[nb] : Dg[nb];
+          if constexpr (TCOL) {
+            const uint32_t col = ph_tcol_col(nb);
+            nb = ph_tcol_tid(nb);
+#ifdef PH_TABLE_PROBE
+            tp_lds += (uint32_t)__popcll(__ballot(fresh && ph_tcol_in_window(col, a.tiny_win)));
+            tp_glb += (uint32_t)__popcll(__ballot(fresh && !ph_tcol_in_window(col, a.tiny_win)));
+#endif
+            if (fresh) myd = ph_tcol_in_window(col, a.tiny_win) ? ((const float *)(smem + a.tiny_win_off))[col] : Dg[col];
+          } else {
+            if (fresh) myd = tiny_lds_row ? Dl[nb] : Dg[nb];
+          }
         } else if constexpr (Dist::EARLY) {
           myd = dist.finish(a.dist, fm, lane);
         } else {
@@ -572,6 +615,12 @@
                tprof[3] * 0.01, tprof[4] * 0.01, tprof[5] * 0.01, tprof[6] * 0.01);
 #endif
 
+#ifdef PH_TABLE_PROBE
+      if (tl && lane == 0) {
+        atomicAdd(&a.tprobe_out[2u * li], (unsigned long long)tp_lds);
+        atomicAdd(&a.tprobe_out[2u * li + 1u], (unsigned long long)tp_glb);
+      }
+#endif
 #ifdef PH_VISITED_PROBE
       if (!tl && lane == 0) {
         const uint32_t k = li == last_layer ? 1u : 0u;
@@ -723,6 +772,10 @@
       queue_sync<BIG>();
     }
 
+    if constexpr (TCOL) {
+      if (T && layer_lo < T && !tiny_lds_row && layer_hi <= T)
+        for (uint32_t i = lane; i < a.tiny_win; i += 64) H[i] = PH_EMPTY32;
+    }
     if (err != ST_OK) {
       if (!DENSE_ONLY)
         for (uint64_t w = lane; w < a.visited_words; w += 64) vis[w] = 0u;
diff --git a/parallel_hnsw_amd/csrc/table_columns.h b/parallel_hnsw_amd/csrc/table_columns.h
--- /dev/null
+++ b/parallel_hnsw_amd/csrc/table_columns.h
@@ -0,0 +1,45 @@
+#pragma once
+#include <stdint.h>
+
+#if defined(__HIPCC__)
+#define PH_TCOL_HD __host__ __device__
+#else
+#define PH_TCOL_HD
+#endif
+
+#define PH_TCOL_EMPTY 0xFFFFFFFFu
+
+PH_TCOL_HD static inline bool ph_tcol_is_upper(uint32_t member, uint32_t T, bool node_order) {
+  return !node_order && T >= 2u && ((member >> (T - 2u)) & 1u) != 0u;
+}
+
+PH_TCOL_HD static inline uint32_t ph_tcol_column(bool upper, uint32_t tid, uint32_t uppers_before, uint32_t n_upper) {
+  return upper ? uppers_before : n_upper + (tid - uppers_before);
+}
+
+PH_TCOL_HD static inline uint32_t ph_tcol_window(uint32_t cap, uint32_t lds_words, uint32_t tiny_n) {
+  uint32_t w = lds_words < tiny_n ? lds_words : tiny_n;
+  return cap < w ? cap : w;
+}
+PH_TCOL_HD static inline bool ph_tcol_in_window(uint32_t col, uint32_t lds_cols) { return col < lds_cols; }
+
+PH_TCOL_HD static inline uint32_t ph_tcol_pack(uint32_t tid, uint32_t col) {
+  return tid == PH_TCOL_EMPTY ? PH_TCOL_EMPTY : (col << 16) | tid;
+}
+PH_TCOL_HD static inline uint32_t ph_tcol_tid(uint32_t w) { return w & 0xFFFFu; }
+PH_TCOL_HD static inline uint32_t ph_tcol_col(uint32_t w) { return w >> 16; }
+
+static inline uint32_t ph_tcol_order_host(const uint32_t *member, uint32_t tiny_n, uint32_t T, bool node_order,
+                                          uint32_t *col_of, uint32_t *tid_of) {
+  uint32_t n_upper = 0;
+  for (uint32_t t = 0; t < tiny_n; t++) n_upper += ph_tcol_is_upper(member[t], T, node_order) ? 1u : 0u;
+  uint32_t before = 0;
+  for (uint32_t t = 0; t < tiny_n; t++) {
+    const bool up = ph_tcol_is_upper(member[t], T, node_order);
+    const uint32_t c = ph_tcol_column(up, t, before, n_upper);
+    col_of[t] = c;
+    tid_of[c] = t;
+    before += up ? 1u : 0u;
+  }
+  return n_upper;
+}
diff --git a/parallel_hnsw_amd/csrc/tiny.hip b/parallel_hnsw_amd/csrc/tiny.hip
--- a/parallel_hnsw_amd/csrc/tiny.hip
+++ b/parallel_hnsw_amd/csrc/tiny.hip
@@ -5,13 +5,20 @@
 #include <cstring>
 
 #include "phnsw_device.h"
+#include "table_columns.h"
+
+static_assert(PH_TINY_MAX_NODES < 0xFFFFu, "a table id and a column share a neighbour word (ph_tcol_pack)");
 
 struct PhTinyPrepArgs {
   PhLayerDev layers[PH_TINY_MAX_LAYERS];
   uint32_t T, tiny_n;
   uint32_t off[PH_TINY_MAX_LAYERS];
   uint32_t *nbr;
+  uint32_t *nbrc;
   uint32_t *member;
+  uint32_t *col;
+  uint32_t *colnodes;
+  uint32_t node_order;
 };
 
 __global__ void ph_tiny_prep_kernel(PhTinyPrepArgs p) {
@@ -38,6 +45,37 @@
       }
       p.nbr[p.off[l] + (uint64_t)t * L.W + k] = tn;
     }
+  }
+}
+
+__global__ __launch_bounds__(256) void ph_tiny_cols_kernel(PhTinyPrepArgs p) {
+  __shared__ uint32_t cnt[257];
+  const uint32_t t = threadIdx.x, run = (p.tiny_n + 255u) / 256u;
+  const uint32_t lo = min(t * run, p.tiny_n), hi = min(lo + run, p.tiny_n);
+  const uint32_t *tnodes = p.layers[p.T - 1].nodes;
+  uint32_t c = 0;
+  for (uint32_t i = lo; i < hi; i++) c += ph_tcol_is_upper(p.member[i], p.T, p.node_order != 0u) ? 1u : 0u;
+  cnt[t + 1u] = c;
+  if (t == 0) cnt[0] = 0u;
+  __syncthreads();
+  if (t == 0)
+    for (uint32_t k = 1; k <= 256u; k++) cnt[k] += cnt[k - 1u];
+  __syncthreads();
+  uint32_t before = cnt[t];
+  const uint32_t n_upper = cnt[256];
+  for (uint32_t i = lo; i < hi; i++) {
+    const bool up = ph_tcol_is_upper(p.member[i], p.T, p.node_order != 0u);
+    const uint32_t col = ph_tcol_column(up, i, before, n_upper);
+    p.col[i] = col;
+    p.colnodes[col] = tnodes[i];
+    before += up ? 1u : 0u;
+  }
+}
+
+__global__ void ph_tiny_nbr_cols_kernel(const uint32_t *nbr, uint32_t *nbrc, uint32_t n, const uint32_t *col, uint32_t tiny_n) {
+  for (uint32_t i = blockIdx.x * blockDim.x + threadIdx.x; i < n; i += gridDim.x * blockDim.x) {
+    const uint32_t w = nbr[i];
+    nbrc[i] = w < tiny_n ? ph_tcol_pack(w, col[w]) : PH_EMPTY32;
   }
 }
 
@@ -447,6 +485,9 @@
   if (ws.tiny_d) hipFree(ws.tiny_d);
   if (ws.tiny_nbr) hipFree(ws.tiny_nbr);
   if (ws.tiny_member) hipFree(ws.tiny_member);
+  if (ws.tiny_col) hipFree(ws.tiny_col);
+  ws.tiny_col = nullptr;
+  ws.tiny_col_bytes = 0;
   if (ws.tiny_pq) hipFree(ws.tiny_pq);
   if (ws.tiny_pn) hipFree(ws.tiny_pn);
   ws.tiny_pq = ws.tiny_pn = nullptr;
@@ -519,16 +560,33 @@
   return e;
 }
 
+static bool table_node_order() {
+  const char *e = getenv("PHNSW_TABLE_COLUMNS");
+  return e && !strcmp(e, "node");
+}
+static uint32_t tiny_lds_cols_cap() {
+  const char *e = getenv("PHNSW_TINY_LDS_COLS");
+  return (e && atoll(e) >= 0) ? (uint32_t)std::min<long long>(atoll(e), 0xFFFFFFFFll) : 0xFFFFFFFFu;
+}
+
+static bool same_order(const PhTinyPrepKey &a, const PhTinyPrepKey &b) {
+  if (!a.valid || !b.valid || a.nodes_epoch != b.nodes_epoch || a.T != b.T || a.tn != b.tn || a.vec2node != b.vec2node ||
+      a.node_order != b.node_order)
+    return false;
+  for (uint32_t l = 0; l < a.T; l++)
+    if (a.nodes[l] != b.nodes[l] || a.n[l] != b.n[l]) return false;
+  return true;
+}
 static bool same_key(const PhTinyPrepKey &a, const PhTinyPrepKey &b) {
-  if (!a.valid || !b.valid || a.nodes_epoch != b.nodes_epoch || a.T != b.T || a.tn != b.tn || a.vec2node != b.vec2node) return false;
+  if (!same_order(a, b)) return false;
   for (uint32_t l = 0; l < a.T; l++)
-    if (a.nodes[l] != b.nodes[l] || a.nbrs[l] != b.nbrs[l] || a.n[l] != b.n[l] || a.W[l] != b.W[l] || a.links[l] != b.links[l])
+    if (a.nbrs[l] != b.nbrs[l] || a.n[l] != b.n[l] || a.W[l] != b.W[l] || a.links[l] != b.links[l])
       return false;
   return true;
 }
 
 static int tiny_prep_graph(const phnsw_index *ix, PhWorkspace &ws, PhSearchArgs &a, uint32_t T, uint32_t tn, hipStream_t stream,
-                           bool *kept = nullptr) {
+                           bool cols, bool *kept = nullptr) {
   if (kept) *kept = false;
   PhTinyPrepArgs p;
   memset(&p, 0, sizeof(p));
@@ -540,6 +598,7 @@
   key.T = T;
   key.tn = tn;
   key.vec2node = a.layers[T - 1].vec2node;
+  key.node_order = !cols || table_node_order();
   size_t nbr_words = 0;
   for (uint32_t l = 0; l < T; l++) {
     p.layers[l] = a.layers[l];
@@ -552,23 +611,38 @@
     key.W[l] = a.layers[l].W;
     key.links[l] = ix->layers[l].links_epoch;
   }
-  const uint32_t *nbr_was = ws.tiny_nbr, *member_was = ws.tiny_member;
-  if (grow(&ws.tiny_nbr, &ws.tiny_nbr_bytes, nbr_words * 4u) != hipSuccess ||
+  const uint32_t *nbr_was = ws.tiny_nbr, *member_was = ws.tiny_member, *col_was = ws.tiny_col;
+  if (grow(&ws.tiny_nbr, &ws.tiny_nbr_bytes, 2u * nbr_words * 4u) != hipSuccess ||
+      grow(&ws.tiny_col, &ws.tiny_col_bytes, (size_t)2u * PH_TINY_MAX_NODES * 4u) != hipSuccess ||
       grow(&ws.tiny_member, &ws.tiny_member_bytes, (size_t)(PH_TINY_MAX_NODES + 1u) * 4u) != hipSuccess) {
     (void)hipGetLastError();
     ws.tiny_prep_key.valid = false;
     return 1;
   }
-  if (ws.tiny_nbr == nbr_was && ws.tiny_member == member_was && same_key(key, ws.tiny_prep_key)) {
+  const bool bufs_kept = ws.tiny_nbr == nbr_was && ws.tiny_member == member_was && ws.tiny_col == col_was;
+  a.tiny_nbr = ws.tiny_nbr;
+  a.tiny_nbrc = ws.tiny_nbr + nbr_words;
+  a.tiny_member = ws.tiny_member;
+  a.tiny_cols = key.node_order ? 0u : 1u;
+  a.tiny_lds_cols = tiny_lds_cols_cap();
+  if (bufs_kept && same_key(key, ws.tiny_prep_key)) {
     if (kept) *kept = true;
     return 0;
   }
+  if (!(bufs_kept && same_order(key, ws.tiny_prep_key))) ws.tiny_col_serial++;
   ws.tiny_prep_key = key;
   p.nbr = ws.tiny_nbr;
+  p.nbrc = ws.tiny_nbr + nbr_words;
   p.member = ws.tiny_member;
+  p.col = ws.tiny_col;
+  p.colnodes = ws.tiny_col + PH_TINY_MAX_NODES;
+  p.node_order = key.node_order ? 1u : 0u;
   PH_HIP(hipMemsetAsync(ws.tiny_nbr, 0xFF, nbr_words * 4u, stream));
   PH_HIP(hipMemsetAsync(ws.tiny_member, 0, (size_t)(tn + 1u) * 4u, stream));
   hipLaunchKernelGGL(ph_tiny_prep_kernel, dim3((tn + 255u) / 256u, T), dim3(256), 0, stream, p);
+  hipLaunchKernelGGL(ph_tiny_cols_kernel, dim3(1), dim3(256), 0, stream, p);
+  hipLaunchKernelGGL(ph_tiny_nbr_cols_kernel, dim3((uint32_t)std::min<size_t>((nbr_words + 255u) / 256u, 4096u)), dim3(256), 0,
+                     stream, (const uint32_t *)p.nbr, p.nbrc, (uint32_t)nbr_words, (const uint32_t *)p.col, tn);
   PH_HIP(hipGetLastError());
   return 0;
 }
@@ -600,12 +674,13 @@
   key.nodes_epoch = ix->nodes_epoch;
   key.vecs = dist.rows.base;
   key.tnodes = tnodes;
+  key.cols = ws.tiny_col_serial;
   key.ld = dist.ld;
   key.tn = tn;
   key.nv = kpad;
   const PhTinyPackKey &have = ws.tiny_pack_key;
   const bool pn_kept = ws.tiny_pn == pn_was && key.valid && have.valid && have.nodes_epoch == key.nodes_epoch &&
-                       have.vecs == key.vecs && have.tnodes == key.tnodes && have.ld == key.ld && have.tn == key.tn &&
+                       have.vecs == key.vecs && have.tnodes == key.tnodes && have.cols == key.cols && have.ld == key.ld && have.tn == key.tn &&
                        have.nv == key.nv;
   ws.tiny_pack_key = key;
   if (kept) *kept = pn_kept;
@@ -687,12 +762,13 @@
     key.nodes_epoch = ix->nodes_epoch;
     key.vecs = dist.rows.base;
     key.tnodes = tnodes;
+  key.cols = ws.tiny_col_serial;
     key.ld = dist.ld;
     key.tn = tn;
     key.nv = (uint32_t)nv;
     const PhTinyPackKey &have = ws.tiny_pack_key;
     const bool pn_kept = ws.tiny_pn == pn_was && key.valid && have.valid && have.nodes_epoch == key.nodes_epoch &&
-                         have.vecs == key.vecs && have.tnodes == key.tnodes && have.ld == key.ld && have.tn == key.tn &&
+                         have.vecs == key.vecs && have.tnodes == key.tnodes && have.cols == key.cols && have.ld == key.ld && have.tn == key.tn &&
                          have.nv == key.nv;
     ws.tiny_pack_key = key;
     if (kept) *kept = pn_kept;
@@ -766,7 +842,7 @@
   return 0;
 }
 
-int ph_tiny_prepare(const phnsw_index *ix, PhWorkspace &ws, PhSearchArgs &a, uint32_t max_layers, hipStream_t stream) {
+int ph_tiny_prepare(const phnsw_index *ix, PhWorkspace &ws, PhSearchArgs &a, uint32_t max_layers, hipStream_t stream, bool cols) {
   a.tiny_layers = 0;
   a.tiny_rows = 0;
   if (a.knn_mode || a.layer_lo) return 0;
@@ -788,9 +864,9 @@
     }
   }
   bool prep_kept = false, pack_kept = false;
-  int rc = tiny_prep_graph(ix, ws, a, T, tn, stream, &prep_kept);
+  int rc = tiny_prep_graph(ix, ws, a, T, tn, stream, cols, &prep_kept);
   if (rc) return rc < 0 ? rc : 0;
-  rc = tiny_table(ix, ws, a.dist, a.queries, a.ldq, a.qids, a.order, npos, a.layers[T - 1].nodes, tn, stride, ws.tiny_d, stream,
+  rc = tiny_table(ix, ws, a.dist, a.queries, a.ldq, a.qids, a.order, npos, ws.tiny_col + PH_TINY_MAX_NODES, tn, stride, ws.tiny_d, stream,
                   beside ? 1 : 2, &pack_kept);
   if (rc) return rc < 0 ? rc : 0;
   if (getenv("PHNSW_VERBOSE")) {
@@ -810,8 +886,6 @@
   a.tiny_lds_nodes = PH_TINY_LDS_NODES;
   a.tiny_stride = stride;
   a.tiny_d = ws.tiny_d;
-  a.tiny_nbr = ws.tiny_nbr;
-  a.tiny_member = ws.tiny_member;
   return 0;
 }
 
@@ -914,17 +988,20 @@
     B.lo = B.hi = need_lo;
     B.epoch = ix->nodes_epoch;
   }
+  int rc = tiny_prep_graph(ix, ws, a, T, tn, stream, false);
+  if (rc) return rc < 0 ? rc : 0;
+  const uint32_t *colnodes = ws.tiny_col + PH_TINY_MAX_NODES;
   auto fill = [&](uint32_t lo, uint32_t hi) -> int {
     const uint32_t PIECE = 131072u;
     for (uint32_t at = lo; at < hi; at += PIECE) {
       const uint32_t cnt = std::min(PIECE, hi - at);
-      int rc = tiny_table(ix, ws, a.dist, nullptr, 0, h.qnodes + at, nullptr, cnt, tnodes, tn, stride,
+      int rc = tiny_table(ix, ws, a.dist, nullptr, 0, h.qnodes + at, nullptr, cnt, colnodes, tn, stride,
                           B.D + (size_t)(at - B.lo_alloc) * stride, stream);
       if (rc) return rc;
     }
     return 0;
   };
-  int rc = 0;
+  rc = 0;
   if (B.lo == B.hi) {
     rc = fill(need_lo, need_hi);
     if (!rc) B.lo = need_lo, B.hi = need_hi;
@@ -938,8 +1015,6 @@
       if (!rc) B.hi = need_hi;
     }
   }
-  if (rc) return rc < 0 ? rc : 0;
-  rc = tiny_prep_graph(ix, ws, a, T, tn, stream);
   if (rc) return rc < 0 ? rc : 0;
   a.tiny_layers = T;
   a.tiny_n = tn;
@@ -949,8 +1024,6 @@
   a.tiny_rows = 1;
   a.tiny_row_first = B.lo_alloc;
   a.tiny_row_map = h.vec2node;
-  a.tiny_nbr = ws.tiny_nbr;
-  a.tiny_member = ws.tiny_member;
   *used = true;
   return 0;
 }
```
